# m-dayani/EORB_SLAM

Measured on AMD Instinct MI355X. Metric: front-end frames/s (event-accumulate + extract + match) per GPU; HBM GB/s vs roofline, higher is better.
Workload: dtype f32; 1 GPU; BASELINE.json configs[1]: synthetic 1000000 events/slice on 240x180 (shapes generator, DAVIS sensor pixels; raw (x,y,t,p) records resolved on the GPU through the calibrator's undistortion maps built from the EvETHZ intrinsics, as the reference loader does on the CPU), ev2im_gauss sigma=1 -> ORB-1000 (1.2, 4 levels, FAST 10/0, edge 19) -> SearchForInitialization vs previous slice; input=raw, sequences_per_gpu=1, parallelism=1 GPU

## Files before the change

### eorb_slam_amd/csrc/ev_slots.hip

```cpp
#include "eorb_ctx.h"
#include "ev_common.h"
#include "dev_math.h"
#include "sl_hot_asm.h"
#include <algorithm>
#include <memory>
#include <stdlib.h>
#include <string.h>
#include <vector>

namespace eorb {

constexpr uint32_t kNoSlot = 0xffu;
typedef uint16_t slot_entry;
constexpr uint32_t kEntryTag = 0x1000u;
constexpr int kSlotScatWaves = 8;
constexpr uint16_t kNoGeo = 0xffffu;
constexpr int kCountWaves = 16;

__global__ void sl_assign_kernel(const uint32_t* __restrict__ src_info, int nsrc, int W, int H, int h, int TX,
                                 uint32_t* __restrict__ tile_nslots, uint2* __restrict__ slot_tab, uint16_t* __restrict__ slot_geo,
                                 int* __restrict__ info)
{
    const int i = blockIdx.x * blockDim.x + threadIdx.x;
    if (i >= nsrc) { if (i == nsrc) slot_geo[i] = kNoGeo; return; }
    const uint32_t w = src_info[i];
    const int xi = (int)(int16_t)(w & 0xffff), yi = (int)(int16_t)(w >> 16);
    uint2 o = make_uint2(0u, 0xffffffffu);
    if (xi != -32768) {
        const int x0 = max(xi - h, 0), x1 = min(xi + h, W - 1), y0 = max(yi - h, 0), y1 = min(yi + h, H - 1);
        if (x1 >= x0 && y1 >= y0) {
            const int tx0 = x0 >> 3, tx1 = x1 >> 3, ty0 = y0 >> 3, ty1 = y1 >> 3;
            const int nx = tx1 - tx0 + 1, ny = ty1 - ty0 + 1;
            uint32_t slots = 0xffffffffu;
            for (int dy = 0; dy < ny; dy++)
                for (int dx = 0; dx < nx; dx++) {
                    uint32_t s = atomicAdd(&tile_nslots[(ty0 + dy) * TX + tx0 + dx], 1u);
                    if (s >= kNoSlot) { atomicOr(&info[2], 1); s = 0; }
                    const int sh = 8 * (dy * 2 + dx);
                    slots = (slots & ~(0xffu << sh)) | (s << sh);
                }
            o.x = (uint32_t)tx0 | ((uint32_t)ty0 << 8) | ((uint32_t)nx << 16) | ((uint32_t)ny << 18);
            o.y = slots;
        }
    }
    slot_tab[i] = o;
    slot_geo[i] = o.x ? (uint16_t)((o.x & 0x7f) | (((o.x >> 8) & 0x7f) << 7) | ((((o.x >> 16) & 3) - 1) << 14) | ((((o.x >> 18) & 3) - 1) << 15)) : kNoGeo;
}

__global__ __launch_bounds__(1024) void sl_rowbase_kernel(const uint32_t* __restrict__ nslots, int NT, uint32_t* __restrict__ rowbase,
                                                          int* __restrict__ info)
{
    __shared__ uint32_t wsum[16];
    __shared__ uint32_t wmax[16];
    const int tid = threadIdx.x, lane = tid & 63, wave = tid >> 6;
    const int per = (NT + 1023) / 1024;
    const int t0 = tid * per, t1 = min(t0 + per, NT);
    uint32_t mine = 0, mx = 0;
    for (int t = t0; t < t1; t++) { const uint32_t v = nslots[t]; mine += v; mx = max(mx, v); }
    uint32_t incl = (uint32_t)wave_incl_scan((int)mine);
#pragma unroll
    for (int d = 32; d >= 1; d >>= 1) mx = max(mx, (uint32_t)__shfl_xor((int)mx, d, 64));
    if (lane == 63) wsum[wave] = incl;
    if (lane == 0) wmax[wave] = mx;
    __syncthreads();
    uint32_t before = incl - mine;
    for (int w = 0; w < wave; w++) before += wsum[w];
    for (int t = t0; t < t1; t++) { rowbase[t] = before; before += nslots[t]; }
    if (tid == 1023) {
        uint32_t m = 0;
        for (int w = 0; w < 16; w++) m = max(m, wmax[w]);
        info[0] = (int)before; info[1] = (int)m;
    }
}

__global__ __launch_bounds__(256) void sl_rows_kernel(const uint32_t* __restrict__ src_info, const uint2* __restrict__ slot_tab, int nsrc,
                                                      int W, int H, int h, int TX, const float* __restrict__ stamps, int stamp_stride,
                                                      int SWP, const float2* __restrict__ lut, float two_sig2, float norm, const uint32_t* __restrict__ rowbase, float* __restrict__ rows)
{
    __shared__ uint64_t tab[32];
    if (threadIdx.x < 32) tab[threadIdx.x] = kExp2Tab[threadIdx.x];
    __syncthreads();
    const int src = blockIdx.x * 4 + (threadIdx.x >> 6), lane = threadIdx.x & 63;
    if (src >= nsrc) return;
    const uint2 st = slot_tab[src];
    const int nx = (st.x >> 16) & 3, ny = (st.x >> 18) & 3;
    if (!nx || !ny) return;
    const uint32_t w = src_info[src];
    const int xi = (int)(int16_t)(w & 0xffff), yi = (int)(int16_t)(w >> 16);
    const int tx0 = st.x & 0xff, ty0 = (st.x >> 8) & 0xff;
    for (int dy = 0; dy < ny; dy++)
        for (int dx = 0; dx < nx; dx++) {
            const uint32_t slot = (st.y >> (8 * (dy * 2 + dx))) & 0xffu;
            const int tile = (ty0 + dy) * TX + tx0 + dx;
            const int px = (tx0 + dx) * 8 + (lane & 7), py = (ty0 + dy) * 8 + (lane >> 3);
            const int i = px - xi + h, j = py - yi + h;
            float v = 0.0f;
            if (i >= 0 && i <= 2 * h && j >= 0 && j <= 2 * h && px < W && py < H) {
                if (stamps) v = stamps[(size_t)src * stamp_stride + i * SWP + j];
                else {
                    const float2 q = lut[src];
                    const float xr = q.x - (float)xi, yr = q.y - (float)yi;
                    const float fx = (float)(i - h) - xr, fy = (float)(j - h) - yr;
                    const float xx = fx * fx, yy = fy * fy;
                    float dd = xx + yy;
                    dd = dd / two_sig2;
                    v = dev_expf_nonpos<true>(-dd, tab) / norm;
                }
            }
            rows[((size_t)rowbase[tile] + slot) * 64 + lane] = v;
        }
}

constexpr int kOffsetsInArg = 256;
struct SliceOffsets { int64_t off[kOffsetsInArg + 1]; };
__global__ __launch_bounds__(256) void sl_chunks_kernel(SliceOffsets S, int B, int chunk_shift , int NT, int nchunks,
                                                        ChunkDesc* __restrict__ chunks, int* __restrict__ slice_c0, int64_t* __restrict__ slice_eb)
{
    __shared__ int c0[kOffsetsInArg + 1];
    __shared__ long long e0[kOffsetsInArg + 1];
    const int tid = threadIdx.x;
    const int64_t chunk = (int64_t)1 << chunk_shift;
    const int64_t* off = (const int64_t*)__builtin_amdgcn_kernarg_segment_ptr();
    const int64_t n = tid < B ? off[tid + 1] - off[tid] : 0;
    c0[tid + 1] = tid < B ? (int)((n + chunk - 1) >> chunk_shift) : 0;
    e0[tid + 1] = tid < B ? ((n * 4 + (int64_t)NT * 16 + 15) & ~(int64_t)15) : 0;
    if (tid == 0) { c0[0] = 0; e0[0] = 0; }
    __syncthreads();
    for (int d = 1; d < kOffsetsInArg; d <<= 1) {
        const int a = tid + 1 > d ? c0[tid + 1 - d] : 0;
        const long long b = tid + 1 > d ? e0[tid + 1 - d] : 0;
        __syncthreads();
        c0[tid + 1] += a; e0[tid + 1] += b;
        __syncthreads();
    }
    if (blockIdx.x == 0) {
        if (tid < B) slice_eb[tid] = e0[tid];
        for (int b = tid; b <= B; b += blockDim.x) slice_c0[b] = c0[b];
    }
    const int g = blockIdx.x * blockDim.x + tid;
    if (g >= nchunks) return;
    int lo = 0, hi = B;
    while (hi - lo > 1) { const int mid = (lo + hi) >> 1; if (c0[mid] <= g) lo = mid; else hi = mid; }
    const int64_t start = off[lo] + ((int64_t)(g - c0[lo]) << chunk_shift);
    ChunkDesc cd; cd.start = start; cd.n = (int32_t)min(chunk, off[lo + 1] - start); cd.slice = lo;
    chunks[g] = cd;
}

template <int stride>
__device__ __forceinline__ uint32_t sl_load_rec(const unsigned char* e, int k)
{
    if (stride == 2) { const uint32_t v = *(const uint16_t*)(e + (size_t)k * 2); return v == 0xffffu ? 0x7fffffffu : v; }
    return *(const uint32_t*)(e + (size_t)k * (size_t)(stride < 0 ? -stride : stride));
}
template <int stride>
__global__ __launch_bounds__(256) void sl_count_kernel(const eorb_raw_event* __restrict__ ev, const ChunkDesc* __restrict__ chunks,
                                                       const uint2* __restrict__ slot_tab, int LW, int LH, int TX, int NT,
                                                       uint16_t* __restrict__ segcnt)
{
    extern __shared__ uint32_t cnt[];
    const ChunkDesc cd = chunks[blockIdx.x];
    for (int i = threadIdx.x; i < NT; i += blockDim.x) cnt[i] = 0;
    __syncthreads();
    const unsigned char* e = (const unsigned char*)ev + (size_t)cd.start * (size_t)(stride < 0 ? -stride : stride);
    const uint32_t xmask = stride == 4 ? 0x7fffu : 0xffffu;
    const bool hashed = stride < 0 || stride == 2;
    constexpr int U = 8;
    for (int k0 = threadIdx.x; k0 < cd.n; k0 += blockDim.x * U) {
        uint32_t xy[U], rg[U];
#pragma unroll
        for (int u = 0; u < U; u++) { const int k = k0 + u * blockDim.x; xy[u] = k < cd.n ? sl_load_rec<stride>(e, k) : 0xffffffffu; }
#pragma unroll
        for (int u = 0; u < U; u++) {
            const int x = (int)(xy[u] & xmask), y = (int)(xy[u] >> 16);
            const uint32_t row = xy[u] & 0x7fffffffu;
            if (hashed) rg[u] = (row != 0x7fffffffu && row < (uint32_t)LW * (uint32_t)LH) ? slot_tab[row].x : 0u;
            else rg[u] = (x < LW && y < LH) ? slot_tab[(uint32_t)y * (uint32_t)LW + x].x : 0u;
        }
#pragma unroll
        for (int u = 0; u < U; u++) {
            const int nx = (rg[u] >> 16) & 3, ny = (rg[u] >> 18) & 3;
            const int t0 = (int)((rg[u] >> 8) & 0xff) * TX + (int)(rg[u] & 0xff);
            if (nx && ny) {
                atomicAdd(&cnt[t0], 1u);
                if (nx > 1) atomicAdd(&cnt[t0 + 1], 1u);
                if (ny > 1) { atomicAdd(&cnt[t0 + TX], 1u); if (nx > 1) atomicAdd(&cnt[t0 + TX + 1], 1u); }
            }
        }
    }
    __syncthreads();
    uint16_t* sc = segcnt + (size_t)blockIdx.x * NT;
    for (int i = threadIdx.x; i < NT; i += blockDim.x) sc[i] = (uint16_t)cnt[i];
}

__device__ __forceinline__ uint32_t sl_dict_hash(uint64_t k)
{
    k ^= k >> 33; k *= 0xff51afd7ed558ccdull; k ^= k >> 33; k *= 0xc4ceb9fe1a85ec53ull; k ^= k >> 33;
    return (uint32_t)k;
}
template <int stride, bool KEYED = false, bool RANKS = false>
__global__ __launch_bounds__(64 * kCountWaves) void sl_count_lds_kernel(const eorb_raw_event* __restrict__ ev, const ChunkDesc* __restrict__ chunks,
                                                                       int nchunks, const uint16_t* __restrict__ slot_geo, int LW, int LH,
                                                                       int TX, int NT, uint16_t* __restrict__ segcnt, SlotDict D = SlotDict{nullptr, 0u, nullptr, nullptr, 0},
                                                                       uint16_t* __restrict__ rec16 = nullptr)
{
    extern __shared__ uint32_t smc[];
    const int tid = threadIdx.x, lane = tid & 63, wave = tid >> 6;
    const int ntab = (LW * LH + 2) >> 1, NTp = (NT + 1) & ~1;
    for (int i = tid; i < ntab; i += 64 * kCountWaves) smc[i] = ((const uint32_t*)slot_geo)[i];
    const uint16_t* tab = (const uint16_t*)smc;
    uint32_t* cnt = smc + ntab + wave * (NTp >> 1);
    __syncthreads();
    constexpr int astride = stride < 0 ? -stride : stride;
    const uint32_t xmask = stride == 4 ? 0x7fffu : 0xffffu;
    constexpr int U = 8;
    for (int ch = blockIdx.x * kCountWaves + wave; ch < nchunks; ch += gridDim.x * kCountWaves) {
        const ChunkDesc cd = chunks[ch];
        for (int i = lane; i < (NTp >> 1); i += 64) cnt[i] = 0u;
        const unsigned char* e = (const unsigned char*)ev + (size_t)cd.start * (size_t)astride;
        uint32_t xyn[U];
        if (!KEYED) {
#pragma unroll
            for (int u = 0; u < U; u++) { const int k = lane + u * 64; xyn[u] = k < cd.n ? sl_load_rec<stride>(e, k) : 0xffffffffu; }
        }
        for (int k0 = lane; k0 < cd.n; k0 += 64 * U) {
            uint32_t xy[U], g[U];
            uint32_t r16[U];
            if (KEYED) {
                uint2 pos[U]; uint32_t ex[U], ey[U], ez[U], hh[U];
#pragma unroll
                for (int u = 0; u < U; u++) { const int k = k0 + u * 64; pos[u] = k < cd.n ? *(const uint2*)(e + (size_t)k * 16) : make_uint2(0x7fc00000u, 0x7fc00000u); }
#pragma unroll
                for (int u = 0; u < U; u++) { hh[u] = sl_dict_hash((uint64_t)pos[u].x | ((uint64_t)pos[u].y << 32)) & D.mask; const uint4 t = D.hash[hh[u]]; ex[u] = t.x; ey[u] = t.y; ez[u] = t.z; }
#pragma unroll
                for (int u = 0; u < U; u++) {
                    const int k = k0 + u * 64;
                    const float fx = __uint_as_float(pos[u].x), fy = __uint_as_float(pos[u].y);
                    uint32_t id = 0x7fffffffu;
                    if (k < cd.n && fx == fx && fy == fy) {
                        uint32_t h = hh[u], qx = ex[u], qy = ey[u], qz = ez[u]; int probes = 0;
                        while (!(qx == pos[u].x && qy == pos[u].y) && qz != 0xffffffffu && ++probes <= 64) { h = (h + 1) & D.mask; const uint4 t = D.hash[h]; qx = t.x; qy = t.y; qz = t.z; }
                        if (qx == pos[u].x && qy == pos[u].y && qz != 0xffffffffu) id = qz;
                        else atomicAdd(D.miss, 1);
                    }
                    if (RANKS) r16[u] = id < (uint32_t)LW * (uint32_t)LH ? id : 0xffffu;
                    else if (k < cd.n) {
                        if (D.rec2) ((uint16_t*)D.rec)[cd.start + k] = id == 0x7fffffffu ? (uint16_t)0xffffu : (uint16_t)id;
                        else D.rec[cd.start + k] = id;
                    }
                    g[u] = id < (uint32_t)LW * (uint32_t)LH ? tab[id] : kNoGeo;
                }
            } else {
#pragma unroll
            for (int u = 0; u < U; u++) xy[u] = xyn[u];
            if (k0 + 64 * U < cd.n) {
#pragma unroll
                for (int u = 0; u < U; u++) { const int k = k0 + 64 * U + u * 64; xyn[u] = k < cd.n ? sl_load_rec<stride>(e, k) : 0xffffffffu; }
            }
#pragma unroll
            for (int u = 0; u < U; u++) {
                const uint32_t x = xy[u] & xmask, y = xy[u] >> 16, row = xy[u] & 0x7fffffffu;
                if (stride < 0 || stride == 2) g[u] = row < (uint32_t)LW * (uint32_t)LH ? tab[row] : kNoGeo;
                else g[u] = (x < (uint32_t)LW && y < (uint32_t)LH) ? tab[y * (uint32_t)LW + x] : kNoGeo;
                if (RANKS) {
                    if (stride < 0 || stride == 2) r16[u] = row < (uint32_t)LW * (uint32_t)LH ? row : 0xffffu;
                    else r16[u] = (x < (uint32_t)LW && y < (uint32_t)LH) ? y * (uint32_t)LW + x : 0xffffu;
                } else if ((stride == 16 || stride == 4) && rec16) {
                    const int k = k0 + u * 64;
                    if (k < cd.n) rec16[cd.start + k] = (x < (uint32_t)LW && y < (uint32_t)LH) ? (uint16_t)(y * (uint32_t)LW + x) : (uint16_t)0xffffu;
                }
            }
            }
            if (RANKS) {
#pragma unroll
                for (int u = 0; u < U; u++) {
                    uint64_t rk = 0ull;
                    if (g[u] != kNoGeo) {
                        const int tx0 = (int)(g[u] & 0x7f), ty0 = (int)((g[u] >> 7) & 0x7f);
                        const int nx = 1 + (int)((g[u] >> 14) & 1), ny = 1 + (int)((g[u] >> 15) & 1);
#pragma unroll
                        for (int j = 0; j < 4; j++) {
                            const int dx = ((j & 1) - tx0) & 1, dy = ((j >> 1) - ty0) & 1;
                            if (dx < nx && dy < ny) {
                                const int t = (ty0 + dy) * TX + tx0 + dx;
                                const uint32_t o = atomicAdd(&cnt[t >> 1], 1u << (16 * (t & 1)));
                                rk |= (uint64_t)((o >> (16 * (t & 1))) & 0xfffu) << (12 * j);
                            }
                        }
                    }
                    const int k = k0 + u * 64;
                    if (k < cd.n) ((uint64_t*)rec16)[cd.start + k] = (uint64_t)(r16[u] & 0xffffu) | (rk << 16);
                }
                continue;
            }
#pragma unroll
            for (int u = 0; u < U; u++) {
                if (g[u] != kNoGeo) {
                    const int t0 = (int)((g[u] >> 7) & 0x7f) * TX + (int)(g[u] & 0x7f);
                    const bool two_x = (g[u] >> 14) & 1, two_y = (g[u] >> 15) & 1;
                    atomicAdd(&cnt[t0 >> 1], 1u << (16 * (t0 & 1)));
                    if (two_x) atomicAdd(&cnt[(t0 + 1) >> 1], 1u << (16 * ((t0 + 1) & 1)));
                    if (two_y) {
                        atomicAdd(&cnt[(t0 + TX) >> 1], 1u << (16 * ((t0 + TX) & 1)));
                        if (two_x) atomicAdd(&cnt[(t0 + TX + 1) >> 1], 1u << (16 * ((t0 + TX + 1) & 1)));
                    }
                }
            }
        }
        __builtin_amdgcn_wave_barrier();
        uint16_t* sc = segcnt + (size_t)ch * NT;
        const uint16_t* c16 = (const uint16_t*)cnt;
        for (int i = lane; i < NT; i += 64) sc[i] = c16[i];
        __builtin_amdgcn_wave_barrier();
    }
}

__global__ __launch_bounds__(1024) void sl_scan_kernel(const int* __restrict__ slice_chunk0, const uint16_t* __restrict__ segcnt, int NT,
                                                       uint32_t* __restrict__ segbase, uint32_t* __restrict__ tile_cnt,
                                                       uint32_t* __restrict__ tile_base)
{
    __shared__ uint32_t wsum[16];
    __shared__ uint32_t carry;
    const int slice = blockIdx.x;
    const int c0 = slice_chunk0[slice], c1 = slice_chunk0[slice + 1];
    const int lane = threadIdx.x & 63, wave = threadIdx.x >> 6;
    if (threadIdx.x == 0) carry = 0;
    __syncthreads();
    for (int t0 = 0; t0 < NT; t0 += blockDim.x) {
        const int tile = t0 + threadIdx.x;
        uint32_t run = 0;
        if (tile < NT) {
            int c = c0;
            for (; c + 8 <= c1; c += 8) {
                uint32_t v[8];
#pragma unroll
                for (int u = 0; u < 8; u++) v[u] = segcnt[(size_t)(c + u) * NT + tile];
#pragma unroll
                for (int u = 0; u < 8; u++) { segbase[(size_t)(c + u) * NT + tile] = run; run += v[u]; }
            }
            for (; c < c1; c++) { const uint32_t v = segcnt[(size_t)c * NT + tile]; segbase[(size_t)c * NT + tile] = run; run += v; }
            tile_cnt[(size_t)slice * NT + tile] = run;
        }
        const uint32_t padded = (run + 15u) & ~15u;
        uint32_t incl = (uint32_t)wave_incl_scan((int)padded);
        if (lane == 63) wsum[wave] = incl;
        __syncthreads();
        uint32_t before = carry;
        for (int w = 0; w < wave; w++) before += wsum[w];
        if (tile < NT) tile_base[(size_t)slice * NT + tile] = before + incl - padded;
        __syncthreads();
        if (threadIdx.x == blockDim.x - 1) carry = before + incl;
        __syncthreads();
    }
}

__global__ __launch_bounds__(64 * kSlotScatWaves) void sl_scatter_kernel(const eorb_raw_event* __restrict__ ev, const ChunkDesc* __restrict__ chunks,
                                                                         const uint2* __restrict__ slot_tab, int stride, int LW, int LH, int TX, int TY,
                                                                         int NT, int chunk_cap, const int64_t* __restrict__ slice_ebase,
                                                                         const uint32_t* __restrict__ segbase, const uint32_t* __restrict__ tile_base,
                                                                         slot_entry* __restrict__ entries)
{
    extern __shared__ unsigned char sm2[];
    __shared__ uint32_t s_wsum[kSlotScatWaves];
    constexpr int NTHR = 64 * kSlotScatWaves;
    constexpr int R = 2;
    const int tid = threadIdx.x, lane = tid & 63, wave = tid >> 6;
    const int chunk = blockIdx.x;
    const ChunkDesc cd = chunks[chunk];
    const int NTp = (NT + 1) & ~1;
    uint32_t* pay = (uint32_t*)sm2;
    uint16_t* prng = (uint16_t*)(pay + chunk_cap);
    uint16_t* sidx = prng + chunk_cap;
    uint16_t* cntw = sidx + (size_t)chunk_cap * R * R;
    uint16_t* loff = cntw + kSlotScatWaves * NTp;
    uint32_t* gbase = (uint32_t*)(loff + NTp + 2);
    for (int i = tid; i < kSlotScatWaves * NTp / 2; i += NTHR) ((uint32_t*)cntw)[i] = 0u;
    const unsigned char* e = (const unsigned char*)ev + (size_t)cd.start * (size_t)(stride < 0 ? -stride : stride);
    const uint32_t xmask = stride == 4 ? 0x7fffu : 0xffffu;
    const bool hashed = stride < 0 || stride == 2;
    const int Q = (((cd.n + kSlotScatWaves - 1) / kSlotScatWaves) + 63) & ~63;
    const int S = Q >> 6;
    constexpr int SMAX = 4;
    uint32_t rng[SMAX];
    __syncthreads();
    uint32_t* cw32 = (uint32_t*)(cntw + wave * NTp);
    uint32_t rsrc[SMAX];
#pragma unroll
    for (int s = 0; s < SMAX; s++) {
        const int k = wave * Q + s * 64 + lane;
        uint32_t q = 0xffffffffu;
        if (s < S && k < cd.n) q = stride == 2 ? sl_load_rec<2>(e, k) : *(const uint32_t*)(e + (size_t)k * (size_t)(stride < 0 ? -stride : stride));
        const int x = q == 0xffffffffu ? 0xffff : (int)(q & xmask), y = (int)(q >> 16);
        if (hashed) { const uint32_t row = q & 0x7fffffffu; rsrc[s] = (row != 0x7fffffffu && row < (uint32_t)LW * (uint32_t)LH) ? row : 0xffffffffu; }
        else rsrc[s] = (x < LW && y < LH) ? (uint32_t)y * (uint32_t)LW + x : 0xffffffffu;
    }
    uint2 rst[SMAX];
#pragma unroll
    for (int s = 0; s < SMAX; s++) rst[s] = rsrc[s] != 0xffffffffu ? slot_tab[rsrc[s]] : make_uint2(0u, 0xffffffffu);
#pragma unroll
    for (int s = 0; s < SMAX; s++) {
        rng[s] = 0u;
        const int k = wave * Q + s * 64 + lane;
        if (s < S && k < cd.n) {
            const uint32_t rg = rst[s].x;
            const int nx = (rg >> 16) & 3, ny = (rg >> 18) & 3;
            pay[k] = rst[s].y;
            prng[k] = (uint16_t)(rg & 0xffff);
            if (nx && ny) {
                rng[s] = rg;
                const int t0 = (int)((rg >> 8) & 0xff) * TX + (int)(rg & 0xff);
                for (int dy = 0; dy < ny; dy++)
                    for (int dx = 0; dx < nx; dx++) {
                        const int t = t0 + dy * TX + dx;
                        atomicAdd(&cw32[t >> 1], 1u << (16 * (t & 1)));
                    }
            }
        }
    }
    __syncthreads();
    {
        const int per = (NT + NTHR - 1) / NTHR;
        const int t0 = tid * per, t1 = min(t0 + per, NT);
        uint32_t mine = 0;
        for (int t = t0; t < t1; t++) {
            uint32_t run = 0;
#pragma unroll
            for (int w = 0; w < kSlotScatWaves; w++) { const uint32_t v = cntw[w * NTp + t]; cntw[w * NTp + t] = (uint16_t)run; run += v; }
            loff[t] = (uint16_t)run;
            mine += run;
            gbase[t] = tile_base[(size_t)cd.slice * NT + t] + segbase[(size_t)chunk * NT + t];
        }
        uint32_t incl = (uint32_t)wave_incl_scan((int)mine);
        if (lane == 63) s_wsum[wave] = incl;
        __syncthreads();
        uint32_t before = incl - mine;
        for (int w = 0; w < wave; w++) before += s_wsum[w];
        for (int t = t0; t < t1; t++) { const uint32_t v = loff[t]; loff[t] = (uint16_t)before; before += v; }
        if (tid == NTHR - 1) loff[NT] = (uint16_t)before;
    }
    __syncthreads();
    const uint64_t lt_mask = (lane == 0) ? 0ull : (~0ull >> (64 - lane));
    uint16_t* cw = cntw + wave * NTp;
    const int txr = (TX + R - 1) / R;
    int mbits = 1; while ((1 << mbits) < txr * ((TY + R - 1) / R)) mbits++;
#pragma unroll
    for (int s = 0; s < SMAX; s++) {
        if (s >= S) break;
        const uint32_t rg = rng[s];
        const int tx0 = rg & 0xff, ty0 = (rg >> 8) & 0xff, tx1 = tx0 + (int)((rg >> 16) & 3) - 1, ty1 = ty0 + (int)((rg >> 18) & 3) - 1;
        const bool valid = rg != 0u;
        const uint16_t kloc = (uint16_t)(wave * Q + s * 64 + lane);
#pragma unroll
        for (int cy = 0; cy < R; cy++) {
#pragma unroll
            for (int cx = 0; cx < R; cx++) {
                const int tx = tx0 + ((cx - tx0 % R) + R) % R;
                const int ty = ty0 + ((cy - ty0 % R) + R) % R;
                const bool has = valid && tx <= tx1 && ty <= ty1;
                uint64_t m = __ballot(has);
                if (m == 0ull) continue;
                const int key = has ? ty * TX + tx : 0;
                const int mkey = has ? (ty / R) * txr + (tx / R) : 0;
                for (int b = 0; b < mbits; b++) {
                    const bool bit = (mkey >> b) & 1;
                    const uint64_t bal = __ballot(bit);
                    m &= bit ? bal : ~bal;
                }
                if (has) {
                    const int rank = __popcll(m & lt_mask);
                    const uint32_t base = cw[key];
                    sidx[(uint32_t)loff[key] + base + rank] = (uint16_t)(kloc | ((tx - tx0) << 11) | ((ty - ty0) << 13));
                    if (rank == 0) cw[key] = (uint16_t)(base + (uint32_t)__popcll(m));
                }
            }
        }
    }
    __syncthreads();
    slot_entry* out = entries + (size_t)slice_ebase[cd.slice];
    const int E = loff[NT];
    for (int p = tid; p < E; p += NTHR) {
        const uint32_t sv = sidx[p];
        const int k = sv & 0x7ff;
        const int dx = (sv >> 11) & 3, dy = (sv >> 13) & 3;
        const uint32_t r0 = prng[k];
        const int t = ((int)(r0 >> 8) + dy) * TX + (int)(r0 & 0xff) + dx;
        const uint32_t slot = (pay[k] >> (8 * (dy * 2 + dx))) & 0xffu;
        out[(size_t)gbase[t] + (uint32_t)(p - (int)loff[t])] = (slot_entry)(kEntryTag | slot);
    }
}

template <int stride, int NW >
__global__ __launch_bounds__(64 * NW) void sl_scatter_rank_kernel(const eorb_raw_event* __restrict__ ev, const ChunkDesc* __restrict__ chunks,
                                                                              const uint2* __restrict__ slot_tab, int LW, int LH, int TX, int NT,
                                                                              int chunk_cap, const int64_t* __restrict__ slice_ebase,
                                                                              const uint32_t* __restrict__ segbase, const uint32_t* __restrict__ tile_base,
                                                                              slot_entry* __restrict__ entries)
{
    extern __shared__ unsigned char sm2[];
    __shared__ uint32_t s_wsum[NW];
    constexpr int NTHR = 64 * NW;
    const int tid = threadIdx.x, lane = tid & 63, wave = tid >> 6;
    const int chunk = blockIdx.x;
    const ChunkDesc cd = chunks[chunk];
    const int NTp = (NT + 1) & ~1;
    uint32_t* gbase = (uint32_t*)sm2;
    uint16_t* stile = (uint16_t*)(gbase + NT);
    uint16_t* cntw = stile + (size_t)chunk_cap * 4;
    uint16_t* loff = cntw + NW * NTp;
    uint8_t* sorted = (uint8_t*)(loff + NTp + 2);
    for (int i = tid; i < NW * NTp / 2; i += NTHR) ((uint32_t*)cntw)[i] = 0u;
    const unsigned char* e = (const unsigned char*)ev + (size_t)cd.start * (size_t)(stride < 0 ? -stride : stride);
    const uint32_t xmask = stride == 4 ? 0x7fffu : 0xffffu;
    const bool hashed = stride < 0 || stride == 2;
    const int Q = (((cd.n + NW - 1) / NW) + 63) & ~63;
    const int S = Q >> 6;
    constexpr int SMAX = 4;
    __syncthreads();
    uint32_t* cw32 = (uint32_t*)(cntw + wave * NTp);
    uint32_t rsrc[SMAX];
#pragma unroll
    for (int s = 0; s < SMAX; s++) {
        const int k = wave * Q + s * 64 + lane;
        const uint32_t q = (s < S && k < cd.n) ? sl_load_rec<stride>(e, k) : 0xffffffffu;
        const int x = q == 0xffffffffu ? 0xffff : (int)(q & xmask), y = (int)(q >> 16);
        if (hashed) { const uint32_t row = q & 0x7fffffffu; rsrc[s] = (row != 0x7fffffffu && row < (uint32_t)LW * (uint32_t)LH) ? row : 0xffffffffu; }
        else rsrc[s] = (x < LW && y < LH) ? (uint32_t)y * (uint32_t)LW + x : 0xffffffffu;
    }
    uint2 rst[SMAX];
#pragma unroll
    for (int s = 0; s < SMAX; s++) rst[s] = rsrc[s] != 0xffffffffu ? slot_tab[rsrc[s]] : make_uint2(0u, 0xffffffffu);
    uint32_t rk[SMAX];
#pragma unroll
    for (int s = 0; s < SMAX; s++) {
        const uint32_t rg = rst[s].x;
        const int nx = (rg >> 16) & 3, ny = (rg >> 18) & 3;
        const int tx0 = rg & 0xff, ty0 = (rg >> 8) & 0xff;
        rk[s] = 0u;
#pragma unroll
        for (int j = 0; j < 4; j++) {
#ifdef EORB_TEST_RANK_ORDER_BUG
            const int dx = j & 1, dy = j >> 1;
#else
            const int dx = ((j & 1) - tx0) & 1, dy = ((j >> 1) - ty0) & 1;
#endif
            if (nx && ny && dx < nx && dy < ny) {
                const int t = (ty0 + dy) * TX + tx0 + dx;
                const uint32_t o = atomicAdd(&cw32[t >> 1], 1u << (16 * (t & 1)));
                rk[s] |= ((o >> (16 * (t & 1))) & 0xffu) << (8 * j);
            }
        }
    }
    __syncthreads();
#if defined(EORB_KO_SCAT) && EORB_KO_SCAT == 1
    if (rk[0] == 0x12345678u) entries[0] = 0; return;
#endif
    {
        const int per = (NT + NTHR - 1) / NTHR;
        const int t0 = tid * per, t1 = min(t0 + per, NT);
        uint32_t mine = 0;
        for (int t = t0; t < t1; t++) {
            uint32_t run = 0;
#pragma unroll
            for (int w = 0; w < NW; w++) { const uint32_t v = cntw[w * NTp + t]; cntw[w * NTp + t] = (uint16_t)run; run += v; }
            loff[t] = (uint16_t)run;
            mine += run;
        }
        uint32_t incl = (uint32_t)wave_incl_scan((int)mine);
        if (lane == 63) s_wsum[wave] = incl;
        __syncthreads();
        uint32_t before = incl - mine;
        for (int w = 0; w < wave; w++) before += s_wsum[w];
        for (int t = t0; t < t1; t++) {
            const uint32_t v = loff[t]; loff[t] = (uint16_t)before;
            gbase[t] = tile_base[(size_t)cd.slice * NT + t] + segbase[(size_t)chunk * NT + t] - before;
            before += v;
        }
        if (tid == NTHR - 1) loff[NT] = (uint16_t)before;
    }
    __syncthreads();
#if defined(EORB_KO_SCAT) && EORB_KO_SCAT == 2
    if (rk[0] == 0x12345678u) entries[0] = 0; return;
#endif
    const uint16_t* cw = cntw + wave * NTp;
#pragma unroll
    for (int s = 0; s < SMAX; s++) {
        const uint32_t rg = rst[s].x, sb = rst[s].y;
        const int nx = (rg >> 16) & 3, ny = (rg >> 18) & 3;
        const int tx0 = rg & 0xff, ty0 = (rg >> 8) & 0xff;
#pragma unroll
        for (int j = 0; j < 4; j++) {
#ifdef EORB_TEST_RANK_ORDER_BUG
            const int dx = j & 1, dy = j >> 1;
#else
            const int dx = ((j & 1) - tx0) & 1, dy = ((j >> 1) - ty0) & 1;
#endif
            if (nx && ny && dx < nx && dy < ny) {
                const int t = (ty0 + dy) * TX + tx0 + dx;
                const uint32_t pos = (uint32_t)loff[t] + cw[t] + ((rk[s] >> (8 * j)) & 0xffu);
                sorted[pos] = (uint8_t)((sb >> (8 * (dy * 2 + dx))) & 0xffu);
                stile[pos] = (uint16_t)t;
            }
        }
    }
    __syncthreads();
#if defined(EORB_KO_SCAT) && EORB_KO_SCAT == 3
    if (rk[0] == 0x12345678u) entries[0] = 0; return;
#endif
    slot_entry* out = entries + (size_t)slice_ebase[cd.slice];
    const int E = loff[NT];
    for (int p = tid; p < E; p += NTHR) out[(size_t)(uint32_t)(gbase[stile[p]] + (uint32_t)p)] = (slot_entry)(kEntryTag | sorted[p]);
}

template <int NW>
__global__ __launch_bounds__(64 * NW) void sl_scatter_pre_kernel(const uint64_t* __restrict__ rec, const ChunkDesc* __restrict__ chunks,
                                                                 const uint2* __restrict__ slot_tab, int nsrc, int TX, int NT, int chunk_cap,
                                                                 const int64_t* __restrict__ slice_ebase, const uint16_t* __restrict__ segcnt,
                                                                 const uint32_t* __restrict__ segbase, const uint32_t* __restrict__ tile_base,
                                                                 slot_entry* __restrict__ entries)
{
    extern __shared__ unsigned char sm2[];
    __shared__ uint32_t s_wsum[NW];
    constexpr int NTHR = 64 * NW;
    const int tid = threadIdx.x, lane = tid & 63, wave = tid >> 6;
    const int chunk = blockIdx.x;
    const ChunkDesc cd = chunks[chunk];
    const int NTp = (NT + 1) & ~1;
    uint32_t* gbase = (uint32_t*)sm2;
    uint16_t* stile = (uint16_t*)(gbase + NT);
    uint16_t* loff = stile + (size_t)chunk_cap * 4;
    uint8_t* sorted = (uint8_t*)(loff + NTp + 2);
    const int Q = (((cd.n + NW - 1) / NW) + 63) & ~63;
    const int S = Q >> 6;
    constexpr int SMAX = 4;
    uint64_t rr[SMAX]; uint2 rst[SMAX];
#pragma unroll
    for (int s = 0; s < SMAX; s++) {
        const int k = wave * Q + s * 64 + lane;
        rr[s] = (s < S && k < cd.n) ? rec[cd.start + k] : 0xffffull;
    }
#pragma unroll
    for (int s = 0; s < SMAX; s++) {
        const uint32_t row = (uint32_t)(rr[s] & 0xffffull);
        rst[s] = (row != 0xffffu && row < (uint32_t)nsrc) ? slot_tab[row] : make_uint2(0u, 0xffffffffu);
    }
    {
        const int per = (NT + NTHR - 1) / NTHR;
        const int t0 = tid * per, t1 = min(t0 + per, NT);
        const uint16_t* sc = segcnt + (size_t)chunk * NT;
        uint32_t mine = 0;
        for (int t = t0; t < t1; t++) mine += sc[t];
        uint32_t incl = (uint32_t)wave_incl_scan((int)mine);
        if (lane == 63) s_wsum[wave] = incl;
        __syncthreads();
        uint32_t before = incl - mine;
        for (int w = 0; w < wave; w++) before += s_wsum[w];
        for (int t = t0; t < t1; t++) {
            const uint32_t v = sc[t];
            loff[t] = (uint16_t)before;
            gbase[t] = tile_base[(size_t)cd.slice * NT + t] + segbase[(size_t)chunk * NT + t] - before;
            before += v;
        }
        if (tid == NTHR - 1) loff[NT] = (uint16_t)before;
    }
    __syncthreads();
#if defined(EORB_KO_SCAT) && EORB_KO_SCAT == 2
    if (rst[0].x == 0x12345678u) entries[0] = 0; return;
#endif
#pragma unroll
    for (int s = 0; s < SMAX; s++) {
        const uint32_t rg = rst[s].x, sb = rst[s].y;
        const int nx = (rg >> 16) & 3, ny = (rg >> 18) & 3;
        const int tx0 = rg & 0xff, ty0 = (rg >> 8) & 0xff;
        const uint64_t rk = rr[s] >> 16;
#pragma unroll
        for (int j = 0; j < 4; j++) {
            const int dx = ((j & 1) - tx0) & 1, dy = ((j >> 1) - ty0) & 1;
            if (nx && ny && dx < nx && dy < ny) {
                const int t = (ty0 + dy) * TX + tx0 + dx;
                const uint32_t pos = (uint32_t)loff[t] + (uint32_t)((rk >> (12 * j)) & 0xfffull);
                sorted[pos] = (uint8_t)((sb >> (8 * (dy * 2 + dx))) & 0xffu);
                stile[pos] = (uint16_t)t;
            }
        }
    }
    __syncthreads();
#if defined(EORB_KO_SCAT) && EORB_KO_SCAT == 3
    if (rst[0].x == 0x12345678u) entries[0] = 0; return;
#endif
    slot_entry* out = entries + (size_t)slice_ebase[cd.slice];
    const int E = loff[NT];
    for (int p = tid; p < E; p += NTHR) out[(size_t)(uint32_t)(gbase[stile[p]] + (uint32_t)p)] = (slot_entry)(kEntryTag | sorted[p]);
}

__global__ __launch_bounds__(1024) void sl_rankcheck_kernel(unsigned long long* bad)
{
    __shared__ uint32_t cnt[16 * 64];
    __shared__ uint32_t noise[1024];
    const int lane = threadIdx.x & 63, wave = threadIdx.x >> 6;
    unsigned long long nbad = 0;
    uint32_t h = (uint32_t)(blockIdx.x * 1024 + threadIdx.x) * 2654435761u + 12345u;
    for (int t = 0; t < 64; t++) {
        for (int i = threadIdx.x; i < 16 * 64; i += blockDim.x) cnt[i] = 0;
        __syncthreads();
        h = h * 1664525u + 1013904223u;
        const int spread = 1 << (1 + (t % 7));
        const uint32_t a = ((h >> 9) % spread) + wave * 128;
        const bool act = ((h >> 3) & 7u) != 0u;
        uint32_t r = 0xffffffffu;
        noise[(threadIdx.x * 33 + t) & 1023] = h;
        uint32_t rr[4];
#pragma unroll
        for (int q = 0; q < 4; q++) {
            rr[q] = 0xffffffffu;
            if (act && ((h >> (12 + q)) & 1u)) { const uint32_t o = atomicAdd(&cnt[a >> 1], 1u << (16 * (a & 1))); rr[q] = (o >> (16 * (a & 1))) & 0xffffu; }
        }
#pragma unroll
        for (int q = 0; q < 4; q++) {
            r = rr[q];
            for (int j = 0; j < 64; j++) {
                const uint32_t aj = __shfl(a, j, 64), rj = __shfl(r, j, 64);
                if (r != 0xffffffffu && rj != 0xffffffffu && j < lane && aj == a && !(rj < r)) nbad++;
            }
        }
        __syncthreads();
    }
    if (noise[threadIdx.x] == 0x12345u) nbad += 0;
    if (nbad) atomicAdd(bad, nbad);
}

constexpr int kHotBuckets = 16, kHotCap = 8192;
struct HotDesc { uint32_t slice, tile, cnt, off_lo, off_hi, tx0, ty0, rows_off; };
__global__ __launch_bounds__(256) void sl_plan_kernel(const uint32_t* __restrict__ tile_cnt, const uint32_t* __restrict__ tile_base,
                                                      const int64_t* __restrict__ slice_ebase, int B, int NT, int TX, uint32_t hot_min,
                                                      const uint32_t* __restrict__ nslots, const uint32_t* __restrict__ rowbase,
                                                      uint4* __restrict__ items, uint32_t* __restrict__ tile_w, uint32_t* __restrict__ tile_m,
                                                      uint32_t* __restrict__ ctr, uint32_t* __restrict__ hot_cnt, HotDesc* __restrict__ hot_items,
                                                      uint32_t hot_cap )
{
    extern __shared__ uint32_t pc[];
    __shared__ uint32_t red[8];
    __shared__ uint32_t hb[kHotBuckets], hbase[kHotBuckets];
    uint32_t* hloc = pc + B;
    const int t = blockIdx.x, tid = threadIdx.x;
    const bool hot_ok = hot_min != 0u && nslots[t] <= (uint32_t)SL_HOT_NROWS;
    if (tid < kHotBuckets) hb[tid] = 0u;
    __syncthreads();
    for (int s = tid; s < B; s += blockDim.x) {
        const uint32_t c = tile_cnt[(size_t)s * NT + t];
        uint32_t v = c;
        if (hot_ok && c >= hot_min) {
            const int lg = 31 - __clz(c), lg0 = 31 - __clz(hot_min);
            const int q = (lg - lg0) * 4 + (int)((c >> max(lg - 2, 0)) & 3u) - (int)((hot_min >> max(lg0 - 2, 0)) & 3u);
            const int b = kHotBuckets - 1 - min(max(q, 0), kHotBuckets - 1);
            hloc[s] = ((uint32_t)b << 16) | atomicAdd(&hb[b], 1u);
            v = c | 0x80000000u;
        }
        pc[s] = v;
    }
    __syncthreads();
    if (tid < kHotBuckets) hbase[tid] = hb[tid] ? atomicAdd(&hot_cnt[tid], hb[tid]) : 0u;
    __syncthreads();
    uint32_t sum = 0, mx = 0;
    for (int s = tid; s < B; s += blockDim.x) {
        uint32_t v = pc[s];
        if (v & 0x80000000u) {
            const uint32_t c = v & 0x7fffffffu, b = hloc[s] >> 16, k = hbase[b] + (hloc[s] & 0xffffu);
            if (k < hot_cap) {
                const uint64_t off = ((uint64_t)slice_ebase[s] + tile_base[(size_t)s * NT + t]) * sizeof(slot_entry);
                HotDesc d; d.slice = (uint32_t)s; d.tile = (uint32_t)t; d.cnt = c; d.off_lo = (uint32_t)off; d.off_hi = (uint32_t)(off >> 32);
                d.tx0 = (uint32_t)(t % TX) * 8u; d.ty0 = (uint32_t)(t / TX) * 8u; d.rows_off = rowbase[t] * 256u;
                hot_items[(size_t)b * kHotCap + k] = d;
            } else { v = c; pc[s] = v; atomicAdd(&hot_cnt[33], 1u); }
        }
        if (!(v & 0x80000000u)) { sum += v; mx = max(mx, v); }
    }
    __syncthreads();
    const bool sorted = B <= 2048;
    for (int s = tid; s < B; s += blockDim.x) {
        const uint32_t c = pc[s];
        int rank = s;
        if (sorted) { rank = 0; for (int j = 0; j < B; j++) { const uint32_t v = pc[j]; rank += (v > c || (v == c && j < s)) ? 1 : 0; } }
        const uint64_t off = ((uint64_t)slice_ebase[s] + tile_base[(size_t)s * NT + t]) * sizeof(slot_entry);
        items[(size_t)t * B + rank] = make_uint4((uint32_t)s | (c & 0x80000000u), c & 0x7fffffffu, (uint32_t)off, (uint32_t)(off >> 32));
    }
#pragma unroll
    for (int d = 32; d >= 1; d >>= 1) { sum += (uint32_t)__shfl_xor((int)sum, d, 64); mx = max(mx, (uint32_t)__shfl_xor((int)mx, d, 64)); }
    if ((tid & 63) == 0) { red[tid >> 6] = sum; red[4 + (tid >> 6)] = mx; }
    __syncthreads();
    if (tid == 0) {
        tile_w[t] = red[0] + red[1] + red[2] + red[3];
        tile_m[t] = max(max(red[4], red[5]), max(red[6], red[7]));
        ctr[t] = 0u;
    }
}
__global__ __launch_bounds__(1024) void sl_tasks_kernel(const uint32_t* __restrict__ tile_w, const uint32_t* __restrict__ tile_m, int NT, int G,
                                                        int max_per_tile, uint32_t* __restrict__ scratch , uint32_t* __restrict__ task_tile, uint32_t* __restrict__ hot_cnt,
                                                        uint32_t hot_cap)
{
    if (threadIdx.x < kHotBuckets) hot_cnt[threadIdx.x] = min(hot_cnt[threadIdx.x], hot_cap);
    __shared__ unsigned long long wred[16];
    __shared__ uint32_t wsum[16], wsum2[16];
    const int tid = threadIdx.x, lane = tid & 63, wave = tid >> 6;
    unsigned long long tot = 0;
    for (int t = tid; t < NT; t += 1024) tot += tile_w[t];
#pragma unroll
    for (int d = 32; d >= 1; d >>= 1) tot += (unsigned long long)__shfl_xor((long long)tot, d, 64);
    if (lane == 0) wred[wave] = tot;
    __syncthreads();
    tot = 0;
    for (int w = 0; w < 16; w++) tot += wred[w];
    const unsigned long long spare = (unsigned long long)max(G - NT, 0);
    uint32_t* nsorted = scratch; uint32_t* tsorted = scratch + NT;
    extern __shared__ uint32_t tm[];
    for (int t = tid; t < NT; t += 1024) tm[t] = tile_m[t];
    __syncthreads();
    for (int t = tid; t < NT; t += 1024) {
        const uint32_t m = tm[t];
        int rank = 0;
        for (int u = 0; u < NT; u++) { const uint32_t v = tm[u]; rank += (v > m || (v == m && u < t)) ? 1 : 0; }
        uint32_t n = 1u + (tot ? (uint32_t)((unsigned long long)tile_w[t] * spare / tot) : 0u);
        n = min(n, (uint32_t)max(max_per_tile, 1));
        nsorted[rank] = n; tsorted[rank] = (uint32_t)t;
    }
    __syncthreads();
    const int per = (NT + 1023) / 1024;
    const int r0 = tid * per, r1 = min(r0 + per, NT);
    uint32_t mine1 = 0, mine2 = 0;
    for (int r = r0; r < r1; r++) { const uint32_t n = nsorted[r], a = min(n, 2u); mine1 += a; mine2 += n - a; }
    const uint32_t incl1 = (uint32_t)wave_incl_scan((int)mine1), incl2 = (uint32_t)wave_incl_scan((int)mine2);
    if (lane == 63) { wsum[wave] = incl1; wsum2[wave] = incl2; }
    __syncthreads();
    uint32_t b1 = incl1 - mine1, b2 = incl2 - mine2, tot1 = 0;
    for (int w = 0; w < 16; w++) { if (w < wave) { b1 += wsum[w]; b2 += wsum2[w]; } tot1 += wsum[w]; }
    b2 += tot1;
    for (int r = r0; r < r1; r++) {
        const uint32_t n = nsorted[r], a = min(n, 2u), t = tsorted[r];
        for (uint32_t k = 0; k < a; k++) if (b1 + k < (uint32_t)G) task_tile[b1 + k] = t;
        for (uint32_t k = 0; k < n - a; k++) if (b2 + k < (uint32_t)G) task_tile[b2 + k] = t;
        b1 += a; b2 += n - a;
    }
    const uint32_t before = b2;
    if (tid == 1023) for (uint32_t k = before; k < (uint32_t)G; k++) task_tile[k] = 0xffffffffu;
}

struct SlotGather {
    const uint32_t* task_tile; const uint4* items; const uint8_t* entries;
    const uint32_t* nslots; const uint32_t* rowbase; const float* rows; const uint32_t* tile_w; uint32_t* ctr;
    float* img; uint32_t* minmax_enc; int* info; int* status;
    int B, W, H, TX, NT, null_slot; uint32_t prio_ref;
    unsigned long long* trace;
};

__global__ __launch_bounds__(1024) __attribute__((amdgpu_waves_per_eu(8, 8)))
void sl_gather_kernel(SlotGather P)
{
    extern __shared__ __attribute__((aligned(16))) float lds[];
    const int tid = threadIdx.x, lane = tid & 63;
#ifdef EORB_SLOT_TRACE
    const unsigned long long tr_t0 = wall_clock64(); unsigned long long tr_ent = 0, tr_items = 0, tr_kept = 0;
#endif
    const uint32_t task = P.task_tile[blockIdx.x];
    if (task == 0xffffffffu) return;
    const int tile = (int)task;
    const uint32_t wt = P.tile_w[tile];
    const int tx0 = (tile % P.TX) * kTile, ty0 = (tile / P.TX) * kTile;
    const int px = tx0 + (lane & 7), py = ty0 + (lane >> 3);
    const bool inimg = px < P.W && py < P.H;
    if ((uint32_t)(uintptr_t)lds != 0u) { if (tid == 0) { atomicOr(&P.info[3], 1); atomicOr(P.status, 256); } return; }
    if (wt) {
        const int ns = (int)P.nslots[tile];
        const int n4 = ns * 16;
        const float4* src = (const float4*)(P.rows + (size_t)P.rowbase[tile] * 64);
        float4* dst = (float4*)lds;
        for (int i = tid; i < n4; i += blockDim.x) dst[i] = src[i];
        if (tid < 16) dst[P.null_slot * 16 + tid] = make_float4(0.f, 0.f, 0.f, 0.f);
    }
    __syncthreads();
    const uint32_t nullword = (uint32_t)P.null_slot * 0x00010001u;
    uint32_t* const ctr = P.ctr + tile;
    const uint32_t lane4 = (uint32_t)lane * 4u;
    uint32_t sel0 = 0x0c0c0400u, sel1 = 0x0c0c0600u;
    asm volatile("" : "+v"(sel0), "+v"(sel1));
    const int nit = P.B;
    const uint4* const items = P.items + (size_t)tile * P.B;
    auto ticket = [&]() { int t = 0; if (lane == 0) t = (int)atomicAdd(ctr, 1u); return t; };
    auto uni = [&](uint32_t v) { return (uint32_t)__builtin_amdgcn_readfirstlane((int)v); };
    auto item_of = [&](int tkv) { return (int)min((uint32_t)__builtin_amdgcn_readfirstlane(tkv), (uint32_t)nit); };
    int k = item_of(ticket());
    uint4 d = make_uint4(0u, 0u, 0u, 0u);
    if (k < nit) d = items[k];
    uint4 En = make_uint4(0u, 0u, 0u, 0u);
    bool have_first = false;
    while (k < nit) {
        const bool hot = (uni(d.x) >> 31) != 0u;
        const int s = (int)(uni(d.x) & 0x7fffffffu);
        const uint32_t cnt = hot ? 0u : uni(d.y);
        const uint4* const list = (const uint4*)(P.entries + (((uint64_t)uni(d.w) << 32) | uni(d.z)));
        if (cnt >= P.prio_ref) __builtin_amdgcn_s_setprio(3);
        else if (cnt >= P.prio_ref / 4u) __builtin_amdgcn_s_setprio(2);
        else if (cnt >= P.prio_ref / 16u) __builtin_amdgcn_s_setprio(1);
        else __builtin_amdgcn_s_setprio(0);
        float acc = 0.0f;
        const int nblk = (int)((cnt + 511u) >> 9);
        if (!have_first && nblk) En = list[lane];
        have_first = false;
        int tk = 0; int stage_t = 0;
        uint4 dn = make_uint4(0u, 0u, 0u, 0u); int kn = nit;
        for (int b = 0; b < nblk; b++) {
            uint4 E = En;
            if (stage_t == 1) { kn = item_of(tk); if (kn < nit) dn = items[kn]; stage_t = 2; }
            else if (stage_t == 0 && nblk - b <= 4) { tk = ticket(); stage_t = 1; }
            if (b + 1 < nblk) En = list[(size_t)(b + 1) * 64 + lane];
            else if (stage_t == 2 && kn < nit && uni(dn.y)) {
                En = ((const uint4*)(P.entries + (((uint64_t)uni(dn.w) << 32) | uni(dn.z))))[lane];
                have_first = true;
            }
            const int rem = (int)cnt - b * 512;
            if (rem < 512) {
                auto fix = [&](uint32_t w, int dd) {
                    const int nv = rem - lane * 8 - dd * 2;
                    const uint32_t keep = nv >= 2 ? 0xffffffffu : (nv <= 0 ? 0u : 0xffffu);
                    return (w & keep) | (nullword & ~keep);
                };
                E.x = fix(E.x, 0); E.y = fix(E.y, 1); E.z = fix(E.z, 2); E.w = fix(E.w, 3);
            }
            const int lane_end = (min(64, (rem + 7) >> 3) + 1) & ~1;
#ifdef EORB_SLOT_TRACE
            tr_kept += (unsigned long long)lane_end * 8;
#endif
            {
            float r0, r1, r2, r3, r4, r5, r6, r7, r8, r9, r10, r11, r12, r13, r14, r15;
            int sl, sl1, se, sf;
#define SL_GROUP(EV, EW, SL, RA, RB, RC, RD, AA, AB, AC, AD) \
            "s_waitcnt lgkmcnt(8)\n" \
            "v_readlane_b32 %[se], %[" EV "], %[" SL "]\n" \
            "v_add_f32 %[acc], %[acc], %[" AA "]\n" \
            "v_readlane_b32 %[sf], %[" EW "], %[" SL "]\n" \
            "v_perm_b32 %[" RA "], %[se], %[l4], %[q0]\n" \
            "v_perm_b32 %[" RB "], %[se], %[l4], %[q1]\n" \
            "ds_read_b32 %[" RA "], %[" RA "]\n" \
            "v_add_f32 %[acc], %[acc], %[" AB "]\n" \
            "v_perm_b32 %[" RC "], %[sf], %[l4], %[q0]\n" \
            "ds_read_b32 %[" RB "], %[" RB "]\n" \
            "v_add_f32 %[acc], %[acc], %[" AC "]\n" \
            "v_perm_b32 %[" RD "], %[sf], %[l4], %[q1]\n" \
            "ds_read_b32 %[" RC "], %[" RC "]\n" \
            "v_add_f32 %[acc], %[acc], %[" AD "]\n" \
            "ds_read_b32 %[" RD "], %[" RD "]\n"
            asm volatile(
                "v_mov_b32 %[r4], 0\n v_mov_b32 %[r5], 0\n v_mov_b32 %[r6], 0\n v_mov_b32 %[r7], 0\n"
                "v_mov_b32 %[r8], 0\n v_mov_b32 %[r9], 0\n v_mov_b32 %[r10], 0\n v_mov_b32 %[r11], 0\n"
                "v_mov_b32 %[r12], 0\n v_mov_b32 %[r13], 0\n v_mov_b32 %[r14], 0\n v_mov_b32 %[r15], 0\n"
                "s_mov_b32 %[sl], 0\n"
                "1:\n"
                "s_add_u32 %[sl1], %[sl], 1\n"
                SL_GROUP("e0", "e1", "sl", "r0", "r1", "r2", "r3", "r4", "r5", "r6", "r7")
                SL_GROUP("e2", "e3", "sl", "r4", "r5", "r6", "r7", "r8", "r9", "r10", "r11")
                SL_GROUP("e0", "e1", "sl1", "r8", "r9", "r10", "r11", "r12", "r13", "r14", "r15")
                SL_GROUP("e2", "e3", "sl1", "r12", "r13", "r14", "r15", "r0", "r1", "r2", "r3")
                "s_add_u32 %[sl], %[sl], 2\n"
                "s_cmp_lt_u32 %[sl], %[lend]\n"
                "s_cbranch_scc1 1b\n"
                "s_waitcnt lgkmcnt(0)\n"
                "v_add_f32 %[acc], %[acc], %[r4]\n v_add_f32 %[acc], %[acc], %[r5]\n v_add_f32 %[acc], %[acc], %[r6]\n v_add_f32 %[acc], %[acc], %[r7]\n"
                "v_add_f32 %[acc], %[acc], %[r8]\n v_add_f32 %[acc], %[acc], %[r9]\n v_add_f32 %[acc], %[acc], %[r10]\n v_add_f32 %[acc], %[acc], %[r11]\n"
                "v_add_f32 %[acc], %[acc], %[r12]\n v_add_f32 %[acc], %[acc], %[r13]\n v_add_f32 %[acc], %[acc], %[r14]\n v_add_f32 %[acc], %[acc], %[r15]\n"
                : [acc] "+v"(acc), [r0] "=&v"(r0), [r1] "=&v"(r1), [r2] "=&v"(r2), [r3] "=&v"(r3), [r4] "=&v"(r4), [r5] "=&v"(r5),
                  [r6] "=&v"(r6), [r7] "=&v"(r7), [r8] "=&v"(r8), [r9] "=&v"(r9), [r10] "=&v"(r10), [r11] "=&v"(r11),
                  [r12] "=&v"(r12), [r13] "=&v"(r13), [r14] "=&v"(r14), [r15] "=&v"(r15),
                  [sl] "=&s"(sl), [sl1] "=&s"(sl1), [se] "=&s"(se), [sf] "=&s"(sf)
                : [e0] "v"(E.x), [e1] "v"(E.y), [e2] "v"(E.z), [e3] "v"(E.w), [lend] "s"(lane_end), [l4] "v"(lane4),
                  [q0] "v"(sel0), [q1] "v"(sel1), [ldsp] "v"(lds)
                : "scc", "memory");
#undef SL_GROUP
            }
        }
        if (inimg && !hot) P.img[(size_t)s * P.W * P.H + (size_t)py * P.W + px] = acc;
        if (cnt) {
            float vmax = inimg ? acc : -1000000.0f;
#pragma unroll
            for (int dd = 32; dd >= 1; dd >>= 1) vmax = fmaxf(vmax, __shfl_xor(vmax, dd, 64));
            if (lane == 0) atomicMax(&P.minmax_enc[s * 2 + 1], enc_f32(vmax));
        }
#ifdef EORB_SLOT_TRACE
        tr_ent += cnt; tr_items++;
#endif
        if (stage_t == 0) { tk = ticket(); stage_t = 1; }
        if (stage_t == 1) { kn = item_of(tk); if (kn < nit) dn = items[kn]; }
        k = kn; d = dn;
    }
#ifdef EORB_SLOT_TRACE
    if (lane == 0 && P.trace) {
        unsigned long long* r = P.trace + ((size_t)blockIdx.x * 16 + (tid >> 6)) * 6;
        r[0] = (unsigned long long)tile; r[1] = tr_t0; r[2] = wall_clock64(); r[3] = tr_ent; r[4] = tr_items; r[5] = tr_kept;
    }
#endif
}

__global__ __launch_bounds__(64) void sl_hot_kernel(const uint32_t* __restrict__ hcnt, uint32_t* __restrict__ ticket, const HotDesc* __restrict__ items,
                                                    int hcap, const float* __restrict__ rows, const slot_entry* __restrict__ entries,
                                                    float* __restrict__ img, uint32_t* __restrict__ mm, int W, int H)
{
    const uint32_t rows_lo = (uint32_t)(uintptr_t)rows, rows_hi = (uint32_t)((uintptr_t)rows >> 32);
    const uint32_t ent_lo = (uint32_t)(uintptr_t)entries, ent_hi = (uint32_t)((uintptr_t)entries >> 32);
    const uint32_t img_lo = (uint32_t)(uintptr_t)img, img_hi = (uint32_t)((uintptr_t)img >> 32);
    asm volatile(SL_HOT_ASM
                 :
                 : [hcnt] "s"(hcnt), [ticket] "s"(ticket), [items] "s"(items), [hcap] "s"(hcap), [rows_lo] "s"(rows_lo), [rows_hi] "s"(rows_hi),
                   [ent_lo] "s"(ent_lo), [ent_hi] "s"(ent_hi), [img_lo] "s"(img_lo), [img_hi] "s"(img_hi), [mm] "s"(mm), [W] "s"(W), [H] "s"(H)
                 : SL_HOT_CLOBBERS);
}

int ev_slots_prepare_launch(eorb_ctx* c, int W, int H, int h, int TX, int TY)
{
    c->sl_ok = 0; c->sl_launched = 0;
    if (h < 1 || h > 4 || TX >= 256 || TY >= 256) return EORB_OK;
    const int nsrc = c->lut_w * c->lut_h, NT = TX * TY;
    int rc;
    const size_t geo_off = sizeof(uint2) * (size_t)nsrc;
    if ((rc = ensure(c, c->sl_tab, geo_off + sizeof(uint16_t) * ((size_t)nsrc + 2)))) return rc;
    if ((rc = ensure(c, c->sl_tile, sizeof(uint32_t) * (5 * (size_t)NT + 8)))) return rc;
    uint32_t* d_nslots = (uint32_t*)c->sl_tile.p;
    uint32_t* d_rowbase = d_nslots + NT;
    int* d_info = (int*)(d_nslots + 5 * (size_t)NT);
    c->sl_info_off = sizeof(uint32_t) * 5 * (size_t)NT;
    EORB_HIP(c, hipMemsetAsync(c->sl_tile.p, 0, sizeof(uint32_t) * (5 * (size_t)NT + 8), c->stream));
    sl_assign_kernel<<<(nsrc + 256) / 256, 256, 0, c->stream>>>((const uint32_t*)c->src_info.p, nsrc, W, H, h, TX, d_nslots, (uint2*)c->sl_tab.p,
                                                                (uint16_t*)((char*)c->sl_tab.p + geo_off), d_info);
    sl_rowbase_kernel<<<1, 1024, 0, c->stream>>>(d_nslots, NT, d_rowbase, d_info);
    EORB_LAUNCH_CHECK(c, "slot table kernels");
    if (c->sl_rank_ok < 0) {
        unsigned long long* d_bad = (unsigned long long*)(d_info + 4);
        sl_rankcheck_kernel<<<128, 512, 0, c->stream>>>(d_bad);
        sl_rankcheck_kernel<<<128, 1024, 0, c->stream>>>(d_bad);
    }
    int* rb = readback_buf(c);
    if (!rb) return set_err(c, EORB_E_HIP, "pinned alloc failed");
    EORB_HIP(c, hipMemcpyAsync(rb + 8, d_info, sizeof(c->sl_hinfo), hipMemcpyDeviceToHost, c->stream));
    c->sl_launched = 1;
    return EORB_OK;
}

int ev_slots_prepare_finish(eorb_ctx* c, int W, int H, int h, int TX, int TY, const float* d_stamps, int stamp_stride, int SWP, float two_sig2, float norm)
{
    if (!c->sl_launched) return EORB_OK;
    c->sl_launched = 0;
    const int nsrc = c->lut_w * c->lut_h, NT = TX * TY;
    memcpy(c->sl_hinfo, readback_buf(c) + 8, sizeof(c->sl_hinfo));
    const int* hinfo = c->sl_hinfo;
    int rc;
    if (c->sl_rank_ok < 0) c->sl_rank_ok = (hinfo[4] == 0 && hinfo[5] == 0) ? 1 : 0;
    if (hinfo[2] || hinfo[1] >= (int)kNoSlot || hinfo[0] <= 0) return EORB_OK;
    if ((rc = ensure(c, c->sl_rows, sizeof(float) * 64 * (size_t)hinfo[0] + 4096 + 256 * 256))) return rc;
    const uint32_t* d_rowbase = (const uint32_t*)c->sl_tile.p + NT;
    sl_rows_kernel<<<(nsrc + 3) / 4, 256, 0, c->stream>>>((const uint32_t*)c->src_info.p, (const uint2*)c->sl_tab.p, nsrc, W, H, h, TX, d_stamps,
                                                            stamp_stride, SWP, (const float2*)c->lut.p, two_sig2, norm, d_rowbase, (float*)c->sl_rows.p);
    EORB_LAUNCH_CHECK(c, "sl_rows_kernel");
    c->sl_null = hinfo[1];
    c->sl_ok = 1;
    return EORB_OK;
}

int ev_slots_prepare(eorb_ctx* c, int W, int H, int h, int TX, int TY, const float* d_stamps, int stamp_stride, int SWP, float two_sig2, float norm)
{
    int rc;
    if (!c->sl_launched) {
        if ((rc = ev_slots_prepare_launch(c, W, H, h, TX, TY))) return rc;
        if (!c->sl_launched) return EORB_OK;
        EORB_HIP(c, hipStreamSynchronize(c->stream));
    }
    return ev_slots_prepare_finish(c, W, H, h, TX, TY, d_stamps, stamp_stride, SWP, two_sig2, norm);
}

static int sl_optin(eorb_ctx* c, int bit, const void* fn, int bytes)
{
    if (c->sl_attr & (1u << bit)) return EORB_OK;
    EORB_HIP(c, hipFuncSetAttribute(fn, hipFuncAttributeMaxDynamicSharedMemorySize, bytes));
    c->sl_attr |= 1u << bit;
    return EORB_OK;
}
static int sl_ncu(eorb_ctx* c)
{
    if (!c->ncu) { hipDeviceProp_t pr; if (hipGetDeviceProperties(&pr, c->device) == hipSuccess) c->ncu = pr.multiProcessorCount; if (c->ncu <= 0) c->ncu = 256; }
    return c->ncu;
}

constexpr int kSlotDeclined = 1;

struct SlotScatterChoice { int chunk, waves; bool rank; size_t lds; };
static size_t sl_lds_rank(int NT, int chunk, int waves) { const int NTp = (NT + 1) & ~1; return ((size_t)NT * 4 + (size_t)chunk * 4 * 2 + (size_t)waves * NTp * 2 + (size_t)(NTp + 2) * 2 + (size_t)chunk * 4 + 15) & ~(size_t)15; }
static size_t sl_lds_pre(int NT, int chunk) { const int NTp = (NT + 1) & ~1; return ((size_t)NT * 4 + (size_t)chunk * 4 * 2 + (size_t)(NTp + 2) * 2 + (size_t)chunk * 4 + 15) & ~(size_t)15; }
static size_t sl_lds_ballot(int NT, int chunk) { const int NTp = (NT + 1) & ~1; return ((size_t)chunk * 4 + (size_t)chunk * 2 + (size_t)chunk * 4 * 2 + (size_t)kSlotScatWaves * NTp * 2 + (size_t)(NTp + 2) * 2 + (size_t)NT * 4 + 15) & ~(size_t)15; }
static bool sl_choose_scatter(const eorb_ctx* c, int NT, int64_t per_slice, bool rank_allowed, SlotScatterChoice* out)
{
    static const int chunk_env = [] { const char* e = getenv("EORB_SLOT_CHUNK"); const int v = e ? atoi(e) : 0; return (v == 256 || v == 1024 || v == 2048 || v == 4096) ? v : 0; }();
    const int pref = chunk_env ? chunk_env : (per_slice >= (int64_t)1 << 18 ? 4096 : (per_slice >= (int64_t)1 << 17 ? 2048 : (per_slice >= (int64_t)1 << 14 ? 1024 : 256)));
    static const int sizes[4] = {4096, 2048, 1024, 256};
    for (int i = 0; i < 4; i++) {
        const int chunk = sizes[i];
        if (chunk > pref) continue;
        if (rank_allowed) {
            const int waves = chunk == 4096 ? 16 : kSlotScatWaves;
            const size_t l = sl_lds_rank(NT, chunk, waves);
            if (l <= (size_t)(chunk == 4096 ? 79 : 158) * 1024) { *out = {chunk, waves, true, l}; return true; }
        }
        if (chunk <= 2048) {
            const size_t l = sl_lds_ballot(NT, chunk);
            if (l <= 64 * 1024) { *out = {chunk, kSlotScatWaves, false, l}; return true; }
        }
    }
    (void)c;
    return false;
}

static int sl_streams(eorb_ctx* c)
{
    if (c->sl_side) return EORB_OK;
    int lo = 0, hi = 0;
    (void)hipDeviceGetStreamPriorityRange(&lo, &hi);
    hipStream_t st[3] = {nullptr, nullptr, nullptr};
    hipEvent_t ev[eorb_ctx::kSlotEvents];
    for (auto& e : ev) e = nullptr;
    bool ok = hipStreamCreateWithPriority(&st[0], hipStreamNonBlocking, hi) == hipSuccess && hipStreamCreateWithFlags(&st[1], hipStreamNonBlocking) == hipSuccess &&
              hipStreamCreateWithFlags(&st[2], hipStreamNonBlocking) == hipSuccess;
    for (int i = 0; ok && i < eorb_ctx::kSlotEvents; i++) ok = hipEventCreateWithFlags(&ev[i], hipEventDisableTiming) == hipSuccess;
    if (!ok) {
        for (auto& e : ev) if (e) (void)hipEventDestroy(e);
        for (auto& q : st) if (q) (void)hipStreamDestroy(q);
        return set_err(c, EORB_E_HIP, "slot form: streams / events");
    }
    c->sl_side = st[0]; c->sl_pstream = st[1]; c->sl_gstream = st[2];
    for (int i = 0; i < eorb_ctx::kSlotEvents; i++) c->sl_ev[i] = ev[i];
    return EORB_OK;
}

static int slots_part(eorb_ctx* c, eorb_ctx::SlotWS& ws, int part, int nparts, const void* d_events, int stride_in, const int64_t* h_offsets, int B,
                      int W, int H, int TX, int TY, float* d_f32, uint32_t* d_minmax_enc, const SlotScatterChoice& sc, const SlotDict* dict)
{
    const int stride = dict ? (dict->rec2 ? 2 : -4) : stride_in;
    const int NT = TX * TY;
    const int64_t nev = h_offsets[B] - h_offsets[0];
    const int chunk = sc.chunk;
    hipStream_t M = c->stream, P = c->sl_pstream, Hs = c->sl_side, G = nparts > 1 ? c->sl_gstream : c->stream;
    hipEvent_t* E = c->sl_ev + 5 * part;
    const bool on_dev = B <= kOffsetsInArg;
    std::vector<ChunkDesc> cds;
    std::vector<int> slice_c0(on_dev ? 0 : B + 1);
    std::vector<int64_t> slice_eb(on_dev ? 0 : B + 1);
    int64_t eb = 0, nch = 0;
    for (int b = 0; b < B; b++) {
        if (!on_dev) slice_c0[b] = (int)nch;
        const int64_t s = h_offsets[b], e = h_offsets[b + 1];
        if (!on_dev) slice_eb[b] = eb;
        eb = (eb + (e - s) * 4 + (int64_t)NT * 16 + 15) & ~(int64_t)15;
        nch += (e - s + chunk - 1) / chunk;
        if (!on_dev)
            for (int64_t k = s; k < e; k += chunk) {
                ChunkDesc cd; cd.start = k; cd.n = (int32_t)std::min<int64_t>(chunk, e - k); cd.slice = b;
                cds.push_back(cd);
            }
    }
    if (nch >= (int64_t)1 << 31) return set_err(c, EORB_E_CAPACITY, "ev_accumulate: too many chunks");
    if (!on_dev) { slice_c0[B] = (int)nch; slice_eb[B] = eb; }
    const int nchunks = (int)nch;
    const size_t cd_bytes = sizeof(ChunkDesc) * (size_t)std::max(nchunks, 1);
    const size_t sc_bytes = (sizeof(int) * (size_t)(B + 1) + 7) & ~(size_t)7;
    const size_t eb_bytes = sizeof(int64_t) * (size_t)B;
    const int nb = B * NT;
    c->sl_last_nb[part] = nb;
    int rc;
    if ((rc = ensure(c, ws.chunks, cd_bytes + sc_bytes + eb_bytes))) return rc;
    const size_t cnt_bytes = (sizeof(uint16_t) * (size_t)std::max(nchunks, 1) * NT + 15) & ~(size_t)15;
    if ((rc = ensure(c, ws.segoff, cnt_bytes + sizeof(uint32_t) * (size_t)std::max(nchunks, 1) * NT))) return rc;
    if ((rc = ensure(c, ws.entries, sizeof(slot_entry) * (size_t)eb + 8192))) return rc;
    if ((rc = ensure(c, ws.tile_order, sizeof(uint32_t) * 2 * (size_t)nb))) return rc;
    if (on_dev) {
        SliceOffsets so;
        for (int b = 0; b <= B; b++) so.off[b] = h_offsets[b];
        sl_chunks_kernel<<<std::max(1, (nchunks + 255) / 256), 256, 0, M>>>(so, B, chunk == 4096 ? 12 : (chunk == 2048 ? 11 : (chunk == 1024 ? 10 : 8)), NT, nchunks, (ChunkDesc*)ws.chunks.p, (int*)((char*)ws.chunks.p + cd_bytes),
                                                                                  (int64_t*)((char*)ws.chunks.p + cd_bytes + sc_bytes));
    }
    else {
        char* hp = (char*)pinned(c, cd_bytes + sc_bytes + eb_bytes);
        if (!hp) return set_err(c, EORB_E_HIP, "pinned alloc failed");
        if (nchunks) memcpy(hp, cds.data(), sizeof(ChunkDesc) * nchunks);
        memcpy(hp + cd_bytes, slice_c0.data(), sizeof(int) * (size_t)(B + 1));
        memcpy(hp + cd_bytes + sc_bytes, slice_eb.data(), eb_bytes);
        EORB_HIP(c, hipMemcpyAsync(ws.chunks.p, hp, cd_bytes + sc_bytes + eb_bytes, hipMemcpyHostToDevice, M));
        pinned_commit(c);
    }
    const ChunkDesc* d_chunks = (const ChunkDesc*)ws.chunks.p;
    const int* d_slice_c0 = (const int*)((char*)ws.chunks.p + cd_bytes);
    const int64_t* d_slice_eb = (const int64_t*)((char*)ws.chunks.p + cd_bytes + sc_bytes);
    uint16_t* d_segcnt = (uint16_t*)ws.segoff.p;
    uint32_t* d_segbase = (uint32_t*)((char*)ws.segoff.p + cnt_bytes);
    uint32_t* d_tile_cnt = (uint32_t*)ws.tile_order.p;
    uint32_t* d_tile_base = d_tile_cnt + nb;
    uint32_t* d_nslots = (uint32_t*)c->sl_tile.p;
    uint32_t* d_rowbase = d_nslots + NT;
    int* d_info = (int*)(d_nslots + 5 * (size_t)NT);
    const eorb_raw_event* d_ev = dict ? (const eorb_raw_event*)dict->rec : (const eorb_raw_event*)d_events;
    int scat_stride = stride;
    bool prerank = false;
    const uint2* d_tab = (const uint2*)c->sl_tab.p;
    const int ncu = sl_ncu(c);
    const int NTp = (NT + 1) & ~1;
    const size_t lds_g = (size_t)(c->sl_null + 1) * 256;
    const int wg_per_cu = std::max(1, (int)((160 * 1024) / lds_g));
    static const int nw_env = [] { const char* e = getenv("EORB_SLOT_WAVES"); return e ? atoi(e) : 0; }();
    static const int ns_env = [] { const char* e = getenv("EORB_SLOT_ROUNDS"); return e ? atoi(e) : 0; }();
    int nw = std::min(16, std::max(1, 16 / wg_per_cu));
    if (nw_env >= 1 && nw_env <= 16) nw = nw_env;
    nw = std::min(nw, std::max(1, B));
    const int rounds = ns_env >= 1 ? ns_env : 4;
    const int Gt = NT + rounds * ncu * wg_per_cu;
    const int max_per_tile = (B + nw - 1) / nw;
    if ((rc = ensure(c, ws.plan, sizeof(uint4) * (size_t)nb + sizeof(uint32_t) * ((size_t)Gt + 5 * (size_t)NT)))) return rc;
    uint4* d_items = (uint4*)ws.plan.p;
    uint32_t* d_task = (uint32_t*)(d_items + nb);
    uint32_t* d_tile_m = d_task + Gt;
    uint32_t* d_scr = d_tile_m + NT;
    uint32_t* d_tile_w = d_scr + 2 * (size_t)NT;
    uint32_t* d_ctr = d_tile_w + NT;
    const uint32_t prio_ref = (uint32_t)std::min<int64_t>(std::max<int64_t>(4096, nev / 2000), 0x7fffffff);
    static const long long hot_env = [] { const char* e = getenv("EORB_SLOT_HOT_MIN"); return e ? atoll(e) : -1ll; }();
    uint32_t hot_min = c->sl_null <= SL_HOT_NROWS ? (uint32_t)std::min<int64_t>(std::max<int64_t>(4096, nev * nparts / 16000), 0x7fffffff) : 0u;
    const long long hot_over = c->dbg_slot_hot_min >= 0 ? c->dbg_slot_hot_min : hot_env;
    if (hot_over >= 0) hot_min = (c->sl_null <= SL_HOT_NROWS && hot_over > 0) ? (uint32_t)std::min<long long>(std::max<long long>(hot_over, 64), 0x7fffffff) : 0u;
    const uint32_t hot_cap = c->dbg_slot_hot_cap > 0 ? (uint32_t)std::min(c->dbg_slot_hot_cap, kHotCap) : (uint32_t)kHotCap;
    if ((rc = ensure(c, ws.hot, sizeof(HotDesc) * (size_t)kHotBuckets * kHotCap + 256))) return rc;
    uint32_t* d_hot_cnt = (uint32_t*)ws.hot.p;
    HotDesc* d_hot_items = (HotDesc*)((char*)ws.hot.p + 256);
    {
        std::unique_ptr<ProfScope> ps(new ProfScope(c, "ev_count"));
        const size_t lds = sizeof(uint32_t) * (size_t)NT;
        const size_t nsrc = (size_t)c->lut_w * (size_t)c->lut_h;
        const size_t lds_c = 4 * ((nsrc + 2) / 2) + (size_t)kCountWaves * NTp * 2;
        static const int cl_env = [] { const char* e = getenv("EORB_SLOT_COUNT_LDS"); return e ? atoi(e) : 1; }();
        if (dict && !(TX <= 127 && TY <= 127 && lds_c <= 159 * 1024)) return set_err(c, EORB_E_CAPACITY, "slot form: the position dictionary needs the LDS count pass");
        if (nchunks && dict) {
            const uint16_t* d_geo = (const uint16_t*)((const char*)c->sl_tab.p + sizeof(uint2) * nsrc);
            const int g = std::min(ncu, (nchunks + kCountWaves - 1) / kCountWaves);
            static const int pre_env_d = [] { const char* e = getenv("EORB_SLOT_PRERANK"); return e ? atoi(e) : 1; }();
            const int pre_on_d = c->dbg_slot_prerank >= 0 ? c->dbg_slot_prerank : pre_env_d;
            if (pre_on_d && dict->rec2 && sc.rank && sl_lds_pre(NT, chunk) <= 158 * 1024) {
                if ((rc = ensure(c, ws.rec16, sizeof(uint64_t) * (size_t)std::max<int64_t>(h_offsets[B], 1)))) return rc;
                prerank = true;
                if ((rc = sl_optin(c, 21, (const void*)sl_count_lds_kernel<16, true, true>, 159 * 1024))) return rc;
                sl_count_lds_kernel<16, true, true><<<g, 64 * kCountWaves, lds_c, M>>>((const eorb_raw_event*)d_events, d_chunks, nchunks, d_geo, c->lut_w, c->lut_h, TX, NT, d_segcnt, *dict, (uint16_t*)ws.rec16.p);
            } else {
            if ((rc = sl_optin(c, 13, (const void*)sl_count_lds_kernel<16, true>, 159 * 1024))) return rc;
            sl_count_lds_kernel<16, true><<<g, 64 * kCountWaves, lds_c, M>>>((const eorb_raw_event*)d_events, d_chunks, nchunks, d_geo, c->lut_w, c->lut_h, TX, NT, d_segcnt, *dict);
            }
        }
        else if (nchunks && cl_env && TX <= 127 && TY <= 127 && lds_c <= 159 * 1024) {
            const uint16_t* d_geo = (const uint16_t*)((const char*)c->sl_tab.p + sizeof(uint2) * nsrc);
            const int g = std::min(ncu, (nchunks + kCountWaves - 1) / kCountWaves);
            static const int tc_env = [] { const char* e = getenv("EORB_SLOT_TRANSCODE"); return e ? atoi(e) : 1; }();
            uint16_t* d_rec16 = nullptr;
            static const int pre_env = [] { const char* e = getenv("EORB_SLOT_PRERANK"); return e ? atoi(e) : 1; }();
            const int pre_on = c->dbg_slot_prerank >= 0 ? c->dbg_slot_prerank : pre_env;
            if (pre_on && (stride == 16 || stride == 4 || stride == 2) && nsrc <= 65535 && sc.rank && sl_lds_pre(NT, chunk) <= 158 * 1024) {
                if ((rc = ensure(c, ws.rec16, sizeof(uint64_t) * (size_t)std::max<int64_t>(h_offsets[B], 1)))) return rc;
                d_rec16 = (uint16_t*)ws.rec16.p;
                prerank = true;
#define SL_COUNTR(ST, BIT) do { if ((rc = sl_optin(c, BIT, (const void*)sl_count_lds_kernel<ST, false, true>, 159 * 1024))) return rc; \
                sl_count_lds_kernel<ST, false, true><<<g, 64 * kCountWaves, lds_c, M>>>(d_ev, d_chunks, nchunks, d_geo, c->lut_w, c->lut_h, TX, NT, d_segcnt, SlotDict{nullptr, 0u, nullptr, nullptr, 0}, d_rec16); } while (0)
                if (stride == 16) SL_COUNTR(16, 18); else if (stride == 4) SL_COUNTR(4, 19); else SL_COUNTR(2, 20);
#undef SL_COUNTR
            }
            else {
            if (tc_env && stride == 16 && nsrc <= 65535 && sc.rank) {
                if ((rc = ensure(c, ws.rec16, sizeof(uint16_t) * (size_t)std::max<int64_t>(h_offsets[B], 1)))) return rc;
                d_rec16 = (uint16_t*)ws.rec16.p;
            }
#define SL_COUNT(ST, BIT) do { if ((rc = sl_optin(c, BIT, (const void*)sl_count_lds_kernel<ST>, 159 * 1024))) return rc; \
                sl_count_lds_kernel<ST><<<g, 64 * kCountWaves, lds_c, M>>>(d_ev, d_chunks, nchunks, d_geo, c->lut_w, c->lut_h, TX, NT, d_segcnt, SlotDict{nullptr, 0u, nullptr, nullptr}, d_rec16); } while (0)
            if (stride == 16) SL_COUNT(16, 0); else if (stride == 4) SL_COUNT(4, 1); else if (stride == 2) SL_COUNT(2, 10); else SL_COUNT(-4, 2);
#undef SL_COUNT
            if (d_rec16) { d_ev = (const eorb_raw_event*)d_rec16; scat_stride = 2; }
            }
        }
        else if (nchunks) {
            if (stride == 16) sl_count_kernel<16><<<nchunks, 256, lds, M>>>(d_ev, d_chunks, d_tab, c->lut_w, c->lut_h, TX, NT, d_segcnt);
            else if (stride == 4) sl_count_kernel<4><<<nchunks, 256, lds, M>>>(d_ev, d_chunks, d_tab, c->lut_w, c->lut_h, TX, NT, d_segcnt);
            else if (stride == 2) sl_count_kernel<2><<<nchunks, 256, lds, M>>>(d_ev, d_chunks, d_tab, c->lut_w, c->lut_h, TX, NT, d_segcnt);
            else sl_count_kernel<-4><<<nchunks, 256, lds, M>>>(d_ev, d_chunks, d_tab, c->lut_w, c->lut_h, TX, NT, d_segcnt);
        }
        ps.reset(); ps.reset(new ProfScope(c, "ev_scan"));
        sl_scan_kernel<<<B, 1024, 0, M>>>(d_slice_c0, d_segcnt, NT, d_segbase, d_tile_cnt, d_tile_base);
        ps.reset();
        EORB_HIP(c, hipEventRecord(E[0], M));
        EORB_HIP(c, hipStreamWaitEvent(P, E[0], 0));
        EORB_HIP(c, hipMemsetAsync(ws.hot.p, 0, 256, P));
        sl_plan_kernel<<<NT, 256, sizeof(uint32_t) * 2 * (size_t)B, P>>>(d_tile_cnt, d_tile_base, d_slice_eb, B, NT, TX, hot_min, d_nslots, d_rowbase,
                                                                               d_items, d_tile_w, d_tile_m, d_ctr, d_hot_cnt, d_hot_items, hot_cap);
        sl_tasks_kernel<<<1, 1024, sizeof(uint32_t) * (size_t)NT, P>>>(d_tile_w, d_tile_m, NT, Gt, max_per_tile, d_scr, d_task, d_hot_cnt, hot_cap);
        EORB_HIP(c, hipEventRecord(E[1], P));
        ProfScope ps2(c, "ev_scatter");
        const int stride = scat_stride;
        if (nchunks && prerank) {
            const size_t lds_p = sl_lds_pre(NT, chunk);
            const uint16_t* d_segcnt_c = d_segcnt;
            if (sc.waves == 16) {
                if ((rc = sl_optin(c, 16, (const void*)sl_scatter_pre_kernel<16>, 159 * 1024))) return rc;
                sl_scatter_pre_kernel<16><<<nchunks, 64 * 16, lds_p, M>>>((const uint64_t*)ws.rec16.p, d_chunks, d_tab, c->lut_w * c->lut_h, TX, NT, chunk, d_slice_eb, d_segcnt_c, d_segbase, d_tile_base, (slot_entry*)ws.entries.p);
            } else {
                if ((rc = sl_optin(c, 17, (const void*)sl_scatter_pre_kernel<8>, 159 * 1024))) return rc;
                sl_scatter_pre_kernel<8><<<nchunks, 64 * 8, lds_p, M>>>((const uint64_t*)ws.rec16.p, d_chunks, d_tab, c->lut_w * c->lut_h, TX, NT, chunk, d_slice_eb, d_segcnt_c, d_segbase, d_tile_base, (slot_entry*)ws.entries.p);
            }
        }
        else if (nchunks && sc.rank) {
#define SL_SCAT(ST, NW, BIT) do { if ((rc = sl_optin(c, BIT, (const void*)sl_scatter_rank_kernel<ST, NW>, 159 * 1024))) return rc; \
                sl_scatter_rank_kernel<ST, NW><<<nchunks, 64 * NW, sc.lds, M>>>(d_ev, d_chunks, d_tab, c->lut_w, c->lut_h, TX, NT, chunk, \
                                                                                   d_slice_eb, d_segbase, d_tile_base, (slot_entry*)ws.entries.p); } while (0)
            if (sc.waves == 16) { if (stride == 16) SL_SCAT(16, 16, 3); else if (stride == 4) SL_SCAT(4, 16, 4); else if (stride == 2) SL_SCAT(2, 16, 11); else SL_SCAT(-4, 16, 5); }
            else { if (stride == 16) SL_SCAT(16, 8, 6); else if (stride == 4) SL_SCAT(4, 8, 7); else if (stride == 2) SL_SCAT(2, 8, 12); else SL_SCAT(-4, 8, 8); }
#undef SL_SCAT
        }
        else if (nchunks)
            sl_scatter_kernel<<<nchunks, 64 * kSlotScatWaves, sc.lds, M>>>(d_ev, d_chunks, d_tab, stride, c->lut_w, c->lut_h, TX, TY, NT, chunk,
                                                                                 d_slice_eb, d_segbase, d_tile_base, (slot_entry*)ws.entries.p);
        EORB_LAUNCH_CHECK(c, "ev_bin (slot) kernels");
    }
    EORB_HIP(c, hipEventRecord(E[2], M));
    {
        SlotGather Pg{d_task, d_items, (const uint8_t*)ws.entries.p, d_nslots, d_rowbase, (const float*)c->sl_rows.p,
                      d_tile_w, d_ctr, d_f32, d_minmax_enc, d_info, (int*)c->status.p, B, W, H, TX, NT, c->sl_null, prio_ref, nullptr};
#ifdef EORB_SLOT_TRACE
        if ((rc = ensure(c, c->sl_trace, sizeof(unsigned long long) * 6 * 16 * (size_t)Gt + 64))) return rc;
        EORB_HIP(c, hipMemsetAsync(c->sl_trace.p, 0, sizeof(unsigned long long) * 6 * 16 * (size_t)Gt + 64, M));
        Pg.trace = (unsigned long long*)c->sl_trace.p + 8;
        c->sl_trace_n = (long long)Gt * 16;
#endif
        if ((rc = sl_optin(c, 9, (const void*)sl_gather_kernel, 160 * 1024))) return rc;
        if (hot_min) {
            static const int hw_env = [] { const char* e = getenv("EORB_SLOT_HOT_WAVES"); return e ? atoi(e) : 0; }();
            const int hw = c->dbg_slot_hot_waves > 0 ? c->dbg_slot_hot_waves : (hw_env > 0 ? hw_env : 8 * ncu);
            EORB_HIP(c, hipStreamWaitEvent(Hs, E[2], 0));
            EORB_HIP(c, hipStreamWaitEvent(Hs, E[1], 0));
            sl_hot_kernel<<<hw, 64, 0, Hs>>>(d_hot_cnt, d_hot_cnt + 32, d_hot_items, kHotCap, (const float*)c->sl_rows.p, (const slot_entry*)ws.entries.p,
                                             d_f32, d_minmax_enc, W, H);
        }
        EORB_HIP(c, hipEventRecord(E[3], Hs));
        if (G != M) EORB_HIP(c, hipStreamWaitEvent(G, E[2], 0));
        EORB_HIP(c, hipStreamWaitEvent(G, E[1], 0));
        {
            ProfScope ps(c, "ev_gather", G);
            sl_gather_kernel<<<Gt, 64 * nw, lds_g, G>>>(Pg);
        }
        EORB_HIP(c, hipEventRecord(E[4], G));
        EORB_LAUNCH_CHECK(c, "sl_gather_kernel");
    }
    return EORB_OK;
}

int ev_slots_accumulate(eorb_ctx* c, const void* d_events, int stride, const int64_t* h_offsets, int B, int W, int H, int TX, int TY,
                        float* d_f32, uint32_t* d_minmax_enc, const SlotDict* dict)
{
    const int NT = TX * TY;
    const int64_t nev = h_offsets[B] - h_offsets[0];
    static const int rank_env0 = [] { const char* e = getenv("EORB_SLOT_RANK"); return e ? atoi(e) : 1; }();
    const bool rank_allowed = c->sl_rank_ok == 1 && (c->dbg_slot_rank < 0 ? rank_env0 != 0 : c->dbg_slot_rank != 0);
    static const int halves_env = [] { const char* e = getenv("EORB_SLOT_HALVES"); return e ? atoi(e) : -1; }();
    const int halves_opt = c->dbg_slot_halves >= 0 ? c->dbg_slot_halves : halves_env;
    const int nparts = (halves_opt > 0 && B >= 2) ? 2 : 1;
    const int64_t per_slice = nev / B;
    SlotScatterChoice sc;
    if (B > 2048 || (size_t)NT * 4 > 64 * 1024 || !sl_choose_scatter(c, NT, per_slice, rank_allowed, &sc)) return kSlotDeclined;
    for (int b = 0; b < B; b++) {
        const int64_t s = h_offsets[b], e = h_offsets[b + 1];
        if (e < s) return set_err(c, EORB_E_ARG, "ev_accumulate: offsets not monotone");
        if ((e - s) * 4 + (int64_t)NT * 16 >= (int64_t)1 << 31) return set_err(c, EORB_E_CAPACITY, "ev_accumulate: %lld events in one slice", (long long)(e - s));
    }
    int rc;
    if ((rc = sl_streams(c))) return rc;
    c->sl_calls++;
    c->sl_last_rank = sc.rank ? 1 : 0; c->sl_last_chunk = sc.chunk; c->sl_last_parts = nparts;
    const int B0 = nparts == 2 ? B / 2 : B;
    for (int part = 0; part < nparts; part++) {
        const int b0 = part ? B0 : 0, nb_ = part ? B - B0 : B0;
        if ((rc = slots_part(c, c->sl_ws[part], part, nparts, d_events, stride, h_offsets + b0, nb_, W, H, TX, TY,
                             d_f32 + (size_t)b0 * W * H, d_minmax_enc + 2 * (size_t)b0, sc, dict))) return rc;
    }
    hipEvent_t* E = c->sl_ev + 5 * (nparts - 1);
    EORB_HIP(c, hipStreamWaitEvent(c->stream, E[3], 0));
    if (nparts > 1) EORB_HIP(c, hipStreamWaitEvent(c->stream, E[4], 0));
    return EORB_OK;
}

int ev_slots_trace_read(eorb_ctx* c, unsigned long long* out, long long max_records)
{
    const long long n = std::min<long long>(c->sl_trace_n, max_records);
    if (n <= 0 || !c->sl_trace.p) return 0;
    if (hipMemcpy(out, (unsigned long long*)c->sl_trace.p + 8, sizeof(unsigned long long) * 6 * (size_t)n, hipMemcpyDeviceToHost) != hipSuccess) return -1;
    return (int)n;
}

}
```

### eorb_slam_amd/csrc/sl_hot_asm.h

```cpp
#define SL_HOT_NROWS 240
#define SL_HOT_ASM \
    "s_setprio 3\n" \
    "v_mbcnt_lo_u32_b32 v242, -1, 0\n" \
    "v_mbcnt_hi_u32_b32 v242, -1, v242\n" \
    "v_and_b32 v249, 1, v242\n" \
    "v_lshlrev_b32 v249, 7, v249\n" \
    "v_lshlrev_b32 v252, 6, v242\n" \
    "v_and_b32 v243, 7, v242\n" \
    "v_lshrrev_b32 v244, 3, v242\n" \
    "v_lshlrev_b32 v242, 2, v242\n" \
    "v_mov_b32 v246, v243\n" \
    "v_mov_b32 v247, v244\n" \
    "s_load_dwordx16 s[36:51], %[hcnt], 0x0\n" \
    "s_waitcnt lgkmcnt(0)\n" \
    "SLH_ITEM:\n" \
    "v_mov_b32 v245, 1\n" \
    "v_mov_b32 v248, 0\n" \
    "s_mov_b64 s[62:63], exec\n" \
    "s_mov_b64 exec, 1\n" \
    "global_atomic_add v245, v248, v245, %[ticket] sc0\n" \
    "s_waitcnt vmcnt(0)\n" \
    "s_mov_b64 exec, s[62:63]\n" \
    "s_nop 0\n" \
    "v_readfirstlane_b32 s60, v245\n" \
    "s_mov_b32 s61, 0\n" \
    "s_cmp_lt_u32 s60, s36\n" \
    "s_cbranch_scc1 SLH_FOUND\n" \
    "s_sub_u32 s60, s60, s36\n" \
    "s_add_u32 s61, s61, 1\n" \
    "s_cmp_lt_u32 s60, s37\n" \
    "s_cbranch_scc1 SLH_FOUND\n" \
    "s_sub_u32 s60, s60, s37\n" \
    "s_add_u32 s61, s61, 1\n" \
    "s_cmp_lt_u32 s60, s38\n" \
    "s_cbranch_scc1 SLH_FOUND\n" \
    "s_sub_u32 s60, s60, s38\n" \
    "s_add_u32 s61, s61, 1\n" \
    "s_cmp_lt_u32 s60, s39\n" \
    "s_cbranch_scc1 SLH_FOUND\n" \
    "s_sub_u32 s60, s60, s39\n" \
    "s_add_u32 s61, s61, 1\n" \
    "s_cmp_lt_u32 s60, s40\n" \
    "s_cbranch_scc1 SLH_FOUND\n" \
    "s_sub_u32 s60, s60, s40\n" \
    "s_add_u32 s61, s61, 1\n" \
    "s_cmp_lt_u32 s60, s41\n" \
    "s_cbranch_scc1 SLH_FOUND\n" \
    "s_sub_u32 s60, s60, s41\n" \
    "s_add_u32 s61, s61, 1\n" \
    "s_cmp_lt_u32 s60, s42\n" \
    "s_cbranch_scc1 SLH_FOUND\n" \
    "s_sub_u32 s60, s60, s42\n" \
    "s_add_u32 s61, s61, 1\n" \
    "s_cmp_lt_u32 s60, s43\n" \
    "s_cbranch_scc1 SLH_FOUND\n" \
    "s_sub_u32 s60, s60, s43\n" \
    "s_add_u32 s61, s61, 1\n" \
    "s_cmp_lt_u32 s60, s44\n" \
    "s_cbranch_scc1 SLH_FOUND\n" \
    "s_sub_u32 s60, s60, s44\n" \
    "s_add_u32 s61, s61, 1\n" \
    "s_cmp_lt_u32 s60, s45\n" \
    "s_cbranch_scc1 SLH_FOUND\n" \
    "s_sub_u32 s60, s60, s45\n" \
    "s_add_u32 s61, s61, 1\n" \
    "s_cmp_lt_u32 s60, s46\n" \
    "s_cbranch_scc1 SLH_FOUND\n" \
    "s_sub_u32 s60, s60, s46\n" \
    "s_add_u32 s61, s61, 1\n" \
    "s_cmp_lt_u32 s60, s47\n" \
    "s_cbranch_scc1 SLH_FOUND\n" \
    "s_sub_u32 s60, s60, s47\n" \
    "s_add_u32 s61, s61, 1\n" \
    "s_cmp_lt_u32 s60, s48\n" \
    "s_cbranch_scc1 SLH_FOUND\n" \
    "s_sub_u32 s60, s60, s48\n" \
    "s_add_u32 s61, s61, 1\n" \
    "s_cmp_lt_u32 s60, s49\n" \
    "s_cbranch_scc1 SLH_FOUND\n" \
    "s_sub_u32 s60, s60, s49\n" \
    "s_add_u32 s61, s61, 1\n" \
    "s_cmp_lt_u32 s60, s50\n" \
    "s_cbranch_scc1 SLH_FOUND\n" \
    "s_sub_u32 s60, s60, s50\n" \
    "s_add_u32 s61, s61, 1\n" \
    "s_cmp_lt_u32 s60, s51\n" \
    "s_cbranch_scc1 SLH_FOUND\n" \
    "s_sub_u32 s60, s60, s51\n" \
    "s_add_u32 s61, s61, 1\n" \
    "s_branch SLH_DONE\n" \
    "SLH_FOUND:\n" \
    "s_mul_i32 s61, s61, %[hcap]\n" \
    "s_add_u32 s61, s61, s60\n" \
    "s_lshl_b32 s61, s61, 5\n" \
    "s_load_dwordx8 s[52:59], %[items], s61\n" \
    "s_waitcnt lgkmcnt(0)\n" \
    "s_add_u32 s64, %[rows_lo], s59\n" \
    "s_addc_u32 s65, %[rows_hi], 0\n" \
    "global_load_dword v0, v242, s[64:65] offset:0\n" \
    "global_load_dword v1, v242, s[64:65] offset:256\n" \
    "global_load_dword v2, v242, s[64:65] offset:512\n" \
    "global_load_dword v3, v242, s[64:65] offset:768\n" \
    "global_load_dword v4, v242, s[64:65] offset:1024\n" \
    "global_load_dword v5, v242, s[64:65] offset:1280\n" \
    "global_load_dword v6, v242, s[64:65] offset:1536\n" \
    "global_load_dword v7, v242, s[64:65] offset:1792\n" \
    "global_load_dword v8, v242, s[64:65] offset:2048\n" \
    "global_load_dword v9, v242, s[64:65] offset:2304\n" \
    "global_load_dword v10, v242, s[64:65] offset:2560\n" \
    "global_load_dword v11, v242, s[64:65] offset:2816\n" \
    "global_load_dword v12, v242, s[64:65] offset:3072\n" \
    "global_load_dword v13, v242, s[64:65] offset:3328\n" \
    "global_load_dword v14, v242, s[64:65] offset:3584\n" \
    "global_load_dword v15, v242, s[64:65] offset:3840\n" \
    "s_add_u32 s64, s64, 0x1000\n" \
    "s_addc_u32 s65, s65, 0\n" \
    "global_load_dword v16, v242, s[64:65] offset:0\n" \
    "global_load_dword v17, v242, s[64:65] offset:256\n" \
    "global_load_dword v18, v242, s[64:65] offset:512\n" \
    "global_load_dword v19, v242, s[64:65] offset:768\n" \
    "global_load_dword v20, v242, s[64:65] offset:1024\n" \
    "global_load_dword v21, v242, s[64:65] offset:1280\n" \
    "global_load_dword v22, v242, s[64:65] offset:1536\n" \
    "global_load_dword v23, v242, s[64:65] offset:1792\n" \
    "global_load_dword v24, v242, s[64:65] offset:2048\n" \
    "global_load_dword v25, v242, s[64:65] offset:2304\n" \
    "global_load_dword v26, v242, s[64:65] offset:2560\n" \
    "global_load_dword v27, v242, s[64:65] offset:2816\n" \
    "global_load_dword v28, v242, s[64:65] offset:3072\n" \
    "global_load_dword v29, v242, s[64:65] offset:3328\n" \
    "global_load_dword v30, v242, s[64:65] offset:3584\n" \
    "global_load_dword v31, v242, s[64:65] offset:3840\n" \
    "s_add_u32 s64, s64, 0x1000\n" \
    "s_addc_u32 s65, s65, 0\n" \
    "global_load_dword v32, v242, s[64:65] offset:0\n" \
    "global_load_dword v33, v242, s[64:65] offset:256\n" \
    "global_load_dword v34, v242, s[64:65] offset:512\n" \
    "global_load_dword v35, v242, s[64:65] offset:768\n" \
    "global_load_dword v36, v242, s[64:65] offset:1024\n" \
    "global_load_dword v37, v242, s[64:65] offset:1280\n" \
    "global_load_dword v38, v242, s[64:65] offset:1536\n" \
    "global_load_dword v39, v242, s[64:65] offset:1792\n" \
    "global_load_dword v40, v242, s[64:65] offset:2048\n" \
    "global_load_dword v41, v242, s[64:65] offset:2304\n" \
    "global_load_dword v42, v242, s[64:65] offset:2560\n" \
    "global_load_dword v43, v242, s[64:65] offset:2816\n" \
    "global_load_dword v44, v242, s[64:65] offset:3072\n" \
    "global_load_dword v45, v242, s[64:65] offset:3328\n" \
    "global_load_dword v46, v242, s[64:65] offset:3584\n" \
    "global_load_dword v47, v242, s[64:65] offset:3840\n" \
    "s_add_u32 s64, s64, 0x1000\n" \
    "s_addc_u32 s65, s65, 0\n" \
    "global_load_dword v48, v242, s[64:65] offset:0\n" \
    "global_load_dword v49, v242, s[64:65] offset:256\n" \
    "global_load_dword v50, v242, s[64:65] offset:512\n" \
    "global_load_dword v51, v242, s[64:65] offset:768\n" \
    "global_load_dword v52, v242, s[64:65] offset:1024\n" \
    "global_load_dword v53, v242, s[64:65] offset:1280\n" \
    "global_load_dword v54, v242, s[64:65] offset:1536\n" \
    "global_load_dword v55, v242, s[64:65] offset:1792\n" \
    "global_load_dword v56, v242, s[64:65] offset:2048\n" \
    "global_load_dword v57, v242, s[64:65] offset:2304\n" \
    "global_load_dword v58, v242, s[64:65] offset:2560\n" \
    "global_load_dword v59, v242, s[64:65] offset:2816\n" \
    "global_load_dword v60, v242, s[64:65] offset:3072\n" \
    "global_load_dword v61, v242, s[64:65] offset:3328\n" \
    "global_load_dword v62, v242, s[64:65] offset:3584\n" \
    "global_load_dword v63, v242, s[64:65] offset:3840\n" \
    "s_add_u32 s64, s64, 0x1000\n" \
    "s_addc_u32 s65, s65, 0\n" \
    "global_load_dword v64, v242, s[64:65] offset:0\n" \
    "global_load_dword v65, v242, s[64:65] offset:256\n" \
    "global_load_dword v66, v242, s[64:65] offset:512\n" \
    "global_load_dword v67, v242, s[64:65] offset:768\n" \
    "global_load_dword v68, v242, s[64:65] offset:1024\n" \
    "global_load_dword v69, v242, s[64:65] offset:1280\n" \
    "global_load_dword v70, v242, s[64:65] offset:1536\n" \
    "global_load_dword v71, v242, s[64:65] offset:1792\n" \
    "global_load_dword v72, v242, s[64:65] offset:2048\n" \
    "global_load_dword v73, v242, s[64:65] offset:2304\n" \
    "global_load_dword v74, v242, s[64:65] offset:2560\n" \
    "global_load_dword v75, v242, s[64:65] offset:2816\n" \
    "global_load_dword v76, v242, s[64:65] offset:3072\n" \
    "global_load_dword v77, v242, s[64:65] offset:3328\n" \
    "global_load_dword v78, v242, s[64:65] offset:3584\n" \
    "global_load_dword v79, v242, s[64:65] offset:3840\n" \
    "s_add_u32 s64, s64, 0x1000\n" \
    "s_addc_u32 s65, s65, 0\n" \
    "global_load_dword v80, v242, s[64:65] offset:0\n" \
    "global_load_dword v81, v242, s[64:65] offset:256\n" \
    "global_load_dword v82, v242, s[64:65] offset:512\n" \
    "global_load_dword v83, v242, s[64:65] offset:768\n" \
    "global_load_dword v84, v242, s[64:65] offset:1024\n" \
    "global_load_dword v85, v242, s[64:65] offset:1280\n" \
    "global_load_dword v86, v242, s[64:65] offset:1536\n" \
    "global_load_dword v87, v242, s[64:65] offset:1792\n" \
    "global_load_dword v88, v242, s[64:65] offset:2048\n" \
    "global_load_dword v89, v242, s[64:65] offset:2304\n" \
    "global_load_dword v90, v242, s[64:65] offset:2560\n" \
    "global_load_dword v91, v242, s[64:65] offset:2816\n" \
    "global_load_dword v92, v242, s[64:65] offset:3072\n" \
    "global_load_dword v93, v242, s[64:65] offset:3328\n" \
    "global_load_dword v94, v242, s[64:65] offset:3584\n" \
    "global_load_dword v95, v242, s[64:65] offset:3840\n" \
    "s_add_u32 s64, s64, 0x1000\n" \
    "s_addc_u32 s65, s65, 0\n" \
    "global_load_dword v96, v242, s[64:65] offset:0\n" \
    "global_load_dword v97, v242, s[64:65] offset:256\n" \
    "global_load_dword v98, v242, s[64:65] offset:512\n" \
    "global_load_dword v99, v242, s[64:65] offset:768\n" \
    "global_load_dword v100, v242, s[64:65] offset:1024\n" \
    "global_load_dword v101, v242, s[64:65] offset:1280\n" \
    "global_load_dword v102, v242, s[64:65] offset:1536\n" \
    "global_load_dword v103, v242, s[64:65] offset:1792\n" \
    "global_load_dword v104, v242, s[64:65] offset:2048\n" \
    "global_load_dword v105, v242, s[64:65] offset:2304\n" \
    "global_load_dword v106, v242, s[64:65] offset:2560\n" \
    "global_load_dword v107, v242, s[64:65] offset:2816\n" \
    "global_load_dword v108, v242, s[64:65] offset:3072\n" \
    "global_load_dword v109, v242, s[64:65] offset:3328\n" \
    "global_load_dword v110, v242, s[64:65] offset:3584\n" \
    "global_load_dword v111, v242, s[64:65] offset:3840\n" \
    "s_add_u32 s64, s64, 0x1000\n" \
    "s_addc_u32 s65, s65, 0\n" \
    "global_load_dword v112, v242, s[64:65] offset:0\n" \
    "global_load_dword v113, v242, s[64:65] offset:256\n" \
    "global_load_dword v114, v242, s[64:65] offset:512\n" \
    "global_load_dword v115, v242, s[64:65] offset:768\n" \
    "global_load_dword v116, v242, s[64:65] offset:1024\n" \
    "global_load_dword v117, v242, s[64:65] offset:1280\n" \
    "global_load_dword v118, v242, s[64:65] offset:1536\n" \
    "global_load_dword v119, v242, s[64:65] offset:1792\n" \
    "global_load_dword v120, v242, s[64:65] offset:2048\n" \
    "global_load_dword v121, v242, s[64:65] offset:2304\n" \
    "global_load_dword v122, v242, s[64:65] offset:2560\n" \
    "global_load_dword v123, v242, s[64:65] offset:2816\n" \
    "global_load_dword v124, v242, s[64:65] offset:3072\n" \
    "global_load_dword v125, v242, s[64:65] offset:3328\n" \
    "global_load_dword v126, v242, s[64:65] offset:3584\n" \
    "global_load_dword v127, v242, s[64:65] offset:3840\n" \
    "s_add_u32 s64, s64, 0x1000\n" \
    "s_addc_u32 s65, s65, 0\n" \
    "global_load_dword v128, v242, s[64:65] offset:0\n" \
    "global_load_dword v129, v242, s[64:65] offset:256\n" \
    "global_load_dword v130, v242, s[64:65] offset:512\n" \
    "global_load_dword v131, v242, s[64:65] offset:768\n" \
    "global_load_dword v132, v242, s[64:65] offset:1024\n" \
    "global_load_dword v133, v242, s[64:65] offset:1280\n" \
    "global_load_dword v134, v242, s[64:65] offset:1536\n" \
    "global_load_dword v135, v242, s[64:65] offset:1792\n" \
    "global_load_dword v136, v242, s[64:65] offset:2048\n" \
    "global_load_dword v137, v242, s[64:65] offset:2304\n" \
    "global_load_dword v138, v242, s[64:65] offset:2560\n" \
    "global_load_dword v139, v242, s[64:65] offset:2816\n" \
    "global_load_dword v140, v242, s[64:65] offset:3072\n" \
    "global_load_dword v141, v242, s[64:65] offset:3328\n" \
    "global_load_dword v142, v242, s[64:65] offset:3584\n" \
    "global_load_dword v143, v242, s[64:65] offset:3840\n" \
    "s_add_u32 s64, s64, 0x1000\n" \
    "s_addc_u32 s65, s65, 0\n" \
    "global_load_dword v144, v242, s[64:65] offset:0\n" \
    "global_load_dword v145, v242, s[64:65] offset:256\n" \
    "global_load_dword v146, v242, s[64:65] offset:512\n" \
    "global_load_dword v147, v242, s[64:65] offset:768\n" \
    "global_load_dword v148, v242, s[64:65] offset:1024\n" \
    "global_load_dword v149, v242, s[64:65] offset:1280\n" \
    "global_load_dword v150, v242, s[64:65] offset:1536\n" \
    "global_load_dword v151, v242, s[64:65] offset:1792\n" \
    "global_load_dword v152, v242, s[64:65] offset:2048\n" \
    "global_load_dword v153, v242, s[64:65] offset:2304\n" \
    "global_load_dword v154, v242, s[64:65] offset:2560\n" \
    "global_load_dword v155, v242, s[64:65] offset:2816\n" \
    "global_load_dword v156, v242, s[64:65] offset:3072\n" \
    "global_load_dword v157, v242, s[64:65] offset:3328\n" \
    "global_load_dword v158, v242, s[64:65] offset:3584\n" \
    "global_load_dword v159, v242, s[64:65] offset:3840\n" \
    "s_add_u32 s64, s64, 0x1000\n" \
    "s_addc_u32 s65, s65, 0\n" \
    "global_load_dword v160, v242, s[64:65] offset:0\n" \
    "global_load_dword v161, v242, s[64:65] offset:256\n" \
    "global_load_dword v162, v242, s[64:65] offset:512\n" \
    "global_load_dword v163, v242, s[64:65] offset:768\n" \
    "global_load_dword v164, v242, s[64:65] offset:1024\n" \
    "global_load_dword v165, v242, s[64:65] offset:1280\n" \
    "global_load_dword v166, v242, s[64:65] offset:1536\n" \
    "global_load_dword v167, v242, s[64:65] offset:1792\n" \
    "global_load_dword v168, v242, s[64:65] offset:2048\n" \
    "global_load_dword v169, v242, s[64:65] offset:2304\n" \
    "global_load_dword v170, v242, s[64:65] offset:2560\n" \
    "global_load_dword v171, v242, s[64:65] offset:2816\n" \
    "global_load_dword v172, v242, s[64:65] offset:3072\n" \
    "global_load_dword v173, v242, s[64:65] offset:3328\n" \
    "global_load_dword v174, v242, s[64:65] offset:3584\n" \
    "global_load_dword v175, v242, s[64:65] offset:3840\n" \
    "s_add_u32 s64, s64, 0x1000\n" \
    "s_addc_u32 s65, s65, 0\n" \
    "global_load_dword v176, v242, s[64:65] offset:0\n" \
    "global_load_dword v177, v242, s[64:65] offset:256\n" \
    "global_load_dword v178, v242, s[64:65] offset:512\n" \
    "global_load_dword v179, v242, s[64:65] offset:768\n" \
    "global_load_dword v180, v242, s[64:65] offset:1024\n" \
    "global_load_dword v181, v242, s[64:65] offset:1280\n" \
    "global_load_dword v182, v242, s[64:65] offset:1536\n" \
    "global_load_dword v183, v242, s[64:65] offset:1792\n" \
    "global_load_dword v184, v242, s[64:65] offset:2048\n" \
    "global_load_dword v185, v242, s[64:65] offset:2304\n" \
    "global_load_dword v186, v242, s[64:65] offset:2560\n" \
    "global_load_dword v187, v242, s[64:65] offset:2816\n" \
    "global_load_dword v188, v242, s[64:65] offset:3072\n" \
    "global_load_dword v189, v242, s[64:65] offset:3328\n" \
    "global_load_dword v190, v242, s[64:65] offset:3584\n" \
    "global_load_dword v191, v242, s[64:65] offset:3840\n" \
    "s_add_u32 s64, s64, 0x1000\n" \
    "s_addc_u32 s65, s65, 0\n" \
    "global_load_dword v192, v242, s[64:65] offset:0\n" \
    "global_load_dword v193, v242, s[64:65] offset:256\n" \
    "global_load_dword v194, v242, s[64:65] offset:512\n" \
    "global_load_dword v195, v242, s[64:65] offset:768\n" \
    "global_load_dword v196, v242, s[64:65] offset:1024\n" \
    "global_load_dword v197, v242, s[64:65] offset:1280\n" \
    "global_load_dword v198, v242, s[64:65] offset:1536\n" \
    "global_load_dword v199, v242, s[64:65] offset:1792\n" \
    "global_load_dword v200, v242, s[64:65] offset:2048\n" \
    "global_load_dword v201, v242, s[64:65] offset:2304\n" \
    "global_load_dword v202, v242, s[64:65] offset:2560\n" \
    "global_load_dword v203, v242, s[64:65] offset:2816\n" \
    "global_load_dword v204, v242, s[64:65] offset:3072\n" \
    "global_load_dword v205, v242, s[64:65] offset:3328\n" \
    "global_load_dword v206, v242, s[64:65] offset:3584\n" \
    "global_load_dword v207, v242, s[64:65] offset:3840\n" \
    "s_add_u32 s64, s64, 0x1000\n" \
    "s_addc_u32 s65, s65, 0\n" \
    "global_load_dword v208, v242, s[64:65] offset:0\n" \
    "global_load_dword v209, v242, s[64:65] offset:256\n" \
    "global_load_dword v210, v242, s[64:65] offset:512\n" \
    "global_load_dword v211, v242, s[64:65] offset:768\n" \
    "global_load_dword v212, v242, s[64:65] offset:1024\n" \
    "global_load_dword v213, v242, s[64:65] offset:1280\n" \
    "global_load_dword v214, v242, s[64:65] offset:1536\n" \
    "global_load_dword v215, v242, s[64:65] offset:1792\n" \
    "global_load_dword v216, v242, s[64:65] offset:2048\n" \
    "global_load_dword v217, v242, s[64:65] offset:2304\n" \
    "global_load_dword v218, v242, s[64:65] offset:2560\n" \
    "global_load_dword v219, v242, s[64:65] offset:2816\n" \
    "global_load_dword v220, v242, s[64:65] offset:3072\n" \
    "global_load_dword v221, v242, s[64:65] offset:3328\n" \
    "global_load_dword v222, v242, s[64:65] offset:3584\n" \
    "global_load_dword v223, v242, s[64:65] offset:3840\n" \
    "s_add_u32 s64, s64, 0x1000\n" \
    "s_addc_u32 s65, s65, 0\n" \
    "global_load_dword v224, v242, s[64:65] offset:0\n" \
    "global_load_dword v225, v242, s[64:65] offset:256\n" \
    "global_load_dword v226, v242, s[64:65] offset:512\n" \
    "global_load_dword v227, v242, s[64:65] offset:768\n" \
    "global_load_dword v228, v242, s[64:65] offset:1024\n" \
    "global_load_dword v229, v242, s[64:65] offset:1280\n" \
    "global_load_dword v230, v242, s[64:65] offset:1536\n" \
    "global_load_dword v231, v242, s[64:65] offset:1792\n" \
    "global_load_dword v232, v242, s[64:65] offset:2048\n" \
    "global_load_dword v233, v242, s[64:65] offset:2304\n" \
    "global_load_dword v234, v242, s[64:65] offset:2560\n" \
    "global_load_dword v235, v242, s[64:65] offset:2816\n" \
    "global_load_dword v236, v242, s[64:65] offset:3072\n" \
    "global_load_dword v237, v242, s[64:65] offset:3328\n" \
    "global_load_dword v238, v242, s[64:65] offset:3584\n" \
    "global_load_dword v239, v242, s[64:65] offset:3840\n" \
    "s_add_u32 s64, s64, 0x1000\n" \
    "s_addc_u32 s65, s65, 0\n" \
    "v_mov_b32 v240, 0\n" \
    "v_mov_b32 v241, 0\n" \
    "s_add_u32 s100, %[ent_lo], s55\n" \
    "s_addc_u32 s101, %[ent_hi], s56\n" \
    "global_load_dword v250, v252, s[100:101]\n" \
    "v_writelane_b32 v253, s52, 0\n" \
    "v_writelane_b32 v253, s54, 1\n" \
    "v_writelane_b32 v253, s57, 2\n" \
    "v_writelane_b32 v253, s58, 3\n" \
    "s_lshr_b32 s35, s54, 6\n" \
    "s_load_dwordx16 s[36:51], s[100:101], 0x0\n" \
    "s_load_dwordx16 s[52:67], s[100:101], 0x40\n" \
    "s_mov_b32 s34, 0x80\n" \
    "s_mov_b32 s33, 0\n" \
    "s_waitcnt vmcnt(0)\n" \
    "s_set_gpr_idx_on s33, gpr_idx(SRC0)\n" \
    "SLH_LOOP:\n" \
    "v_add_u32 v251, s34, v249\n" \
    "global_load_dword v250, v251, s[100:101] offset:3968\n" \
    "s_sub_u32 s35, s35, 1\n" \
    "s_cbranch_scc1 SLH_TAIL\n" \
    "s_waitcnt lgkmcnt(0)\n" \
    "s_load_dwordx16 s[68:83], s[100:101], s34\n" \
    "s_add_u32 s33, s34, 0x40\n" \
    "s_load_dwordx16 s[84:99], s[100:101], s33\n" \
    "s_add_u32 s34, s34, 0x80\n" \
    "s_mov_b32 m0, s36\n" \
    "v_add_f32 v241, v0, v241\n" \
    "s_lshr_b32 m0, s36, 16\n" \
    "v_add_f32 v241, v0, v241\n" \
    "s_mov_b32 m0, s37\n" \
    "v_add_f32 v241, v0, v241\n" \
    "s_lshr_b32 m0, s37, 16\n" \
    "v_add_f32 v241, v0, v241\n" \
    "s_mov_b32 m0, s38\n" \
    "v_add_f32 v241, v0, v241\n" \
    "s_lshr_b32 m0, s38, 16\n" \
    "v_add_f32 v241, v0, v241\n" \
    "s_mov_b32 m0, s39\n" \
    "v_add_f32 v241, v0, v241\n" \
    "s_lshr_b32 m0, s39, 16\n" \
    "v_add_f32 v241, v0, v241\n" \
    "s_mov_b32 m0, s40\n" \
    "v_add_f32 v241, v0, v241\n" \
    "s_lshr_b32 m0, s40, 16\n" \
    "v_add_f32 v241, v0, v241\n" \
    "s_mov_b32 m0, s41\n" \
    "v_add_f32 v241, v0, v241\n" \
    "s_lshr_b32 m0, s41, 16\n" \
    "v_add_f32 v241, v0, v241\n" \
    "s_mov_b32 m0, s42\n" \
    "v_add_f32 v241, v0, v241\n" \
    "s_lshr_b32 m0, s42, 16\n" \
    "v_add_f32 v241, v0, v241\n" \
    "s_mov_b32 m0, s43\n" \
    "v_add_f32 v241, v0, v241\n" \
    "s_lshr_b32 m0, s43, 16\n" \
    "v_add_f32 v241, v0, v241\n" \
    "s_mov_b32 m0, s44\n" \
    "v_add_f32 v241, v0, v241\n" \
    "s_lshr_b32 m0, s44, 16\n" \
    "v_add_f32 v241, v0, v241\n" \
    "s_mov_b32 m0, s45\n" \
    "v_add_f32 v241, v0, v241\n" \
    "s_lshr_b32 m0, s45, 16\n" \
    "v_add_f32 v241, v0, v241\n" \
    "s_mov_b32 m0, s46\n" \
    "v_add_f32 v241, v0, v241\n" \
    "s_lshr_b32 m0, s46, 16\n" \
    "v_add_f32 v241, v0, v241\n" \
    "s_mov_b32 m0, s47\n" \
    "v_add_f32 v241, v0, v241\n" \
    "s_lshr_b32 m0, s47, 16\n" \
    "v_add_f32 v241, v0, v241\n" \
    "s_mov_b32 m0, s48\n" \
    "v_add_f32 v241, v0, v241\n" \
    "s_lshr_b32 m0, s48, 16\n" \
    "v_add_f32 v241, v0, v241\n" \
    "s_mov_b32 m0, s49\n" \
    "v_add_f32 v241, v0, v241\n" \
    "s_lshr_b32 m0, s49, 16\n" \
    "v_add_f32 v241, v0, v241\n" \
    "s_mov_b32 m0, s50\n" \
    "v_add_f32 v241, v0, v241\n" \
    "s_lshr_b32 m0, s50, 16\n" \
    "v_add_f32 v241, v0, v241\n" \
    "s_mov_b32 m0, s51\n" \
    "v_add_f32 v241, v0, v241\n" \
    "s_lshr_b32 m0, s51, 16\n" \
    "v_add_f32 v241, v0, v241\n" \
    "s_mov_b32 m0, s52\n" \
    "v_add_f32 v241, v0, v241\n" \
    "s_lshr_b32 m0, s52, 16\n" \
    "v_add_f32 v241, v0, v241\n" \
    "s_mov_b32 m0, s53\n" \
    "v_add_f32 v241, v0, v241\n" \
    "s_lshr_b32 m0, s53, 16\n" \
    "v_add_f32 v241, v0, v241\n" \
    "s_mov_b32 m0, s54\n" \
    "v_add_f32 v241, v0, v241\n" \
    "s_lshr_b32 m0, s54, 16\n" \
    "v_add_f32 v241, v0, v241\n" \
    "s_mov_b32 m0, s55\n" \
    "v_add_f32 v241, v0, v241\n" \
    "s_lshr_b32 m0, s55, 16\n" \
    "v_add_f32 v241, v0, v241\n" \
    "s_mov_b32 m0, s56\n" \
    "v_add_f32 v241, v0, v241\n" \
    "s_lshr_b32 m0, s56, 16\n" \
    "v_add_f32 v241, v0, v241\n" \
    "s_mov_b32 m0, s57\n" \
    "v_add_f32 v241, v0, v241\n" \
    "s_lshr_b32 m0, s57, 16\n" \
    "v_add_f32 v241, v0, v241\n" \
    "s_mov_b32 m0, s58\n" \
    "v_add_f32 v241, v0, v241\n" \
    "s_lshr_b32 m0, s58, 16\n" \
    "v_add_f32 v241, v0, v241\n" \
    "s_mov_b32 m0, s59\n" \
    "v_add_f32 v241, v0, v241\n" \
    "s_lshr_b32 m0, s59, 16\n" \
    "v_add_f32 v241, v0, v241\n" \
    "s_mov_b32 m0, s60\n" \
    "v_add_f32 v241, v0, v241\n" \
    "s_lshr_b32 m0, s60, 16\n" \
    "v_add_f32 v241, v0, v241\n" \
    "s_mov_b32 m0, s61\n" \
    "v_add_f32 v241, v0, v241\n" \
    "s_lshr_b32 m0, s61, 16\n" \
    "v_add_f32 v241, v0, v241\n" \
    "s_mov_b32 m0, s62\n" \
    "v_add_f32 v241, v0, v241\n" \
    "s_lshr_b32 m0, s62, 16\n" \
    "v_add_f32 v241, v0, v241\n" \
    "s_mov_b32 m0, s63\n" \
    "v_add_f32 v241, v0, v241\n" \
    "s_lshr_b32 m0, s63, 16\n" \
    "v_add_f32 v241, v0, v241\n" \
    "s_mov_b32 m0, s64\n" \
    "v_add_f32 v241, v0, v241\n" \
    "s_lshr_b32 m0, s64, 16\n" \
    "v_add_f32 v241, v0, v241\n" \
    "s_mov_b32 m0, s65\n" \
    "v_add_f32 v241, v0, v241\n" \
    "s_lshr_b32 m0, s65, 16\n" \
    "v_add_f32 v241, v0, v241\n" \
    "s_mov_b32 m0, s66\n" \
    "v_add_f32 v241, v0, v241\n" \
    "s_lshr_b32 m0, s66, 16\n" \
    "v_add_f32 v241, v0, v241\n" \
    "s_mov_b32 m0, s67\n" \
    "v_add_f32 v241, v0, v241\n" \
    "s_lshr_b32 m0, s67, 16\n" \
    "v_add_f32 v241, v0, v241\n" \
    "s_sub_u32 s35, s35, 1\n" \
    "s_cbranch_scc1 SLH_TAIL\n" \
    "s_waitcnt lgkmcnt(0)\n" \
    "s_load_dwordx16 s[36:51], s[100:101], s34\n" \
    "s_add_u32 s33, s34, 0x40\n" \
    "s_load_dwordx16 s[52:67], s[100:101], s33\n" \
    "s_add_u32 s34, s34, 0x80\n" \
    "s_mov_b32 m0, s68\n" \
    "v_add_f32 v241, v0, v241\n" \
    "s_lshr_b32 m0, s68, 16\n" \
    "v_add_f32 v241, v0, v241\n" \
    "s_mov_b32 m0, s69\n" \
    "v_add_f32 v241, v0, v241\n" \
    "s_lshr_b32 m0, s69, 16\n" \
    "v_add_f32 v241, v0, v241\n" \
    "s_mov_b32 m0, s70\n" \
    "v_add_f32 v241, v0, v241\n" \
    "s_lshr_b32 m0, s70, 16\n" \
    "v_add_f32 v241, v0, v241\n" \
    "s_mov_b32 m0, s71\n" \
    "v_add_f32 v241, v0, v241\n" \
    "s_lshr_b32 m0, s71, 16\n" \
    "v_add_f32 v241, v0, v241\n" \
    "s_mov_b32 m0, s72\n" \
    "v_add_f32 v241, v0, v241\n" \
    "s_lshr_b32 m0, s72, 16\n" \
    "v_add_f32 v241, v0, v241\n" \
    "s_mov_b32 m0, s73\n" \
    "v_add_f32 v241, v0, v241\n" \
    "s_lshr_b32 m0, s73, 16\n" \
    "v_add_f32 v241, v0, v241\n" \
    "s_mov_b32 m0, s74\n" \
    "v_add_f32 v241, v0, v241\n" \
    "s_lshr_b32 m0, s74, 16\n" \
    "v_add_f32 v241, v0, v241\n" \
    "s_mov_b32 m0, s75\n" \
    "v_add_f32 v241, v0, v241\n" \
    "s_lshr_b32 m0, s75, 16\n" \
    "v_add_f32 v241, v0, v241\n" \
    "s_mov_b32 m0, s76\n" \
    "v_add_f32 v241, v0, v241\n" \
    "s_lshr_b32 m0, s76, 16\n" \
    "v_add_f32 v241, v0, v241\n" \
    "s_mov_b32 m0, s77\n" \
    "v_add_f32 v241, v0, v241\n" \
    "s_lshr_b32 m0, s77, 16\n" \
    "v_add_f32 v241, v0, v241\n" \
    "s_mov_b32 m0, s78\n" \
    "v_add_f32 v241, v0, v241\n" \
    "s_lshr_b32 m0, s78, 16\n" \
    "v_add_f32 v241, v0, v241\n" \
    "s_mov_b32 m0, s79\n" \
    "v_add_f32 v241, v0, v241\n" \
    "s_lshr_b32 m0, s79, 16\n" \
    "v_add_f32 v241, v0, v241\n" \
    "s_mov_b32 m0, s80\n" \
    "v_add_f32 v241, v0, v241\n" \
    "s_lshr_b32 m0, s80, 16\n" \
    "v_add_f32 v241, v0, v241\n" \
    "s_mov_b32 m0, s81\n" \
    "v_add_f32 v241, v0, v241\n" \
    "s_lshr_b32 m0, s81, 16\n" \
    "v_add_f32 v241, v0, v241\n" \
    "s_mov_b32 m0, s82\n" \
    "v_add_f32 v241, v0, v241\n" \
    "s_lshr_b32 m0, s82, 16\n" \
    "v_add_f32 v241, v0, v241\n" \
    "s_mov_b32 m0, s83\n" \
    "v_add_f32 v241, v0, v241\n" \
    "s_lshr_b32 m0, s83, 16\n" \
    "v_add_f32 v241, v0, v241\n" \
    "s_mov_b32 m0, s84\n" \
    "v_add_f32 v241, v0, v241\n" \
    "s_lshr_b32 m0, s84, 16\n" \
    "v_add_f32 v241, v0, v241\n" \
    "s_mov_b32 m0, s85\n" \
    "v_add_f32 v241, v0, v241\n" \
    "s_lshr_b32 m0, s85, 16\n" \
    "v_add_f32 v241, v0, v241\n" \
    "s_mov_b32 m0, s86\n" \
    "v_add_f32 v241, v0, v241\n" \
    "s_lshr_b32 m0, s86, 16\n" \
    "v_add_f32 v241, v0, v241\n" \
    "s_mov_b32 m0, s87\n" \
    "v_add_f32 v241, v0, v241\n" \
    "s_lshr_b32 m0, s87, 16\n" \
    "v_add_f32 v241, v0, v241\n" \
    "s_mov_b32 m0, s88\n" \
    "v_add_f32 v241, v0, v241\n" \
    "s_lshr_b32 m0, s88, 16\n" \
    "v_add_f32 v241, v0, v241\n" \
    "s_mov_b32 m0, s89\n" \
    "v_add_f32 v241, v0, v241\n" \
    "s_lshr_b32 m0, s89, 16\n" \
    "v_add_f32 v241, v0, v241\n" \
    "s_mov_b32 m0, s90\n" \
    "v_add_f32 v241, v0, v241\n" \
    "s_lshr_b32 m0, s90, 16\n" \
    "v_add_f32 v241, v0, v241\n" \
    "s_mov_b32 m0, s91\n" \
    "v_add_f32 v241, v0, v241\n" \
    "s_lshr_b32 m0, s91, 16\n" \
    "v_add_f32 v241, v0, v241\n" \
    "s_mov_b32 m0, s92\n" \
    "v_add_f32 v241, v0, v241\n" \
    "s_lshr_b32 m0, s92, 16\n" \
    "v_add_f32 v241, v0, v241\n" \
    "s_mov_b32 m0, s93\n" \
    "v_add_f32 v241, v0, v241\n" \
    "s_lshr_b32 m0, s93, 16\n" \
    "v_add_f32 v241, v0, v241\n" \
    "s_mov_b32 m0, s94\n" \
    "v_add_f32 v241, v0, v241\n" \
    "s_lshr_b32 m0, s94, 16\n" \
    "v_add_f32 v241, v0, v241\n" \
    "s_mov_b32 m0, s95\n" \
    "v_add_f32 v241, v0, v241\n" \
    "s_lshr_b32 m0, s95, 16\n" \
    "v_add_f32 v241, v0, v241\n" \
    "s_mov_b32 m0, s96\n" \
    "v_add_f32 v241, v0, v241\n" \
    "s_lshr_b32 m0, s96, 16\n" \
    "v_add_f32 v241, v0, v241\n" \
    "s_mov_b32 m0, s97\n" \
    "v_add_f32 v241, v0, v241\n" \
    "s_lshr_b32 m0, s97, 16\n" \
    "v_add_f32 v241, v0, v241\n" \
    "s_mov_b32 m0, s98\n" \
    "v_add_f32 v241, v0, v241\n" \
    "s_lshr_b32 m0, s98, 16\n" \
    "v_add_f32 v241, v0, v241\n" \
    "s_mov_b32 m0, s99\n" \
    "v_add_f32 v241, v0, v241\n" \
    "s_lshr_b32 m0, s99, 16\n" \
    "v_add_f32 v241, v0, v241\n" \
    "s_branch SLH_LOOP\n" \
    "SLH_TAIL:\n" \
    "s_waitcnt lgkmcnt(0)\n" \
    "s_set_gpr_idx_off\n" \
    "v_readlane_b32 s33, v253, 1\n" \
    "s_and_b32 s35, s33, 63\n" \
    "s_cmp_eq_u32 s35, 0\n" \
    "s_cbranch_scc1 SLH_STORE\n" \
    "s_add_u32 s34, s33, 1\n" \
    "s_and_b32 s34, s34, -2\n" \
    "s_lshl_b32 s34, s34, 1\n" \
    "s_add_u32 s100, s100, s34\n" \
    "s_addc_u32 s101, s101, 0\n" \
    "s_sub_u32 s100, s100, 0x80\n" \
    "s_subb_u32 s101, s101, 0\n" \
    "s_load_dwordx16 s[36:51], s[100:101], 0x0\n" \
    "s_load_dwordx16 s[52:67], s[100:101], 0x40\n" \
    "s_waitcnt lgkmcnt(0)\n" \
    "s_bitcmp1_b32 s33, 0\n" \
    "s_cbranch_scc0 SLH_TAILGO\n" \
    "s_and_b32 s67, s67, 0xffff\n" \
    "s_or_b32 s67, s67, 0x10f00000\n" \
    "SLH_TAILGO:\n" \
    "s_add_u32 s33, s35, 1\n" \
    "s_lshr_b32 s33, s33, 1\n" \
    "s_sub_u32 s33, 32, s33\n" \
    "s_mul_i32 s33, s33, 16\n" \
    "s_mov_b32 s34, 0\n" \
    "s_set_gpr_idx_on s34, gpr_idx(SRC0)\n" \
    "s_getpc_b64 s[34:35]\n" \
    "s_add_u32 s34, s34, s33\n" \
    "s_addc_u32 s35, s35, 0\n" \
    "s_add_u32 s34, s34, 20\n" \
    "s_addc_u32 s35, s35, 0\n" \
    "s_setpc_b64 s[34:35]\n" \
    "s_mov_b32 m0, s36\n" \
    "v_add_f32 v241, v0, v241\n" \
    "s_lshr_b32 m0, s36, 16\n" \
    "v_add_f32 v241, v0, v241\n" \
    "s_mov_b32 m0, s37\n" \
    "v_add_f32 v241, v0, v241\n" \
    "s_lshr_b32 m0, s37, 16\n" \
    "v_add_f32 v241, v0, v241\n" \
    "s_mov_b32 m0, s38\n" \
    "v_add_f32 v241, v0, v241\n" \
    "s_lshr_b32 m0, s38, 16\n" \
    "v_add_f32 v241, v0, v241\n" \
    "s_mov_b32 m0, s39\n" \
    "v_add_f32 v241, v0, v241\n" \
    "s_lshr_b32 m0, s39, 16\n" \
    "v_add_f32 v241, v0, v241\n" \
    "s_mov_b32 m0, s40\n" \
    "v_add_f32 v241, v0, v241\n" \
    "s_lshr_b32 m0, s40, 16\n" \
    "v_add_f32 v241, v0, v241\n" \
    "s_mov_b32 m0, s41\n" \
    "v_add_f32 v241, v0, v241\n" \
    "s_lshr_b32 m0, s41, 16\n" \
    "v_add_f32 v241, v0, v241\n" \
    "s_mov_b32 m0, s42\n" \
    "v_add_f32 v241, v0, v241\n" \
    "s_lshr_b32 m0, s42, 16\n" \
    "v_add_f32 v241, v0, v241\n" \
    "s_mov_b32 m0, s43\n" \
    "v_add_f32 v241, v0, v241\n" \
    "s_lshr_b32 m0, s43, 16\n" \
    "v_add_f32 v241, v0, v241\n" \
    "s_mov_b32 m0, s44\n" \
    "v_add_f32 v241, v0, v241\n" \
    "s_lshr_b32 m0, s44, 16\n" \
    "v_add_f32 v241, v0, v241\n" \
    "s_mov_b32 m0, s45\n" \
    "v_add_f32 v241, v0, v241\n" \
    "s_lshr_b32 m0, s45, 16\n" \
    "v_add_f32 v241, v0, v241\n" \
    "s_mov_b32 m0, s46\n" \
    "v_add_f32 v241, v0, v241\n" \
    "s_lshr_b32 m0, s46, 16\n" \
    "v_add_f32 v241, v0, v241\n" \
    "s_mov_b32 m0, s47\n" \
    "v_add_f32 v241, v0, v241\n" \
    "s_lshr_b32 m0, s47, 16\n" \
    "v_add_f32 v241, v0, v241\n" \
    "s_mov_b32 m0, s48\n" \
    "v_add_f32 v241, v0, v241\n" \
    "s_lshr_b32 m0, s48, 16\n" \
    "v_add_f32 v241, v0, v241\n" \
    "s_mov_b32 m0, s49\n" \
    "v_add_f32 v241, v0, v241\n" \
    "s_lshr_b32 m0, s49, 16\n" \
    "v_add_f32 v241, v0, v241\n" \
    "s_mov_b32 m0, s50\n" \
    "v_add_f32 v241, v0, v241\n" \
    "s_lshr_b32 m0, s50, 16\n" \
    "v_add_f32 v241, v0, v241\n" \
    "s_mov_b32 m0, s51\n" \
    "v_add_f32 v241, v0, v241\n" \
    "s_lshr_b32 m0, s51, 16\n" \
    "v_add_f32 v241, v0, v241\n" \
    "s_mov_b32 m0, s52\n" \
    "v_add_f32 v241, v0, v241\n" \
    "s_lshr_b32 m0, s52, 16\n" \
    "v_add_f32 v241, v0, v241\n" \
    "s_mov_b32 m0, s53\n" \
    "v_add_f32 v241, v0, v241\n" \
    "s_lshr_b32 m0, s53, 16\n" \
    "v_add_f32 v241, v0, v241\n" \
    "s_mov_b32 m0, s54\n" \
    "v_add_f32 v241, v0, v241\n" \
    "s_lshr_b32 m0, s54, 16\n" \
    "v_add_f32 v241, v0, v241\n" \
    "s_mov_b32 m0, s55\n" \
    "v_add_f32 v241, v0, v241\n" \
    "s_lshr_b32 m0, s55, 16\n" \
    "v_add_f32 v241, v0, v241\n" \
    "s_mov_b32 m0, s56\n" \
    "v_add_f32 v241, v0, v241\n" \
    "s_lshr_b32 m0, s56, 16\n" \
    "v_add_f32 v241, v0, v241\n" \
    "s_mov_b32 m0, s57\n" \
    "v_add_f32 v241, v0, v241\n" \
    "s_lshr_b32 m0, s57, 16\n" \
    "v_add_f32 v241, v0, v241\n" \
    "s_mov_b32 m0, s58\n" \
    "v_add_f32 v241, v0, v241\n" \
    "s_lshr_b32 m0, s58, 16\n" \
    "v_add_f32 v241, v0, v241\n" \
    "s_mov_b32 m0, s59\n" \
    "v_add_f32 v241, v0, v241\n" \
    "s_lshr_b32 m0, s59, 16\n" \
    "v_add_f32 v241, v0, v241\n" \
    "s_mov_b32 m0, s60\n" \
    "v_add_f32 v241, v0, v241\n" \
    "s_lshr_b32 m0, s60, 16\n" \
    "v_add_f32 v241, v0, v241\n" \
    "s_mov_b32 m0, s61\n" \
    "v_add_f32 v241, v0, v241\n" \
    "s_lshr_b32 m0, s61, 16\n" \
    "v_add_f32 v241, v0, v241\n" \
    "s_mov_b32 m0, s62\n" \
    "v_add_f32 v241, v0, v241\n" \
    "s_lshr_b32 m0, s62, 16\n" \
    "v_add_f32 v241, v0, v241\n" \
    "s_mov_b32 m0, s63\n" \
    "v_add_f32 v241, v0, v241\n" \
    "s_lshr_b32 m0, s63, 16\n" \
    "v_add_f32 v241, v0, v241\n" \
    "s_mov_b32 m0, s64\n" \
    "v_add_f32 v241, v0, v241\n" \
    "s_lshr_b32 m0, s64, 16\n" \
    "v_add_f32 v241, v0, v241\n" \
    "s_mov_b32 m0, s65\n" \
    "v_add_f32 v241, v0, v241\n" \
    "s_lshr_b32 m0, s65, 16\n" \
    "v_add_f32 v241, v0, v241\n" \
    "s_mov_b32 m0, s66\n" \
    "v_add_f32 v241, v0, v241\n" \
    "s_lshr_b32 m0, s66, 16\n" \
    "v_add_f32 v241, v0, v241\n" \
    "s_mov_b32 m0, s67\n" \
    "v_add_f32 v241, v0, v241\n" \
    "s_lshr_b32 m0, s67, 16\n" \
    "v_add_f32 v241, v0, v241\n" \
    "SLH_STORE:\n" \
    "s_set_gpr_idx_off\n" \
    "v_readlane_b32 s52, v253, 0\n" \
    "v_readlane_b32 s57, v253, 2\n" \
    "v_readlane_b32 s58, v253, 3\n" \
    "v_add_u32 v243, s57, v246\n" \
    "v_add_u32 v244, s58, v247\n" \
    "v_cmp_gt_u32 vcc, %[W], v243\n" \
    "v_cmp_gt_u32 s[34:35], %[H], v244\n" \
    "s_and_b64 s[34:35], s[34:35], vcc\n" \
    "v_mul_lo_u32 v245, v244, %[W]\n" \
    "v_add_u32 v245, v245, v243\n" \
    "v_lshlrev_b32 v245, 2, v245\n" \
    "s_mul_i32 s33, %[W], %[H]\n" \
    "s_mul_i32 s33, s33, s52\n" \
    "s_mul_hi_u32 s60, s33, 4\n" \
    "s_lshl_b32 s33, s33, 2\n" \
    "s_add_u32 s64, %[img_lo], s33\n" \
    "s_addc_u32 s65, %[img_hi], s60\n" \
    "s_mov_b64 s[62:63], exec\n" \
    "s_and_b64 exec, exec, s[34:35]\n" \
    "global_store_dword v245, v241, s[64:65]\n" \
    "s_mov_b64 exec, s[62:63]\n" \
    "v_mov_b32 v248, v241\n" \
    "s_nop 1\n" \
    "v_max_f32_dpp v248, v248, v248 row_shr:1 row_mask:0xf bank_mask:0xf bound_ctrl:0\n" \
    "s_nop 1\n" \
    "v_max_f32_dpp v248, v248, v248 row_shr:2 row_mask:0xf bank_mask:0xf bound_ctrl:0\n" \
    "s_nop 1\n" \
    "v_max_f32_dpp v248, v248, v248 row_shr:4 row_mask:0xf bank_mask:0xf bound_ctrl:0\n" \
    "s_nop 1\n" \
    "v_max_f32_dpp v248, v248, v248 row_shr:8 row_mask:0xf bank_mask:0xf bound_ctrl:0\n" \
    "s_nop 1\n" \
    "v_max_f32_dpp v248, v248, v248 row_bcast:15 row_mask:0xa bank_mask:0xf\n" \
    "s_nop 1\n" \
    "v_max_f32_dpp v248, v248, v248 row_bcast:31 row_mask:0xc bank_mask:0xf\n" \
    "s_nop 1\n" \
    "v_readlane_b32 s33, v248, 63\n" \
    "s_or_b32 s33, s33, 0x80000000\n" \
    "s_lshl_b32 s34, s52, 3\n" \
    "s_add_u32 s34, s34, 4\n" \
    "v_mov_b32 v245, s34\n" \
    "v_mov_b32 v248, s33\n" \
    "s_mov_b64 s[62:63], exec\n" \
    "s_mov_b64 exec, 1\n" \
    "global_atomic_umax v245, v248, %[mm]\n" \
    "s_mov_b64 exec, s[62:63]\n" \
    "s_load_dwordx16 s[36:51], %[hcnt], 0x0\n" \
    "s_waitcnt vmcnt(0) lgkmcnt(0)\n" \
    "s_branch SLH_ITEM\n" \
    "SLH_DONE:\n" \
    ""
#define SL_HOT_CLOBBERS "v0", "v1", "v2", "v3", "v4", "v5", "v6", "v7", "v8", "v9", "v10", "v11", "v12", "v13", "v14", "v15", "v16", "v17", "v18", "v19", "v20", "v21", "v22", "v23", "v24", "v25", "v26", "v27", "v28", "v29", "v30", "v31", "v32", "v33", "v34", "v35", "v36", "v37", "v38", "v39", "v40", "v41", "v42", "v43", "v44", "v45", "v46", "v47", "v48", "v49", "v50", "v51", "v52", "v53", "v54", "v55", "v56", "v57", "v58", "v59", "v60", "v61", "v62", "v63", "v64", "v65", "v66", "v67", "v68", "v69", "v70", "v71", "v72", "v73", "v74", "v75", "v76", "v77", "v78", "v79", "v80", "v81", "v82", "v83", "v84", "v85", "v86", "v87", "v88", "v89", "v90", "v91", "v92", "v93", "v94", "v95", "v96", "v97", "v98", "v99", "v100", "v101", "v102", "v103", "v104", "v105", "v106", "v107", "v108", "v109", "v110", "v111", "v112", "v113", "v114", "v115", "v116", "v117", "v118", "v119", "v120", "v121", "v122", "v123", "v124", "v125", "v126", "v127", "v128", "v129", "v130", "v131", "v132", "v133", "v134", "v135", "v136", "v137", "v138", "v139", "v140", "v141", "v142", "v143", "v144", "v145", "v146", "v147", "v148", "v149", "v150", "v151", "v152", "v153", "v154", "v155", "v156", "v157", "v158", "v159", "v160", "v161", "v162", "v163", "v164", "v165", "v166", "v167", "v168", "v169", "v170", "v171", "v172", "v173", "v174", "v175", "v176", "v177", "v178", "v179", "v180", "v181", "v182", "v183", "v184", "v185", "v186", "v187", "v188", "v189", "v190", "v191", "v192", "v193", "v194", "v195", "v196", "v197", "v198", "v199", "v200", "v201", "v202", "v203", "v204", "v205", "v206", "v207", "v208", "v209", "v210", "v211", "v212", "v213", "v214", "v215", "v216", "v217", "v218", "v219", "v220", "v221", "v222", "v223", "v224", "v225", "v226", "v227", "v228", "v229", "v230", "v231", "v232", "v233", "v234", "v235", "v236", "v237", "v238", "v239", "v240", "v241", "v242", "v243", "v244", "v245", "v246", "v247", "v248", "v249", "v250", "v251", "v252", "v253", "v254", "v255", "s33", "s34", "s35", "s36", "s37", "s38", "s39", "s40", "s41", "s42", "s43", "s44", "s45", "s46", "s47", "s48", "s49", "s50", "s51", "s52", "s53", "s54", "s55", "s56", "s57", "s58", "s59", "s60", "s61", "s62", "s63", "s64", "s65", "s66", "s67", "s68", "s69", "s70", "s71", "s72", "s73", "s74", "s75", "s76", "s77", "s78", "s79", "s80", "s81", "s82", "s83", "s84", "s85", "s86", "s87", "s88", "s89", "s90", "s91", "s92", "s93", "s94", "s95", "s96", "s97", "s98", "s99", "s100", "s101", "vcc", "scc", "m0", "memory"
```

Before: 47210 frames/s.

## Triple-buffer scalar entry loads in hot accumulate asm kernel via kernarg pointer

The hand-written hot-tile accumulation kernel now reads its arguments straight from the kernarg segment. This frees SGPRs s4-s35, which become a third 128-byte scalar load buffer, so entry lists are prefetched further ahead. The vector prefetch of entries is widened to six lanes with fixed offsets, and per-iteration address arithmetic is dropped. In exchange it adds register spills through lane writes, more over-read beyond the last list (checked with static asserts against the buffer slack), and a larger code footprint.

```diff
diff --git a/eorb_slam_amd/csrc/ev_slots.hip b/eorb_slam_amd/csrc/ev_slots.hip
--- a/eorb_slam_amd/csrc/ev_slots.hip
+++ b/eorb_slam_amd/csrc/ev_slots.hip
@@ -996,17 +996,21 @@
 #endif
 }
 
-__global__ __launch_bounds__(64) void sl_hot_kernel(const uint32_t* __restrict__ hcnt, uint32_t* __restrict__ ticket, const HotDesc* __restrict__ items,
-                                                    int hcap, const float* __restrict__ rows, const slot_entry* __restrict__ entries,
-                                                    float* __restrict__ img, uint32_t* __restrict__ mm, int W, int H)
-{
-    const uint32_t rows_lo = (uint32_t)(uintptr_t)rows, rows_hi = (uint32_t)((uintptr_t)rows >> 32);
-    const uint32_t ent_lo = (uint32_t)(uintptr_t)entries, ent_hi = (uint32_t)((uintptr_t)entries >> 32);
-    const uint32_t img_lo = (uint32_t)(uintptr_t)img, img_hi = (uint32_t)((uintptr_t)img >> 32);
+struct HotArgs {
+    const uint32_t* hcnt; uint32_t* ticket; const HotDesc* items; int hcap; int pad;
+    const float* rows; const slot_entry* entries; float* img; uint32_t* mm; int W, H;
+};
+static_assert(offsetof(HotArgs, hcnt) == SL_HOT_KA_HCNT && offsetof(HotArgs, ticket) == SL_HOT_KA_TICKET && offsetof(HotArgs, items) == SL_HOT_KA_ITEMS &&
+              offsetof(HotArgs, hcap) == SL_HOT_KA_HCAP && offsetof(HotArgs, rows) == SL_HOT_KA_ROWS && offsetof(HotArgs, entries) == SL_HOT_KA_ENTRIES &&
+              offsetof(HotArgs, img) == SL_HOT_KA_IMG && offsetof(HotArgs, mm) == SL_HOT_KA_MM && offsetof(HotArgs, W) == SL_HOT_KA_W &&
+              offsetof(HotArgs, H) == SL_HOT_KA_H, "tools/gen_sl_hot.py: KA");
+constexpr size_t kEntrySlack = 8192;
+static_assert(kEntrySlack >= SL_HOT_OVERREAD_PREFETCH && kEntrySlack >= SL_HOT_OVERREAD_SCALAR, "ws.entries: slack behind the last list");
+__global__ __launch_bounds__(64) void sl_hot_kernel(HotArgs A)
+{
     asm volatile(SL_HOT_ASM
                  :
-                 : [hcnt] "s"(hcnt), [ticket] "s"(ticket), [items] "s"(items), [hcap] "s"(hcap), [rows_lo] "s"(rows_lo), [rows_hi] "s"(rows_hi),
-                   [ent_lo] "s"(ent_lo), [ent_hi] "s"(ent_hi), [img_lo] "s"(img_lo), [img_hi] "s"(img_hi), [mm] "s"(mm), [W] "s"(W), [H] "s"(H)
+                 : [ka] "s"(__builtin_amdgcn_kernarg_segment_ptr())
                  : SL_HOT_CLOBBERS);
 }
 
@@ -1171,7 +1175,7 @@
     if ((rc = ensure(c, ws.chunks, cd_bytes + sc_bytes + eb_bytes))) return rc;
     const size_t cnt_bytes = (sizeof(uint16_t) * (size_t)std::max(nchunks, 1) * NT + 15) & ~(size_t)15;
     if ((rc = ensure(c, ws.segoff, cnt_bytes + sizeof(uint32_t) * (size_t)std::max(nchunks, 1) * NT))) return rc;
-    if ((rc = ensure(c, ws.entries, sizeof(slot_entry) * (size_t)eb + 8192))) return rc;
+    if ((rc = ensure(c, ws.entries, sizeof(slot_entry) * (size_t)eb + kEntrySlack))) return rc;
     if ((rc = ensure(c, ws.tile_order, sizeof(uint32_t) * 2 * (size_t)nb))) return rc;
     if (on_dev) {
         SliceOffsets so;
@@ -1338,8 +1342,8 @@
             const int hw = c->dbg_slot_hot_waves > 0 ? c->dbg_slot_hot_waves : (hw_env > 0 ? hw_env : 8 * ncu);
             EORB_HIP(c, hipStreamWaitEvent(Hs, E[2], 0));
             EORB_HIP(c, hipStreamWaitEvent(Hs, E[1], 0));
-            sl_hot_kernel<<<hw, 64, 0, Hs>>>(d_hot_cnt, d_hot_cnt + 32, d_hot_items, kHotCap, (const float*)c->sl_rows.p, (const slot_entry*)ws.entries.p,
-                                             d_f32, d_minmax_enc, W, H);
+            sl_hot_kernel<<<hw, 64, 0, Hs>>>(HotArgs{d_hot_cnt, d_hot_cnt + 32, d_hot_items, kHotCap, 0, (const float*)c->sl_rows.p, (const slot_entry*)ws.entries.p,
+                                                     d_f32, d_minmax_enc, W, H});
         }
         EORB_HIP(c, hipEventRecord(E[3], Hs));
         if (G != M) EORB_HIP(c, hipStreamWaitEvent(G, E[2], 0));
diff --git a/eorb_slam_amd/csrc/sl_hot_asm.h b/eorb_slam_amd/csrc/sl_hot_asm.h
--- a/eorb_slam_amd/csrc/sl_hot_asm.h
+++ b/eorb_slam_amd/csrc/sl_hot_asm.h
@@ -1,9 +1,23 @@
 #define SL_HOT_NROWS 240
+#define SL_HOT_NBUF 3
+#define SL_HOT_BUFDW 32
+#define SL_HOT_OVERREAD_SCALAR 384
+#define SL_HOT_OVERREAD_PREFETCH 4992
+#define SL_HOT_KA_HCNT 0
+#define SL_HOT_KA_TICKET 8
+#define SL_HOT_KA_ITEMS 16
+#define SL_HOT_KA_HCAP 24
+#define SL_HOT_KA_ROWS 32
+#define SL_HOT_KA_ENTRIES 40
+#define SL_HOT_KA_IMG 48
+#define SL_HOT_KA_MM 56
+#define SL_HOT_KA_W 64
+#define SL_HOT_KA_H 68
 #define SL_HOT_ASM \
     "s_setprio 3\n" \
     "v_mbcnt_lo_u32_b32 v242, -1, 0\n" \
     "v_mbcnt_hi_u32_b32 v242, -1, v242\n" \
-    "v_and_b32 v249, 1, v242\n" \
+    "v_min_u32 v249, 5, v242\n" \
     "v_lshlrev_b32 v249, 7, v249\n" \
     "v_lshlrev_b32 v252, 6, v242\n" \
     "v_and_b32 v243, 7, v242\n" \
@@ -11,18 +25,21 @@
     "v_lshlrev_b32 v242, 2, v242\n" \
     "v_mov_b32 v246, v243\n" \
     "v_mov_b32 v247, v244\n" \
-    "s_load_dwordx16 s[36:51], %[hcnt], 0x0\n" \
-    "s_waitcnt lgkmcnt(0)\n" \
     "SLH_ITEM:\n" \
+    "s_load_dwordx16 s[4:19], %[ka], 0x0\n" \
+    "s_load_dwordx2 s[20:21], %[ka], 0x40\n" \
     "v_mov_b32 v245, 1\n" \
     "v_mov_b32 v248, 0\n" \
+    "s_waitcnt lgkmcnt(0)\n" \
+    "s_load_dwordx16 s[36:51], s[4:5], 0x0\n" \
     "s_mov_b64 s[62:63], exec\n" \
     "s_mov_b64 exec, 1\n" \
-    "global_atomic_add v245, v248, v245, %[ticket] sc0\n" \
+    "global_atomic_add v245, v248, v245, s[6:7] sc0\n" \
     "s_waitcnt vmcnt(0)\n" \
     "s_mov_b64 exec, s[62:63]\n" \
     "s_nop 0\n" \
     "v_readfirstlane_b32 s60, v245\n" \
+    "s_waitcnt lgkmcnt(0)\n" \
     "s_mov_b32 s61, 0\n" \
     "s_cmp_lt_u32 s60, s36\n" \
     "s_cbranch_scc1 SLH_FOUND\n" \
@@ -90,13 +107,13 @@
     "s_add_u32 s61, s61, 1\n" \
     "s_branch SLH_DONE\n" \
     "SLH_FOUND:\n" \
-    "s_mul_i32 s61, s61, %[hcap]\n" \
+    "s_mul_i32 s61, s61, s10\n" \
     "s_add_u32 s61, s61, s60\n" \
     "s_lshl_b32 s61, s61, 5\n" \
-    "s_load_dwordx8 s[52:59], %[items], s61\n" \
+    "s_load_dwordx8 s[52:59], s[8:9], s61\n" \
     "s_waitcnt lgkmcnt(0)\n" \
-    "s_add_u32 s64, %[rows_lo], s59\n" \
-    "s_addc_u32 s65, %[rows_hi], 0\n" \
+    "s_add_u32 s64, s12, s59\n" \
+    "s_addc_u32 s65, s13, 0\n" \
     "global_load_dword v0, v242, s[64:65] offset:0\n" \
     "global_load_dword v1, v242, s[64:65] offset:256\n" \
     "global_load_dword v2, v242, s[64:65] offset:512\n" \
@@ -369,30 +386,170 @@
     "s_addc_u32 s65, s65, 0\n" \
     "v_mov_b32 v240, 0\n" \
     "v_mov_b32 v241, 0\n" \
-    "s_add_u32 s100, %[ent_lo], s55\n" \
-    "s_addc_u32 s101, %[ent_hi], s56\n" \
+    "s_add_u32 s100, s14, s55\n" \
+    "s_addc_u32 s101, s15, s56\n" \
     "global_load_dword v250, v252, s[100:101]\n" \
     "v_writelane_b32 v253, s52, 0\n" \
     "v_writelane_b32 v253, s54, 1\n" \
     "v_writelane_b32 v253, s57, 2\n" \
     "v_writelane_b32 v253, s58, 3\n" \
-    "s_lshr_b32 s35, s54, 6\n" \
-    "s_load_dwordx16 s[36:51], s[100:101], 0x0\n" \
-    "s_load_dwordx16 s[52:67], s[100:101], 0x40\n" \
-    "s_mov_b32 s34, 0x80\n" \
-    "s_mov_b32 s33, 0\n" \
+    "v_writelane_b32 v253, s100, 4\n" \
+    "v_writelane_b32 v253, s101, 5\n" \
+    "v_writelane_b32 v253, s20, 6\n" \
+    "v_writelane_b32 v253, s21, 7\n" \
+    "v_writelane_b32 v253, s16, 8\n" \
+    "v_writelane_b32 v253, s17, 9\n" \
+    "v_writelane_b32 v253, s18, 10\n" \
+    "v_writelane_b32 v253, s19, 11\n" \
+    "s_lshr_b32 vcc_lo, s54, 6\n" \
+    "s_load_dwordx16 s[4:19], s[100:101], 0x0\n" \
+    "s_load_dwordx16 s[20:35], s[100:101], 0x40\n" \
+    "s_load_dwordx16 s[36:51], s[100:101], 0x80\n" \
+    "s_load_dwordx16 s[52:67], s[100:101], 0xc0\n" \
+    "s_add_u32 s100, s100, 0x100\n" \
+    "s_addc_u32 s101, s101, 0\n" \
+    "s_mov_b32 vcc_hi, 0\n" \
     "s_waitcnt vmcnt(0)\n" \
-    "s_set_gpr_idx_on s33, gpr_idx(SRC0)\n" \
+    "s_set_gpr_idx_on vcc_hi, gpr_idx(SRC0)\n" \
     "SLH_LOOP:\n" \
-    "v_add_u32 v251, s34, v249\n" \
-    "global_load_dword v250, v251, s[100:101] offset:3968\n" \
-    "s_sub_u32 s35, s35, 1\n" \
+    "global_load_dword v250, v249, s[100:101] offset:3840\n" \
+    "s_sub_u32 vcc_lo, vcc_lo, 1\n" \
     "s_cbranch_scc1 SLH_TAIL\n" \
     "s_waitcnt lgkmcnt(0)\n" \
-    "s_load_dwordx16 s[68:83], s[100:101], s34\n" \
-    "s_add_u32 s33, s34, 0x40\n" \
-    "s_load_dwordx16 s[84:99], s[100:101], s33\n" \
-    "s_add_u32 s34, s34, 0x80\n" \
+    "s_load_dwordx16 s[68:83], s[100:101], 0x0\n" \
+    "s_load_dwordx16 s[84:99], s[100:101], 0x40\n" \
+    "s_mov_b32 m0, s4\n" \
+    "v_add_f32 v241, v0, v241\n" \
+    "s_lshr_b32 m0, s4, 16\n" \
+    "v_add_f32 v241, v0, v241\n" \
+    "s_mov_b32 m0, s5\n" \
+    "v_add_f32 v241, v0, v241\n" \
+    "s_lshr_b32 m0, s5, 16\n" \
+    "v_add_f32 v241, v0, v241\n" \
+    "s_mov_b32 m0, s6\n" \
+    "v_add_f32 v241, v0, v241\n" \
+    "s_lshr_b32 m0, s6, 16\n" \
+    "v_add_f32 v241, v0, v241\n" \
+    "s_mov_b32 m0, s7\n" \
+    "v_add_f32 v241, v0, v241\n" \
+    "s_lshr_b32 m0, s7, 16\n" \
+    "v_add_f32 v241, v0, v241\n" \
+    "s_mov_b32 m0, s8\n" \
+    "v_add_f32 v241, v0, v241\n" \
+    "s_lshr_b32 m0, s8, 16\n" \
+    "v_add_f32 v241, v0, v241\n" \
+    "s_mov_b32 m0, s9\n" \
+    "v_add_f32 v241, v0, v241\n" \
+    "s_lshr_b32 m0, s9, 16\n" \
+    "v_add_f32 v241, v0, v241\n" \
+    "s_mov_b32 m0, s10\n" \
+    "v_add_f32 v241, v0, v241\n" \
+    "s_lshr_b32 m0, s10, 16\n" \
+    "v_add_f32 v241, v0, v241\n" \
+    "s_mov_b32 m0, s11\n" \
+    "v_add_f32 v241, v0, v241\n" \
+    "s_lshr_b32 m0, s11, 16\n" \
+    "v_add_f32 v241, v0, v241\n" \
+    "s_mov_b32 m0, s12\n" \
+    "v_add_f32 v241, v0, v241\n" \
+    "s_lshr_b32 m0, s12, 16\n" \
+    "v_add_f32 v241, v0, v241\n" \
+    "s_mov_b32 m0, s13\n" \
+    "v_add_f32 v241, v0, v241\n" \
+    "s_lshr_b32 m0, s13, 16\n" \
+    "v_add_f32 v241, v0, v241\n" \
+    "s_mov_b32 m0, s14\n" \
+    "v_add_f32 v241, v0, v241\n" \
+    "s_lshr_b32 m0, s14, 16\n" \
+    "v_add_f32 v241, v0, v241\n" \
+    "s_mov_b32 m0, s15\n" \
+    "v_add_f32 v241, v0, v241\n" \
+    "s_lshr_b32 m0, s15, 16\n" \
+    "v_add_f32 v241, v0, v241\n" \
+    "s_mov_b32 m0, s16\n" \
+    "v_add_f32 v241, v0, v241\n" \
+    "s_lshr_b32 m0, s16, 16\n" \
+    "v_add_f32 v241, v0, v241\n" \
+    "s_mov_b32 m0, s17\n" \
+    "v_add_f32 v241, v0, v241\n" \
+    "s_lshr_b32 m0, s17, 16\n" \
+    "v_add_f32 v241, v0, v241\n" \
+    "s_mov_b32 m0, s18\n" \
+    "v_add_f32 v241, v0, v241\n" \
+    "s_lshr_b32 m0, s18, 16\n" \
+    "v_add_f32 v241, v0, v241\n" \
+    "s_mov_b32 m0, s19\n" \
+    "v_add_f32 v241, v0, v241\n" \
+    "s_lshr_b32 m0, s19, 16\n" \
+    "v_add_f32 v241, v0, v241\n" \
+    "s_mov_b32 m0, s20\n" \
+    "v_add_f32 v241, v0, v241\n" \
+    "s_lshr_b32 m0, s20, 16\n" \
+    "v_add_f32 v241, v0, v241\n" \
+    "s_mov_b32 m0, s21\n" \
+    "v_add_f32 v241, v0, v241\n" \
+    "s_lshr_b32 m0, s21, 16\n" \
+    "v_add_f32 v241, v0, v241\n" \
+    "s_mov_b32 m0, s22\n" \
+    "v_add_f32 v241, v0, v241\n" \
+    "s_lshr_b32 m0, s22, 16\n" \
+    "v_add_f32 v241, v0, v241\n" \
+    "s_mov_b32 m0, s23\n" \
+    "v_add_f32 v241, v0, v241\n" \
+    "s_lshr_b32 m0, s23, 16\n" \
+    "v_add_f32 v241, v0, v241\n" \
+    "s_mov_b32 m0, s24\n" \
+    "v_add_f32 v241, v0, v241\n" \
+    "s_lshr_b32 m0, s24, 16\n" \
+    "v_add_f32 v241, v0, v241\n" \
+    "s_mov_b32 m0, s25\n" \
+    "v_add_f32 v241, v0, v241\n" \
+    "s_lshr_b32 m0, s25, 16\n" \
+    "v_add_f32 v241, v0, v241\n" \
+    "s_mov_b32 m0, s26\n" \
+    "v_add_f32 v241, v0, v241\n" \
+    "s_lshr_b32 m0, s26, 16\n" \
+    "v_add_f32 v241, v0, v241\n" \
+    "s_mov_b32 m0, s27\n" \
+    "v_add_f32 v241, v0, v241\n" \
+    "s_lshr_b32 m0, s27, 16\n" \
+    "v_add_f32 v241, v0, v241\n" \
+    "s_mov_b32 m0, s28\n" \
+    "v_add_f32 v241, v0, v241\n" \
+    "s_lshr_b32 m0, s28, 16\n" \
+    "v_add_f32 v241, v0, v241\n" \
+    "s_mov_b32 m0, s29\n" \
+    "v_add_f32 v241, v0, v241\n" \
+    "s_lshr_b32 m0, s29, 16\n" \
+    "v_add_f32 v241, v0, v241\n" \
+    "s_mov_b32 m0, s30\n" \
+    "v_add_f32 v241, v0, v241\n" \
+    "s_lshr_b32 m0, s30, 16\n" \
+    "v_add_f32 v241, v0, v241\n" \
+    "s_mov_b32 m0, s31\n" \
+    "v_add_f32 v241, v0, v241\n" \
+    "s_lshr_b32 m0, s31, 16\n" \
+    "v_add_f32 v241, v0, v241\n" \
+    "s_mov_b32 m0, s32\n" \
+    "v_add_f32 v241, v0, v241\n" \
+    "s_lshr_b32 m0, s32, 16\n" \
+    "v_add_f32 v241, v0, v241\n" \
+    "s_mov_b32 m0, s33\n" \
+    "v_add_f32 v241, v0, v241\n" \
+    "s_lshr_b32 m0, s33, 16\n" \
+    "v_add_f32 v241, v0, v241\n" \
+    "s_mov_b32 m0, s34\n" \
+    "v_add_f32 v241, v0, v241\n" \
+    "s_lshr_b32 m0, s34, 16\n" \
+    "v_add_f32 v241, v0, v241\n" \
+    "s_mov_b32 m0, s35\n" \
+    "v_add_f32 v241, v0, v241\n" \
+    "s_lshr_b32 m0, s35, 16\n" \
+    "v_add_f32 v241, v0, v241\n" \
+    "s_sub_u32 vcc_lo, vcc_lo, 1\n" \
+    "s_cbranch_scc1 SLH_TAIL\n" \
+    "s_load_dwordx16 s[4:19], s[100:101], 0x80\n" \
+    "s_load_dwordx16 s[20:35], s[100:101], 0xc0\n" \
     "s_mov_b32 m0, s36\n" \
     "v_add_f32 v241, v0, v241\n" \
     "s_lshr_b32 m0, s36, 16\n" \
@@ -521,13 +678,11 @@
     "v_add_f32 v241, v0, v241\n" \
     "s_lshr_b32 m0, s67, 16\n" \
     "v_add_f32 v241, v0, v241\n" \
-    "s_sub_u32 s35, s35, 1\n" \
+    "s_sub_u32 vcc_lo, vcc_lo, 1\n" \
     "s_cbranch_scc1 SLH_TAIL\n" \
     "s_waitcnt lgkmcnt(0)\n" \
-    "s_load_dwordx16 s[36:51], s[100:101], s34\n" \
-    "s_add_u32 s33, s34, 0x40\n" \
-    "s_load_dwordx16 s[52:67], s[100:101], s33\n" \
-    "s_add_u32 s34, s34, 0x80\n" \
+    "s_load_dwordx16 s[36:51], s[100:101], 0x100\n" \
+    "s_load_dwordx16 s[52:67], s[100:101], 0x140\n" \
     "s_mov_b32 m0, s68\n" \
     "v_add_f32 v241, v0, v241\n" \
     "s_lshr_b32 m0, s68, 16\n" \
@@ -656,35 +811,436 @@
     "v_add_f32 v241, v0, v241\n" \
     "s_lshr_b32 m0, s99, 16\n" \
     "v_add_f32 v241, v0, v241\n" \
+    "s_sub_u32 vcc_lo, vcc_lo, 1\n" \
+    "s_cbranch_scc1 SLH_TAIL\n" \
+    "s_load_dwordx16 s[68:83], s[100:101], 0x180\n" \
+    "s_load_dwordx16 s[84:99], s[100:101], 0x1c0\n" \
+    "s_mov_b32 m0, s4\n" \
+    "v_add_f32 v241, v0, v241\n" \
+    "s_lshr_b32 m0, s4, 16\n" \
+    "v_add_f32 v241, v0, v241\n" \
+    "s_mov_b32 m0, s5\n" \
+    "v_add_f32 v241, v0, v241\n" \
+    "s_lshr_b32 m0, s5, 16\n" \
+    "v_add_f32 v241, v0, v241\n" \
+    "s_mov_b32 m0, s6\n" \
+    "v_add_f32 v241, v0, v241\n" \
+    "s_lshr_b32 m0, s6, 16\n" \
+    "v_add_f32 v241, v0, v241\n" \
+    "s_mov_b32 m0, s7\n" \
+    "v_add_f32 v241, v0, v241\n" \
+    "s_lshr_b32 m0, s7, 16\n" \
+    "v_add_f32 v241, v0, v241\n" \
+    "s_mov_b32 m0, s8\n" \
+    "v_add_f32 v241, v0, v241\n" \
+    "s_lshr_b32 m0, s8, 16\n" \
+    "v_add_f32 v241, v0, v241\n" \
+    "s_mov_b32 m0, s9\n" \
+    "v_add_f32 v241, v0, v241\n" \
+    "s_lshr_b32 m0, s9, 16\n" \
+    "v_add_f32 v241, v0, v241\n" \
+    "s_mov_b32 m0, s10\n" \
+    "v_add_f32 v241, v0, v241\n" \
+    "s_lshr_b32 m0, s10, 16\n" \
+    "v_add_f32 v241, v0, v241\n" \
+    "s_mov_b32 m0, s11\n" \
+    "v_add_f32 v241, v0, v241\n" \
+    "s_lshr_b32 m0, s11, 16\n" \
+    "v_add_f32 v241, v0, v241\n" \
+    "s_mov_b32 m0, s12\n" \
+    "v_add_f32 v241, v0, v241\n" \
+    "s_lshr_b32 m0, s12, 16\n" \
+    "v_add_f32 v241, v0, v241\n" \
+    "s_mov_b32 m0, s13\n" \
+    "v_add_f32 v241, v0, v241\n" \
+    "s_lshr_b32 m0, s13, 16\n" \
+    "v_add_f32 v241, v0, v241\n" \
+    "s_mov_b32 m0, s14\n" \
+    "v_add_f32 v241, v0, v241\n" \
+    "s_lshr_b32 m0, s14, 16\n" \
+    "v_add_f32 v241, v0, v241\n" \
+    "s_mov_b32 m0, s15\n" \
+    "v_add_f32 v241, v0, v241\n" \
+    "s_lshr_b32 m0, s15, 16\n" \
+    "v_add_f32 v241, v0, v241\n" \
+    "s_mov_b32 m0, s16\n" \
+    "v_add_f32 v241, v0, v241\n" \
+    "s_lshr_b32 m0, s16, 16\n" \
+    "v_add_f32 v241, v0, v241\n" \
+    "s_mov_b32 m0, s17\n" \
+    "v_add_f32 v241, v0, v241\n" \
+    "s_lshr_b32 m0, s17, 16\n" \
+    "v_add_f32 v241, v0, v241\n" \
+    "s_mov_b32 m0, s18\n" \
+    "v_add_f32 v241, v0, v241\n" \
+    "s_lshr_b32 m0, s18, 16\n" \
+    "v_add_f32 v241, v0, v241\n" \
+    "s_mov_b32 m0, s19\n" \
+    "v_add_f32 v241, v0, v241\n" \
+    "s_lshr_b32 m0, s19, 16\n" \
+    "v_add_f32 v241, v0, v241\n" \
+    "s_mov_b32 m0, s20\n" \
+    "v_add_f32 v241, v0, v241\n" \
+    "s_lshr_b32 m0, s20, 16\n" \
+    "v_add_f32 v241, v0, v241\n" \
+    "s_mov_b32 m0, s21\n" \
+    "v_add_f32 v241, v0, v241\n" \
+    "s_lshr_b32 m0, s21, 16\n" \
+    "v_add_f32 v241, v0, v241\n" \
+    "s_mov_b32 m0, s22\n" \
+    "v_add_f32 v241, v0, v241\n" \
+    "s_lshr_b32 m0, s22, 16\n" \
+    "v_add_f32 v241, v0, v241\n" \
+    "s_mov_b32 m0, s23\n" \
+    "v_add_f32 v241, v0, v241\n" \
+    "s_lshr_b32 m0, s23, 16\n" \
+    "v_add_f32 v241, v0, v241\n" \
+    "s_mov_b32 m0, s24\n" \
+    "v_add_f32 v241, v0, v241\n" \
+    "s_lshr_b32 m0, s24, 16\n" \
+    "v_add_f32 v241, v0, v241\n" \
+    "s_mov_b32 m0, s25\n" \
+    "v_add_f32 v241, v0, v241\n" \
+    "s_lshr_b32 m0, s25, 16\n" \
+    "v_add_f32 v241, v0, v241\n" \
+    "s_mov_b32 m0, s26\n" \
+    "v_add_f32 v241, v0, v241\n" \
+    "s_lshr_b32 m0, s26, 16\n" \
+    "v_add_f32 v241, v0, v241\n" \
+    "s_mov_b32 m0, s27\n" \
+    "v_add_f32 v241, v0, v241\n" \
+    "s_lshr_b32 m0, s27, 16\n" \
+    "v_add_f32 v241, v0, v241\n" \
+    "s_mov_b32 m0, s28\n" \
+    "v_add_f32 v241, v0, v241\n" \
+    "s_lshr_b32 m0, s28, 16\n" \
+    "v_add_f32 v241, v0, v241\n" \
+    "s_mov_b32 m0, s29\n" \
+    "v_add_f32 v241, v0, v241\n" \
+    "s_lshr_b32 m0, s29, 16\n" \
+    "v_add_f32 v241, v0, v241\n" \
+    "s_mov_b32 m0, s30\n" \
+    "v_add_f32 v241, v0, v241\n" \
+    "s_lshr_b32 m0, s30, 16\n" \
+    "v_add_f32 v241, v0, v241\n" \
+    "s_mov_b32 m0, s31\n" \
+    "v_add_f32 v241, v0, v241\n" \
+    "s_lshr_b32 m0, s31, 16\n" \
+    "v_add_f32 v241, v0, v241\n" \
+    "s_mov_b32 m0, s32\n" \
+    "v_add_f32 v241, v0, v241\n" \
+    "s_lshr_b32 m0, s32, 16\n" \
+    "v_add_f32 v241, v0, v241\n" \
+    "s_mov_b32 m0, s33\n" \
+    "v_add_f32 v241, v0, v241\n" \
+    "s_lshr_b32 m0, s33, 16\n" \
+    "v_add_f32 v241, v0, v241\n" \
+    "s_mov_b32 m0, s34\n" \
+    "v_add_f32 v241, v0, v241\n" \
+    "s_lshr_b32 m0, s34, 16\n" \
+    "v_add_f32 v241, v0, v241\n" \
+    "s_mov_b32 m0, s35\n" \
+    "v_add_f32 v241, v0, v241\n" \
+    "s_lshr_b32 m0, s35, 16\n" \
+    "v_add_f32 v241, v0, v241\n" \
+    "s_sub_u32 vcc_lo, vcc_lo, 1\n" \
+    "s_cbranch_scc1 SLH_TAIL\n" \
+    "s_waitcnt lgkmcnt(0)\n" \
+    "s_load_dwordx16 s[4:19], s[100:101], 0x200\n" \
+    "s_load_dwordx16 s[20:35], s[100:101], 0x240\n" \
+    "s_mov_b32 m0, s36\n" \
+    "v_add_f32 v241, v0, v241\n" \
+    "s_lshr_b32 m0, s36, 16\n" \
+    "v_add_f32 v241, v0, v241\n" \
+    "s_mov_b32 m0, s37\n" \
+    "v_add_f32 v241, v0, v241\n" \
+    "s_lshr_b32 m0, s37, 16\n" \
+    "v_add_f32 v241, v0, v241\n" \
+    "s_mov_b32 m0, s38\n" \
+    "v_add_f32 v241, v0, v241\n" \
+    "s_lshr_b32 m0, s38, 16\n" \
+    "v_add_f32 v241, v0, v241\n" \
+    "s_mov_b32 m0, s39\n" \
+    "v_add_f32 v241, v0, v241\n" \
+    "s_lshr_b32 m0, s39, 16\n" \
+    "v_add_f32 v241, v0, v241\n" \
+    "s_mov_b32 m0, s40\n" \
+    "v_add_f32 v241, v0, v241\n" \
+    "s_lshr_b32 m0, s40, 16\n" \
+    "v_add_f32 v241, v0, v241\n" \
+    "s_mov_b32 m0, s41\n" \
+    "v_add_f32 v241, v0, v241\n" \
+    "s_lshr_b32 m0, s41, 16\n" \
+    "v_add_f32 v241, v0, v241\n" \
+    "s_mov_b32 m0, s42\n" \
+    "v_add_f32 v241, v0, v241\n" \
+    "s_lshr_b32 m0, s42, 16\n" \
+    "v_add_f32 v241, v0, v241\n" \
+    "s_mov_b32 m0, s43\n" \
+    "v_add_f32 v241, v0, v241\n" \
+    "s_lshr_b32 m0, s43, 16\n" \
+    "v_add_f32 v241, v0, v241\n" \
+    "s_mov_b32 m0, s44\n" \
+    "v_add_f32 v241, v0, v241\n" \
+    "s_lshr_b32 m0, s44, 16\n" \
+    "v_add_f32 v241, v0, v241\n" \
+    "s_mov_b32 m0, s45\n" \
+    "v_add_f32 v241, v0, v241\n" \
+    "s_lshr_b32 m0, s45, 16\n" \
+    "v_add_f32 v241, v0, v241\n" \
+    "s_mov_b32 m0, s46\n" \
+    "v_add_f32 v241, v0, v241\n" \
+    "s_lshr_b32 m0, s46, 16\n" \
+    "v_add_f32 v241, v0, v241\n" \
+    "s_mov_b32 m0, s47\n" \
+    "v_add_f32 v241, v0, v241\n" \
+    "s_lshr_b32 m0, s47, 16\n" \
+    "v_add_f32 v241, v0, v241\n" \
+    "s_mov_b32 m0, s48\n" \
+    "v_add_f32 v241, v0, v241\n" \
+    "s_lshr_b32 m0, s48, 16\n" \
+    "v_add_f32 v241, v0, v241\n" \
+    "s_mov_b32 m0, s49\n" \
+    "v_add_f32 v241, v0, v241\n" \
+    "s_lshr_b32 m0, s49, 16\n" \
+    "v_add_f32 v241, v0, v241\n" \
+    "s_mov_b32 m0, s50\n" \
+    "v_add_f32 v241, v0, v241\n" \
+    "s_lshr_b32 m0, s50, 16\n" \
+    "v_add_f32 v241, v0, v241\n" \
+    "s_mov_b32 m0, s51\n" \
+    "v_add_f32 v241, v0, v241\n" \
+    "s_lshr_b32 m0, s51, 16\n" \
+    "v_add_f32 v241, v0, v241\n" \
+    "s_mov_b32 m0, s52\n" \
+    "v_add_f32 v241, v0, v241\n" \
+    "s_lshr_b32 m0, s52, 16\n" \
+    "v_add_f32 v241, v0, v241\n" \
+    "s_mov_b32 m0, s53\n" \
+    "v_add_f32 v241, v0, v241\n" \
+    "s_lshr_b32 m0, s53, 16\n" \
+    "v_add_f32 v241, v0, v241\n" \
+    "s_mov_b32 m0, s54\n" \
+    "v_add_f32 v241, v0, v241\n" \
+    "s_lshr_b32 m0, s54, 16\n" \
+    "v_add_f32 v241, v0, v241\n" \
+    "s_mov_b32 m0, s55\n" \
+    "v_add_f32 v241, v0, v241\n" \
+    "s_lshr_b32 m0, s55, 16\n" \
+    "v_add_f32 v241, v0, v241\n" \
+    "s_mov_b32 m0, s56\n" \
+    "v_add_f32 v241, v0, v241\n" \
+    "s_lshr_b32 m0, s56, 16\n" \
+    "v_add_f32 v241, v0, v241\n" \
+    "s_mov_b32 m0, s57\n" \
+    "v_add_f32 v241, v0, v241\n" \
+    "s_lshr_b32 m0, s57, 16\n" \
+    "v_add_f32 v241, v0, v241\n" \
+    "s_mov_b32 m0, s58\n" \
+    "v_add_f32 v241, v0, v241\n" \
+    "s_lshr_b32 m0, s58, 16\n" \
+    "v_add_f32 v241, v0, v241\n" \
+    "s_mov_b32 m0, s59\n" \
+    "v_add_f32 v241, v0, v241\n" \
+    "s_lshr_b32 m0, s59, 16\n" \
+    "v_add_f32 v241, v0, v241\n" \
+    "s_mov_b32 m0, s60\n" \
+    "v_add_f32 v241, v0, v241\n" \
+    "s_lshr_b32 m0, s60, 16\n" \
+    "v_add_f32 v241, v0, v241\n" \
+    "s_mov_b32 m0, s61\n" \
+    "v_add_f32 v241, v0, v241\n" \
+    "s_lshr_b32 m0, s61, 16\n" \
+    "v_add_f32 v241, v0, v241\n" \
+    "s_mov_b32 m0, s62\n" \
+    "v_add_f32 v241, v0, v241\n" \
+    "s_lshr_b32 m0, s62, 16\n" \
+    "v_add_f32 v241, v0, v241\n" \
+    "s_mov_b32 m0, s63\n" \
+    "v_add_f32 v241, v0, v241\n" \
+    "s_lshr_b32 m0, s63, 16\n" \
+    "v_add_f32 v241, v0, v241\n" \
+    "s_mov_b32 m0, s64\n" \
+    "v_add_f32 v241, v0, v241\n" \
+    "s_lshr_b32 m0, s64, 16\n" \
+    "v_add_f32 v241, v0, v241\n" \
+    "s_mov_b32 m0, s65\n" \
+    "v_add_f32 v241, v0, v241\n" \
+    "s_lshr_b32 m0, s65, 16\n" \
+    "v_add_f32 v241, v0, v241\n" \
+    "s_mov_b32 m0, s66\n" \
+    "v_add_f32 v241, v0, v241\n" \
+    "s_lshr_b32 m0, s66, 16\n" \
+    "v_add_f32 v241, v0, v241\n" \
+    "s_mov_b32 m0, s67\n" \
+    "v_add_f32 v241, v0, v241\n" \
+    "s_lshr_b32 m0, s67, 16\n" \
+    "v_add_f32 v241, v0, v241\n" \
+    "s_sub_u32 vcc_lo, vcc_lo, 1\n" \
+    "s_cbranch_scc1 SLH_TAIL\n" \
+    "s_load_dwordx16 s[36:51], s[100:101], 0x280\n" \
+    "s_load_dwordx16 s[52:67], s[100:101], 0x2c0\n" \
+    "s_mov_b32 m0, s68\n" \
+    "v_add_f32 v241, v0, v241\n" \
+    "s_lshr_b32 m0, s68, 16\n" \
+    "v_add_f32 v241, v0, v241\n" \
+    "s_mov_b32 m0, s69\n" \
+    "v_add_f32 v241, v0, v241\n" \
+    "s_lshr_b32 m0, s69, 16\n" \
+    "v_add_f32 v241, v0, v241\n" \
+    "s_mov_b32 m0, s70\n" \
+    "v_add_f32 v241, v0, v241\n" \
+    "s_lshr_b32 m0, s70, 16\n" \
+    "v_add_f32 v241, v0, v241\n" \
+    "s_mov_b32 m0, s71\n" \
+    "v_add_f32 v241, v0, v241\n" \
+    "s_lshr_b32 m0, s71, 16\n" \
+    "v_add_f32 v241, v0, v241\n" \
+    "s_mov_b32 m0, s72\n" \
+    "v_add_f32 v241, v0, v241\n" \
+    "s_lshr_b32 m0, s72, 16\n" \
+    "v_add_f32 v241, v0, v241\n" \
+    "s_mov_b32 m0, s73\n" \
+    "v_add_f32 v241, v0, v241\n" \
+    "s_lshr_b32 m0, s73, 16\n" \
+    "v_add_f32 v241, v0, v241\n" \
+    "s_mov_b32 m0, s74\n" \
+    "v_add_f32 v241, v0, v241\n" \
+    "s_lshr_b32 m0, s74, 16\n" \
+    "v_add_f32 v241, v0, v241\n" \
+    "s_mov_b32 m0, s75\n" \
+    "v_add_f32 v241, v0, v241\n" \
+    "s_lshr_b32 m0, s75, 16\n" \
+    "v_add_f32 v241, v0, v241\n" \
+    "s_mov_b32 m0, s76\n" \
+    "v_add_f32 v241, v0, v241\n" \
+    "s_lshr_b32 m0, s76, 16\n" \
+    "v_add_f32 v241, v0, v241\n" \
+    "s_mov_b32 m0, s77\n" \
+    "v_add_f32 v241, v0, v241\n" \
+    "s_lshr_b32 m0, s77, 16\n" \
+    "v_add_f32 v241, v0, v241\n" \
+    "s_mov_b32 m0, s78\n" \
+    "v_add_f32 v241, v0, v241\n" \
+    "s_lshr_b32 m0, s78, 16\n" \
+    "v_add_f32 v241, v0, v241\n" \
+    "s_mov_b32 m0, s79\n" \
+    "v_add_f32 v241, v0, v241\n" \
+    "s_lshr_b32 m0, s79, 16\n" \
+    "v_add_f32 v241, v0, v241\n" \
+    "s_mov_b32 m0, s80\n" \
+    "v_add_f32 v241, v0, v241\n" \
+    "s_lshr_b32 m0, s80, 16\n" \
+    "v_add_f32 v241, v0, v241\n" \
+    "s_mov_b32 m0, s81\n" \
+    "v_add_f32 v241, v0, v241\n" \
+    "s_lshr_b32 m0, s81, 16\n" \
+    "v_add_f32 v241, v0, v241\n" \
+    "s_mov_b32 m0, s82\n" \
+    "v_add_f32 v241, v0, v241\n" \
+    "s_lshr_b32 m0, s82, 16\n" \
+    "v_add_f32 v241, v0, v241\n" \
+    "s_mov_b32 m0, s83\n" \
+    "v_add_f32 v241, v0, v241\n" \
+    "s_lshr_b32 m0, s83, 16\n" \
+    "v_add_f32 v241, v0, v241\n" \
+    "s_mov_b32 m0, s84\n" \
+    "v_add_f32 v241, v0, v241\n" \
+    "s_lshr_b32 m0, s84, 16\n" \
+    "v_add_f32 v241, v0, v241\n" \
+    "s_mov_b32 m0, s85\n" \
+    "v_add_f32 v241, v0, v241\n" \
+    "s_lshr_b32 m0, s85, 16\n" \
+    "v_add_f32 v241, v0, v241\n" \
+    "s_mov_b32 m0, s86\n" \
+    "v_add_f32 v241, v0, v241\n" \
+    "s_lshr_b32 m0, s86, 16\n" \
+    "v_add_f32 v241, v0, v241\n" \
+    "s_mov_b32 m0, s87\n" \
+    "v_add_f32 v241, v0, v241\n" \
+    "s_lshr_b32 m0, s87, 16\n" \
+    "v_add_f32 v241, v0, v241\n" \
+    "s_mov_b32 m0, s88\n" \
+    "v_add_f32 v241, v0, v241\n" \
+    "s_lshr_b32 m0, s88, 16\n" \
+    "v_add_f32 v241, v0, v241\n" \
+    "s_mov_b32 m0, s89\n" \
+    "v_add_f32 v241, v0, v241\n" \
+    "s_lshr_b32 m0, s89, 16\n" \
+    "v_add_f32 v241, v0, v241\n" \
+    "s_mov_b32 m0, s90\n" \
+    "v_add_f32 v241, v0, v241\n" \
+    "s_lshr_b32 m0, s90, 16\n" \
+    "v_add_f32 v241, v0, v241\n" \
+    "s_mov_b32 m0, s91\n" \
+    "v_add_f32 v241, v0, v241\n" \
+    "s_lshr_b32 m0, s91, 16\n" \
+    "v_add_f32 v241, v0, v241\n" \
+    "s_mov_b32 m0, s92\n" \
+    "v_add_f32 v241, v0, v241\n" \
+    "s_lshr_b32 m0, s92, 16\n" \
+    "v_add_f32 v241, v0, v241\n" \
+    "s_mov_b32 m0, s93\n" \
+    "v_add_f32 v241, v0, v241\n" \
+    "s_lshr_b32 m0, s93, 16\n" \
+    "v_add_f32 v241, v0, v241\n" \
+    "s_mov_b32 m0, s94\n" \
+    "v_add_f32 v241, v0, v241\n" \
+    "s_lshr_b32 m0, s94, 16\n" \
+    "v_add_f32 v241, v0, v241\n" \
+    "s_mov_b32 m0, s95\n" \
+    "v_add_f32 v241, v0, v241\n" \
+    "s_lshr_b32 m0, s95, 16\n" \
+    "v_add_f32 v241, v0, v241\n" \
+    "s_mov_b32 m0, s96\n" \
+    "v_add_f32 v241, v0, v241\n" \
+    "s_lshr_b32 m0, s96, 16\n" \
+    "v_add_f32 v241, v0, v241\n" \
+    "s_mov_b32 m0, s97\n" \
+    "v_add_f32 v241, v0, v241\n" \
+    "s_lshr_b32 m0, s97, 16\n" \
+    "v_add_f32 v241, v0, v241\n" \
+    "s_mov_b32 m0, s98\n" \
+    "v_add_f32 v241, v0, v241\n" \
+    "s_lshr_b32 m0, s98, 16\n" \
+    "v_add_f32 v241, v0, v241\n" \
+    "s_mov_b32 m0, s99\n" \
+    "v_add_f32 v241, v0, v241\n" \
+    "s_lshr_b32 m0, s99, 16\n" \
+    "v_add_f32 v241, v0, v241\n" \
+    "s_add_u32 s100, s100, 0x300\n" \
+    "s_addc_u32 s101, s101, 0\n" \
     "s_branch SLH_LOOP\n" \
     "SLH_TAIL:\n" \
     "s_waitcnt lgkmcnt(0)\n" \
     "s_set_gpr_idx_off\n" \
-    "v_readlane_b32 s33, v253, 1\n" \
-    "s_and_b32 s35, s33, 63\n" \
-    "s_cmp_eq_u32 s35, 0\n" \
+    "v_readlane_b32 vcc_hi, v253, 1\n" \
+    "s_and_b32 s33, vcc_hi, 63\n" \
+    "s_cmp_eq_u32 s33, 0\n" \
     "s_cbranch_scc1 SLH_STORE\n" \
-    "s_add_u32 s34, s33, 1\n" \
-    "s_and_b32 s34, s34, -2\n" \
-    "s_lshl_b32 s34, s34, 1\n" \
-    "s_add_u32 s100, s100, s34\n" \
+    "v_readlane_b32 s100, v253, 4\n" \
+    "v_readlane_b32 s101, v253, 5\n" \
+    "s_add_u32 s32, vcc_hi, 1\n" \
+    "s_and_b32 s32, s32, -2\n" \
+    "s_lshl_b32 s32, s32, 1\n" \
+    "s_add_u32 s100, s100, s32\n" \
     "s_addc_u32 s101, s101, 0\n" \
     "s_sub_u32 s100, s100, 0x80\n" \
     "s_subb_u32 s101, s101, 0\n" \
     "s_load_dwordx16 s[36:51], s[100:101], 0x0\n" \
     "s_load_dwordx16 s[52:67], s[100:101], 0x40\n" \
     "s_waitcnt lgkmcnt(0)\n" \
-    "s_bitcmp1_b32 s33, 0\n" \
+    "s_bitcmp1_b32 vcc_hi, 0\n" \
     "s_cbranch_scc0 SLH_TAILGO\n" \
     "s_and_b32 s67, s67, 0xffff\n" \
     "s_or_b32 s67, s67, 0x10f00000\n" \
     "SLH_TAILGO:\n" \
-    "s_add_u32 s33, s35, 1\n" \
+    "s_add_u32 s33, s33, 1\n" \
     "s_lshr_b32 s33, s33, 1\n" \
     "s_sub_u32 s33, 32, s33\n" \
     "s_mul_i32 s33, s33, 16\n" \
-    "s_mov_b32 s34, 0\n" \
-    "s_set_gpr_idx_on s34, gpr_idx(SRC0)\n" \
+    "s_mov_b32 s32, 0\n" \
+    "s_set_gpr_idx_on s32, gpr_idx(SRC0)\n" \
     "s_getpc_b64 s[34:35]\n" \
     "s_add_u32 s34, s34, s33\n" \
     "s_addc_u32 s35, s35, 0\n" \
@@ -824,22 +1380,28 @@
     "v_readlane_b32 s52, v253, 0\n" \
     "v_readlane_b32 s57, v253, 2\n" \
     "v_readlane_b32 s58, v253, 3\n" \
+    "v_readlane_b32 s20, v253, 6\n" \
+    "v_readlane_b32 s21, v253, 7\n" \
+    "v_readlane_b32 s16, v253, 8\n" \
+    "v_readlane_b32 s17, v253, 9\n" \
+    "v_readlane_b32 s18, v253, 10\n" \
+    "v_readlane_b32 s19, v253, 11\n" \
     "v_add_u32 v243, s57, v246\n" \
     "v_add_u32 v244, s58, v247\n" \
-    "v_cmp_gt_u32 vcc, %[W], v243\n" \
-    "v_cmp_gt_u32 s[34:35], %[H], v244\n" \
-    "s_and_b64 s[34:35], s[34:35], vcc\n" \
-    "v_mul_lo_u32 v245, v244, %[W]\n" \
+    "v_cmp_gt_u32 vcc, s20, v243\n" \
+    "v_cmp_gt_u32 s[24:25], s21, v244\n" \
+    "s_and_b64 s[24:25], s[24:25], vcc\n" \
+    "v_mul_lo_u32 v245, v244, s20\n" \
     "v_add_u32 v245, v245, v243\n" \
     "v_lshlrev_b32 v245, 2, v245\n" \
-    "s_mul_i32 s33, %[W], %[H]\n" \
-    "s_mul_i32 s33, s33, s52\n" \
-    "s_mul_hi_u32 s60, s33, 4\n" \
-    "s_lshl_b32 s33, s33, 2\n" \
-    "s_add_u32 s64, %[img_lo], s33\n" \
-    "s_addc_u32 s65, %[img_hi], s60\n" \
+    "s_mul_i32 s22, s20, s21\n" \
+    "s_mul_i32 s22, s22, s52\n" \
+    "s_mul_hi_u32 s60, s22, 4\n" \
+    "s_lshl_b32 s22, s22, 2\n" \
+    "s_add_u32 s64, s16, s22\n" \
+    "s_addc_u32 s65, s17, s60\n" \
     "s_mov_b64 s[62:63], exec\n" \
-    "s_and_b64 exec, exec, s[34:35]\n" \
+    "s_and_b64 exec, exec, s[24:25]\n" \
     "global_store_dword v245, v241, s[64:65]\n" \
     "s_mov_b64 exec, s[62:63]\n" \
     "v_mov_b32 v248, v241\n" \
@@ -856,19 +1418,18 @@
     "s_nop 1\n" \
     "v_max_f32_dpp v248, v248, v248 row_bcast:31 row_mask:0xc bank_mask:0xf\n" \
     "s_nop 1\n" \
-    "v_readlane_b32 s33, v248, 63\n" \
-    "s_or_b32 s33, s33, 0x80000000\n" \
-    "s_lshl_b32 s34, s52, 3\n" \
-    "s_add_u32 s34, s34, 4\n" \
-    "v_mov_b32 v245, s34\n" \
-    "v_mov_b32 v248, s33\n" \
+    "v_readlane_b32 s22, v248, 63\n" \
+    "s_or_b32 s22, s22, 0x80000000\n" \
+    "s_lshl_b32 s23, s52, 3\n" \
+    "s_add_u32 s23, s23, 4\n" \
+    "v_mov_b32 v245, s23\n" \
+    "v_mov_b32 v248, s22\n" \
     "s_mov_b64 s[62:63], exec\n" \
     "s_mov_b64 exec, 1\n" \
-    "global_atomic_umax v245, v248, %[mm]\n" \
+    "global_atomic_umax v245, v248, s[18:19]\n" \
     "s_mov_b64 exec, s[62:63]\n" \
-    "s_load_dwordx16 s[36:51], %[hcnt], 0x0\n" \
-    "s_waitcnt vmcnt(0) lgkmcnt(0)\n" \
+    "s_waitcnt vmcnt(0)\n" \
     "s_branch SLH_ITEM\n" \
     "SLH_DONE:\n" \
     ""
-#define SL_HOT_CLOBBERS "v0", "v1", "v2", "v3", "v4", "v5", "v6", "v7", "v8", "v9", "v10", "v11", "v12", "v13", "v14", "v15", "v16", "v17", "v18", "v19", "v20", "v21", "v22", "v23", "v24", "v25", "v26", "v27", "v28", "v29", "v30", "v31", "v32", "v33", "v34", "v35", "v36", "v37", "v38", "v39", "v40", "v41", "v42", "v43", "v44", "v45", "v46", "v47", "v48", "v49", "v50", "v51", "v52", "v53", "v54", "v55", "v56", "v57", "v58", "v59", "v60", "v61", "v62", "v63", "v64", "v65", "v66", "v67", "v68", "v69", "v70", "v71", "v72", "v73", "v74", "v75", "v76", "v77", "v78", "v79", "v80", "v81", "v82", "v83", "v84", "v85", "v86", "v87", "v88", "v89", "v90", "v91", "v92", "v93", "v94", "v95", "v96", "v97", "v98", "v99", "v100", "v101", "v102", "v103", "v104", "v105", "v106", "v107", "v108", "v109", "v110", "v111", "v112", "v113", "v114", "v115", "v116", "v117", "v118", "v119", "v120", "v121", "v122", "v123", "v124", "v125", "v126", "v127", "v128", "v129", "v130", "v131", "v132", "v133", "v134", "v135", "v136", "v137", "v138", "v139", "v140", "v141", "v142", "v143", "v144", "v145", "v146", "v147", "v148", "v149", "v150", "v151", "v152", "v153", "v154", "v155", "v156", "v157", "v158", "v159", "v160", "v161", "v162", "v163", "v164", "v165", "v166", "v167", "v168", "v169", "v170", "v171", "v172", "v173", "v174", "v175", "v176", "v177", "v178", "v179", "v180", "v181", "v182", "v183", "v184", "v185", "v186", "v187", "v188", "v189", "v190", "v191", "v192", "v193", "v194", "v195", "v196", "v197", "v198", "v199", "v200", "v201", "v202", "v203", "v204", "v205", "v206", "v207", "v208", "v209", "v210", "v211", "v212", "v213", "v214", "v215", "v216", "v217", "v218", "v219", "v220", "v221", "v222", "v223", "v224", "v225", "v226", "v227", "v228", "v229", "v230", "v231", "v232", "v233", "v234", "v235", "v236", "v237", "v238", "v239", "v240", "v241", "v242", "v243", "v244", "v245", "v246", "v247", "v248", "v249", "v250", "v251", "v252", "v253", "v254", "v255", "s33", "s34", "s35", "s36", "s37", "s38", "s39", "s40", "s41", "s42", "s43", "s44", "s45", "s46", "s47", "s48", "s49", "s50", "s51", "s52", "s53", "s54", "s55", "s56", "s57", "s58", "s59", "s60", "s61", "s62", "s63", "s64", "s65", "s66", "s67", "s68", "s69", "s70", "s71", "s72", "s73", "s74", "s75", "s76", "s77", "s78", "s79", "s80", "s81", "s82", "s83", "s84", "s85", "s86", "s87", "s88", "s89", "s90", "s91", "s92", "s93", "s94", "s95", "s96", "s97", "s98", "s99", "s100", "s101", "vcc", "scc", "m0", "memory"
+#define SL_HOT_CLOBBERS "v0", "v1", "v2", "v3", "v4", "v5", "v6", "v7", "v8", "v9", "v10", "v11", "v12", "v13", "v14", "v15", "v16", "v17", "v18", "v19", "v20", "v21", "v22", "v23", "v24", "v25", "v26", "v27", "v28", "v29", "v30", "v31", "v32", "v33", "v34", "v35", "v36", "v37", "v38", "v39", "v40", "v41", "v42", "v43", "v44", "v45", "v46", "v47", "v48", "v49", "v50", "v51", "v52", "v53", "v54", "v55", "v56", "v57", "v58", "v59", "v60", "v61", "v62", "v63", "v64", "v65", "v66", "v67", "v68", "v69", "v70", "v71", "v72", "v73", "v74", "v75", "v76", "v77", "v78", "v79", "v80", "v81", "v82", "v83", "v84", "v85", "v86", "v87", "v88", "v89", "v90", "v91", "v92", "v93", "v94", "v95", "v96", "v97", "v98", "v99", "v100", "v101", "v102", "v103", "v104", "v105", "v106", "v107", "v108", "v109", "v110", "v111", "v112", "v113", "v114", "v115", "v116", "v117", "v118", "v119", "v120", "v121", "v122", "v123", "v124", "v125", "v126", "v127", "v128", "v129", "v130", "v131", "v132", "v133", "v134", "v135", "v136", "v137", "v138", "v139", "v140", "v141", "v142", "v143", "v144", "v145", "v146", "v147", "v148", "v149", "v150", "v151", "v152", "v153", "v154", "v155", "v156", "v157", "v158", "v159", "v160", "v161", "v162", "v163", "v164", "v165", "v166", "v167", "v168", "v169", "v170", "v171", "v172", "v173", "v174", "v175", "v176", "v177", "v178", "v179", "v180", "v181", "v182", "v183", "v184", "v185", "v186", "v187", "v188", "v189", "v190", "v191", "v192", "v193", "v194", "v195", "v196", "v197", "v198", "v199", "v200", "v201", "v202", "v203", "v204", "v205", "v206", "v207", "v208", "v209", "v210", "v211", "v212", "v213", "v214", "v215", "v216", "v217", "v218", "v219", "v220", "v221", "v222", "v223", "v224", "v225", "v226", "v227", "v228", "v229", "v230", "v231", "v232", "v233", "v234", "v235", "v236", "v237", "v238", "v239", "v240", "v241", "v242", "v243", "v244", "v245", "v246", "v247", "v248", "v249", "v250", "v251", "v252", "v253", "v254", "v255", "s4", "s5", "s6", "s7", "s8", "s9", "s10", "s11", "s12", "s13", "s14", "s15", "s16", "s17", "s18", "s19", "s20", "s21", "s22", "s23", "s24", "s25", "s26", "s27", "s28", "s29", "s30", "s31", "s32", "s33", "s34", "s35", "s36", "s37", "s38", "s39", "s40", "s41", "s42", "s43", "s44", "s45", "s46", "s47", "s48", "s49", "s50", "s51", "s52", "s53", "s54", "s55", "s56", "s57", "s58", "s59", "s60", "s61", "s62", "s63", "s64", "s65", "s66", "s67", "s68", "s69", "s70", "s71", "s72", "s73", "s74", "s75", "s76", "s77", "s78", "s79", "s80", "s81", "s82", "s83", "s84", "s85", "s86", "s87", "s88", "s89", "s90", "s91", "s92", "s93", "s94", "s95", "s96", "s97", "s98", "s99", "s100", "s101", "vcc", "scc", "m0", "memory"
```

Measured after the change: 47700 frames/s, median of 6. +1.0%, better.
